# fegemo/palette-and-histo-gan

Measured on AMD Instinct MI355X. Metric: train images/sec (64x64x4 sprites), higher is better.
Workload: dtype bf16

## Files before the change

### include/p2pgan.h

```cpp
#ifndef P2PGAN_H
#define P2PGAN_H

#ifdef __cplusplus
extern "C" {
#endif

typedef enum { P2P_F32 = 0, P2P_BF16 = 1 } p2p_dtype;
typedef enum { P2P_OP_G = 0, P2P_OP_P = 1, P2P_OP_W = 2 } p2p_convop;
typedef enum { P2P_ACT_NONE = 0, P2P_ACT_LEAKY = 1, P2P_ACT_RELU = 2 } p2p_act;

typedef struct {
    void* ptr;
    long long img_stride;
    int row_stride;
    int ld;
} p2p_tensor;

typedef struct {
    const void* ptr;
    int kind;
    int nslabs;
    long long slab_stride;
    int ld;
    int coff;
} p2p_gsrc;

const char* p2p_last_error(void);
int p2p_version(void);
int p2p_view_halo_pixels(void);


int p2p_conv_direct(int op, int stride, int dtype, int N, int LH, int LW, int Cg, int Cd,
                    const p2p_tensor* hi, const p2p_tensor* lo, const void* w, const float* bias,
                    float* dw, float* dbias, void* stream);

int p2p_igemm(int op, int dtype, int N, int LH, int LW, int Cg, int Cd,
              const p2p_tensor* hi, const p2p_tensor* lo, const void* w,
              int splitk, float* slabs, float* stat_part, void* stream);
int p2p_igemm_stat_slots(int op, int N, int LH, int LW, int ncols);

int p2p_brig_ok(int op, int dtype, int N, int LH, int LW, int Cg, int Cd);
int p2p_igemm_norm_act_ok(int op, int dtype, int N, int LH, int LW, int Cg, int Cd);
int p2p_igemm_norm_act(int op, int dtype, int N, int LH, int LW, int Cg, int Cd, const p2p_tensor* hi, const p2p_tensor* lo,
                       const void* w, const float* gamma, const float* beta, float eps, int act, float alpha,
                       const p2p_tensor* act_out, float* stats, void* stream);
int p2p_brig_stat_slots(int op, int dtype, int N, int LH, int LW, int Cg, int Cd);
int p2p_igemm_layer_stat_slots(int op, int dtype, int N, int LH, int LW, int Cg, int Cd);

int p2p_igemm_edge(int op, int stride, int dtype, int N, int LH, int LW, int cin_pad, int ncols, int w_rows,
                   const p2p_tensor* in, const p2p_tensor* out, const void* w, const float* bias,
                   int act, float alpha, void* stream);

int p2p_conv_strip_ok(int op, int dtype, int N, int LH, int LW, int Cg, int Cd);
int p2p_conv_strip_stat_slots(int op, int dtype, int N, int LH, int LW, int Cg, int Cd);
int p2p_conv_strip(int op, int dtype, int N, int LH, int LW, int Cg, int Cd,
                   const p2p_tensor* hi, const p2p_tensor* lo, const void* w, float* stat_part, void* stream);

int p2p_conv_fewout_ok(int op, int stride, int dtype, int N, int LH, int LW, int cin_pad, int ncols);
int p2p_conv_fewout(int op, int stride, int dtype, int N, int LH, int LW, int cin_pad, int ncols, int w_rows,
                    const p2p_tensor* in, const p2p_tensor* out, const void* w, const float* bias,
                    int act, float alpha, void* stream);

int p2p_conv_fewin_ok(int op, int stride, int dtype, int N, int LH, int LW, int cin_pad, int ncols);
int p2p_conv_fewin(int op, int stride, int dtype, int N, int LH, int LW, int cin_pad, int ncols, int w_rows,
                   const p2p_tensor* in, const p2p_tensor* out, const void* w, const float* bias,
                   int act, float alpha, void* stream);

int p2p_conv_fewin_actbwd(int op, int stride, int dtype, int N, int LH, int LW, int cin_pad, int ncols, int w_rows,
                          const p2p_tensor* in, const p2p_tensor* out, const void* w, const p2p_tensor* gate, float alpha,
                          void* stream);

long long p2p_wgemm_workspace_bytes(int N, int LH, int LW, int Cg, int Cd, int msplit);
int p2p_wgemm(int dtype, int N, int LH, int LW, int Cg, int Cd,
              const p2p_tensor* hi, const p2p_tensor* lo, float* dw,
              int msplit, void* workspace, void* stream);

int p2p_wgemm_edge(int dtype, int stride, int N, int LH, int LW, int Cg, int Cd,
                   const p2p_tensor* hi, const p2p_tensor* lo, float* dw,
                   int msplit, void* workspace, void* stream);

int p2p_wgrad_small_blocks(int dtype, int stride, int N, int LH, int LW, int Cg, int Cd, int hi_ld, int lo_ld);
int p2p_wgrad_small(int dtype, int stride, int N, int LH, int LW, int Cg, int Cd,
                    const p2p_tensor* hi, const p2p_tensor* lo, float* dw, void* workspace, void* stream);

long long p2p_view_colsum_workspace_bytes(int dtype, int N, int H, int W, int C, const p2p_tensor* v);
int p2p_view_colsum(int dtype, int N, int H, int W, int C, const p2p_tensor* v, float* out, float* workspace, void* stream);


int p2p_norm_act_fwd(int dtype, int N, int H, int W, int C,
                     const void* raw, int raw_kind, int nslabs, long long slab_stride,
                     const float* gamma, const float* beta, float eps, int act, float alpha,
                     const unsigned char* mask, const p2p_tensor* out, void* raw_out, float* stats,
                     float* ws, long long ws_bytes, int nsplit, void* stream);
int p2p_norm_act_fwd_tail(int dtype, int N, int H, int W, int C,
                          const void* raw, int raw_kind, int nslabs, long long slab_stride,
                          const float* gamma, const float* beta, float eps, int act, float alpha,
                          const unsigned char* mask, const p2p_tensor* out, void* raw_out, float* stats,
                          float* ws, long long ws_bytes, int nsplit, const p2p_tensor* tail, int tail_ch, void* stream);

int p2p_norm_act_bwd(int dtype, int N, int H, int W, int C,
                     const void* raw, const float* stats, const float* gamma, const float* beta,
                     int act, float alpha, const unsigned char* mask,
                     const p2p_gsrc* g1, const p2p_gsrc* g2,
                     const p2p_tensor* draw, float* dgamma_part, float* dbeta_part,
                     float* ws, long long ws_bytes, int nsplit, void* stream);

int p2p_act_bwd(int dtype, int N, int H, int W, int C, const p2p_tensor* act_out, const p2p_gsrc* g1,
                const p2p_gsrc* g2, float alpha, const p2p_tensor* draw, void* stream);

int p2p_colsum(const float* part, int rows, int cols, float scale, float* out, void* stream);

int p2p_colsum_batched(const float* part, const int* table, int ntasks, int max_cols, float* out, void* stream);


#define P2P_LOSS_BLOCKS 256
int p2p_loss_partials_sum(const float* partials, int K, float* out, void* stream);

int p2p_bce_logits(int dtype, int N2, int n_real, int H, int W, const p2p_tensor* logits,
                   float inv_count, const p2p_tensor* dlogits_d, const p2p_tensor* dlogits_g,
                   float* partials, void* stream);
int p2p_bce_logits_pad8(int dtype, int N2, int n_real, int H, int W, const p2p_tensor* logits,
                        float inv_count, const p2p_tensor* dlogits_d, const p2p_tensor* dlogits_g,
                        float* partials, void* stream);

int p2p_tanh_l1_fwd(int dtype, int N, int H, int W, int C, const p2p_tensor* z, const p2p_tensor* real,
                    const p2p_tensor* fake, float inv_count, float* partials, float* fake_f32, void* stream);
int p2p_tanh_l1_fwd_pair(int dtype, int N, int H, int W, const p2p_tensor* z, const p2p_tensor* real_pair,
                         const p2p_tensor* fake_pair, float inv_count, float* partials, float* fake_f32, void* stream);

int p2p_tanh_l1_bwd(int dtype, int N, int H, int W, int C, const p2p_tensor* fake, const p2p_tensor* real,
                    const p2p_gsrc* g_d, const p2p_gsrc* g_extra, float l1_scale,
                    const p2p_tensor* dz, void* stream);
int p2p_tanh_l1_bwd_pad8(int dtype, int N, int H, int W, const p2p_tensor* fake, const p2p_tensor* real,
                         const p2p_gsrc* g_d, const p2p_gsrc* g_extra, float l1_scale, const p2p_tensor* dz,
                         void* stream);


int p2p_rgbuv_hist_fwd(int dtype, int N, int H, int W, const p2p_tensor* img, float* hist, void* stream);
int p2p_rgbuv_hist_general(int dtype, int N, int H, int W, const p2p_tensor* img, int size, int method, float sigma, float* hist,
                           void* stream);

long long p2p_rgbuv_hist_fwd3_workspace_bytes(int N);
int p2p_rgbuv_hist_fwd3(int dtype, int N, int H, int W, const p2p_tensor* img, const float* points, const int* npoints, int cap,
                        float* hist, float* workspace, void* stream);
int p2p_rgbuv_points(int dtype, int N, int H, int W, const p2p_tensor* img, int cap, float* points, int* npoints, void* stream);

int p2p_hist_normalize(const float* raw, int N, float* out, void* stream);

int p2p_hellinger_fwd(const float* hist_true, const float* hist_pred, int N, float* tot_true, float* tot_pred,
                      float* sq_part, float* sq_sum, void* stream);
int p2p_hellinger_finish(const float* sq_sum, float inv_global_batch, float* loss_out, void* stream);
int p2p_rgbuv_hist_hellinger_bwd(int dtype, int N, int H, int W, const p2p_tensor* fake, const float* hist_true,
                                 const float* hist_pred, const float* tot_true, const float* tot_pred,
                                 const float* sq_sum, float coef, float* gh_ws, float* dimg, void* stream);
int p2p_rgbuv_hist_hellinger_bwd3(int dtype, int N, int H, int W, const p2p_tensor* fake, const float* hist_true,
                                  const float* hist_pred, const float* tot_true, const float* tot_pred, const float* sq_sum,
                                  float coef, float* gh_ws, float* dimg, void* stream);

int p2p_hist_normalize_bwd(const float* raw, const float* grad_out, int N, int size, float* gh, void* stream);
int p2p_rgbuv_hist_bwd(int dtype, int N, int H, int W, const p2p_tensor* img, const float* gh, float* dimg, void* stream);
int p2p_rgbuv_hist_general_bwd(int dtype, int N, int H, int W, const p2p_tensor* img, int size, int method, float sigma,
                               const float* gh, float* dimg, void* stream);

long long p2p_soft_palette_workspace_bytes(int N, int H, int W);
int p2p_soft_palette_fwd(int N, int H, int W, const float* img, const int* palette, const int* sizes, int K, float tau,
                         float* hist, float* conf, float* workspace, void* stream);
int p2p_soft_palette_bwd(int N, int H, int W, const float* img, const int* palette, const int* sizes, int K, float tau,
                         const float* gh, const float* gm, float* dimg, void* stream);
int p2p_palette_extract(int N, int H, int W, const float* img, int cap, int* palette_out, int* sizes_out, void* stream);
int p2p_palette_snap(int N, int H, int W, const float* img, const int* palette, const int* sizes, int K, int* index_out,
                     float* image_out, int* dist_out, int* counts_out, long long* stats_out, void* stream);

long long p2p_diffaug_workspace_bytes(int N, int H, int W);
int p2p_diffaug_fwd(int N, int H, int W, const float* img, const float* color, const int* geometry, int ch, int cw,
                    int policy_bits, float fill, float* out, float* workspace, void* stream);
int p2p_diffaug_bwd(int N, int H, int W, const float* grad_out, const float* color, const int* geometry, int ch, int cw,
                    int policy_bits, float fill, float* grad_img, float* workspace, void* stream);


#define P2P_SOFTMAX_MAX_BLOCKS 8192
int p2p_softmax_cce_argmax(int dtype, int N, int H, int W, int C, const p2p_tensor* z, const p2p_tensor* target,
                           const p2p_tensor* fake_idx, float grad_scale, float inv_count, const p2p_tensor* dz,
                           float* probs_out, float* loss_part, float* loss_out, void* stream);
int p2p_softmax_bwd(int dtype, int N, int H, int W, int C, const float* probs, const float* gp, const float* gz,
                    float scale, const p2p_tensor* dz, void* stream);
int p2p_argmax_lastdim(const float* probs, long long M, int C, int* out, void* stream);

int p2p_head_softmax_ok(int dtype, int N, int H, int W, int cin_pad, int ncls);
long long p2p_head_softmax_workspace_bytes(int N, int H);
int p2p_head_softmax_cce(int dtype, int N, int H, int W, int cin_pad, int ncls, const p2p_tensor* in, const void* wt,
                         const float* bias, const p2p_tensor* target, const p2p_tensor* fake_idx, float grad_scale,
                         float inv_count, const p2p_tensor* dz, float* dbias, float* workspace, float* loss_out, void* stream);
int p2p_head_dgrad_ok(int dtype, int N, int H, int W, int ncls, int cout, int w_rows, int dz_ld, int out_ld);
int p2p_head_dgrad(int dtype, int N, int H, int W, int ncls, int cout, const p2p_tensor* dz, const void* wn, int w_rows,
                   const p2p_tensor* out, void* stream);


int p2p_adam_flat(float* p, const float* g, float* m, float* v, long long n, int t,
                  float lr, float beta1, float beta2, float eps, float gscale, void* stream);

int p2p_adam_tick(int* t_dev, float* lr_t_dev, float lr, float beta1, float beta2, void* stream);
int p2p_adam_flat_dev(float* p, const float* g, float* m, float* v, long long n, const float* lr_t_dev,
                      float beta1, float beta2, float eps, float gscale, void* stream);
int p2p_counter_add(long long* counter_dev, long long inc, void* stream);
int p2p_grad_accumulate(float* dst, const float* src, long long n, int first, void* stream);

int p2p_weight_prep(int dtype, const float* w, int Cg, int Cd, void* wn, void* wt, void* stream);

int p2p_weight_prep_pad(int dtype, const float* w, int Cg, int Cd, void* wn, int wn_rows, int wn_cols,
                        void* wt, int wt_rows, int wt_cols, void* stream);

typedef struct p2p_prep_task {
    const float* w;
    void* wn;
    void* wt;
    int Cg, Cd, wn_rows, wn_cols, wt_rows, wt_cols, tiles_g, tiles_d;
    long long first_block;
} p2p_prep_task;
long long p2p_weight_prep_task_blocks(int Cg, int Cd, int wn_rows, int wn_cols, int wt_rows, int wt_cols,
                                      int have_wn, int have_wt, int* tiles_g, int* tiles_d);
int p2p_weight_prep_batched(int dtype, const p2p_prep_task* tasks_dev, int ntasks, long long total_blocks, void* stream);
int p2p_adam_prep_batched(int dtype, long long n_elems, const p2p_prep_task* tasks_dev, int ntasks, long long total_blocks,
                          float* params, const float* grads, float* m, float* v, const float* lr_t_dev, float beta1, float beta2,
                          float eps, void* stream);


int p2p_pack_input(int dtype, int N, int H, int W, int C, const void* src, int src_is_int,
                   const p2p_tensor* dst, void* stream);
int p2p_pack_input_multi(int dtype, int N, int H, int W, int C, const void* src, int src_is_int,
                         const p2p_tensor* dsts, int ndst, void* stream);
int p2p_pack_pair(int dtype, int N, int H, int W, const float* source, const float* target,
                  const p2p_tensor* v_src, const p2p_tensor* v_c6, const p2p_tensor* v_dreal, const p2p_tensor* v_dfake,
                  void* stream);
int p2p_pack_pair_idx(int dtype, int N, int H, int W, const int* source, const int* target,
                      const p2p_tensor* v_src, const p2p_tensor* v_c6, const p2p_tensor* v_dreal, const p2p_tensor* v_dfake,
                      void* stream);
int p2p_finish_losses(const float* slots, int aux_slot, int l1_slot, float lambda_l1, float lambda_aux, float* out,
                      void* stream);
int p2p_unpack(int dtype, int N, int H, int W, int C, const p2p_tensor* src, float* dst, void* stream);

int p2p_dropout_mask(unsigned char* mask, long long n, long long seed, long long counter, void* stream);
int p2p_dropout_mask_dev(unsigned char* mask, long long n, long long seed, const long long* counter_dev,
                         long long salt, long long elem_offset, void* stream);


int p2p_comm_unique_id(void* id_out_128_bytes);
int p2p_comm_init(const void* id_128_bytes, int rank, int world, void** comm_out);
int p2p_comm_allreduce_sum(void* comm, float* buf, long long n, void* stream);
int p2p_comm_destroy(void* comm);

int p2p_event_create(void** ev_out);
int p2p_event_destroy(void* ev);
int p2p_event_record(void* ev, void* stream);
int p2p_stream_wait_event(void* stream, void* ev);
int p2p_arm_stop_event(void* ev);
int p2p_disarm_stop_event(int* was_pending);

#define P2P_REPLAY_MAX_ARGS 24
typedef struct {
    int fn;
    int nargs;
    unsigned ind64;
    unsigned ind32;
    unsigned long long a[P2P_REPLAY_MAX_ARGS];
} p2p_replay_call;
int p2p_replay_fn_index(const char* name);
int p2p_replay_fn_nargs(int fn);
int p2p_replay(const p2p_replay_call* calls, int n);


int p2p_png_unfilter(const unsigned char* filtered, int height, int row_bytes, int bpp, unsigned char* out);

int p2p_sprites_rgba_batch(const void* sprites, int n_sprites, int S, const int* src_idx, const int* tgt_idx, const float* aug,
                           int B, int normalise, float* source, float* target, void* stream);

int p2p_gather_rows_i32(const int* table, int n_rows, int row_ints, const int* sel, int B, int* out, void* stream);

int p2p_palette_relabel_batch(const int* src_idx, const int* tgt_idx, const int* palette, const int* perm, const int* inv,
                              int B, int n, int P, int C, int* src_out, int* tgt_out, int* pal_out, void* stream);


int p2p_inc_prep(int N, int H, int W, int C, const float* images, const int* rows, const int* cols, const int* chans, int OH,
                 int OW, double w0, double w1, int filter, const p2p_tensor* out, float* minmax, void* stream);
int p2p_inc_conv(int N, int H, int W, int Cin, int kh, int kw, int stride, int pad_top, int pad_left, int OH, int OW, int Cout,
                 const p2p_tensor* in, const float* w, const float* scale, const float* shift, const p2p_tensor* out, void* stream);
int p2p_inc_pool(int kind, int N, int H, int W, int C, const p2p_tensor* in, const p2p_tensor* out, void* stream);
int p2p_inc_gap(int N, int H, int W, int C, const p2p_tensor* in, float* out, void* stream);

#ifdef __cplusplus
}
#endif
#endif
```

### palette_and_histo_gan_amd/_lib.py

```python
import ctypes as C
import os

HERE = os.path.dirname(os.path.abspath(__file__))
LIB_PATH = os.environ.get("P2P_LIB") or os.path.join(HERE, "libp2pgan_hip.so")

F32, BF16 = 0, 1
OP_G, OP_P, OP_W = 0, 1, 2
ACT_NONE, ACT_LEAKY, ACT_RELU = 0, 1, 2


class Tensor(C.Structure):
    _fields_ = [("ptr", C.c_void_p), ("img_stride", C.c_longlong), ("row_stride", C.c_int), ("ld", C.c_int)]


class GSrc(C.Structure):
    _fields_ = [("ptr", C.c_void_p), ("kind", C.c_int), ("nslabs", C.c_int), ("slab_stride", C.c_longlong),
                ("ld", C.c_int), ("coff", C.c_int)]


_TP = C.POINTER(Tensor)
_GP = C.POINTER(GSrc)
_vp, _i, _f, _ll = C.c_void_p, C.c_int, C.c_float, C.c_longlong

SIGNATURES = {
    "p2p_conv_direct": [_i, _i, _i, _i, _i, _i, _i, _i, _TP, _TP, _vp, _vp, _vp, _vp, _vp],
    "p2p_igemm": [_i, _i, _i, _i, _i, _i, _i, _TP, _TP, _vp, _i, _vp, _vp, _vp],
    "p2p_igemm_norm_act": [_i, _i, _i, _i, _i, _i, _i, _TP, _TP, _vp, _vp, _vp, _f, _i, _f, _TP, _vp, _vp],
    "p2p_igemm_edge": [_i, _i, _i, _i, _i, _i, _i, _i, _i, _TP, _TP, _vp, _vp, _i, _f, _vp],
    "p2p_conv_strip": [_i, _i, _i, _i, _i, _i, _i, _TP, _TP, _vp, _vp, _vp],
    "p2p_conv_fewin": [_i, _i, _i, _i, _i, _i, _i, _i, _i, _TP, _TP, _vp, _vp, _i, _f, _vp],
    "p2p_conv_fewin_actbwd": [_i, _i, _i, _i, _i, _i, _i, _i, _i, _TP, _TP, _vp, _TP, _f, _vp],
    "p2p_conv_fewout": [_i, _i, _i, _i, _i, _i, _i, _i, _i, _TP, _TP, _vp, _vp, _i, _f, _vp],
    "p2p_wgemm_edge": [_i, _i, _i, _i, _i, _i, _i, _TP, _TP, _vp, _i, _vp, _vp],
    "p2p_wgrad_small": [_i, _i, _i, _i, _i, _i, _i, _TP, _TP, _vp, _vp, _vp],
    "p2p_view_colsum": [_i, _i, _i, _i, _i, _TP, _vp, _vp, _vp],
    "p2p_act_bwd": [_i, _i, _i, _i, _i, _TP, _GP, _GP, _f, _TP, _vp],
    "p2p_weight_prep_pad": [_i, _vp, _i, _i, _vp, _i, _i, _vp, _i, _i, _vp],
    "p2p_wgemm": [_i, _i, _i, _i, _i, _i, _TP, _TP, _vp, _i, _vp, _vp],
    "p2p_norm_act_fwd": [_i, _i, _i, _i, _i, _vp, _i, _i, _ll, _vp, _vp, _f, _i, _f, _vp, _TP, _vp, _vp, _vp, _ll, _i, _vp],
    "p2p_norm_act_fwd_tail": [_i, _i, _i, _i, _i, _vp, _i, _i, _ll, _vp, _vp, _f, _i, _f, _vp, _TP, _vp, _vp, _vp, _ll, _i, _TP, _i, _vp],
    "p2p_norm_act_bwd": [_i, _i, _i, _i, _i, _vp, _vp, _vp, _vp, _i, _f, _vp, _GP, _GP, _TP, _vp, _vp, _vp, _ll, _i, _vp],
    "p2p_colsum": [_vp, _i, _i, _f, _vp, _vp],
    "p2p_colsum_batched": [_vp, _vp, _i, _i, _vp, _vp],
    "p2p_bce_logits": [_i, _i, _i, _i, _i, _TP, _f, _TP, _TP, _vp, _vp],
    "p2p_bce_logits_pad8": [_i, _i, _i, _i, _i, _TP, _f, _TP, _TP, _vp, _vp],
    "p2p_loss_partials_sum": [_vp, _i, _vp, _vp],
    "p2p_tanh_l1_fwd": [_i, _i, _i, _i, _i, _TP, _TP, _TP, _f, _vp, _vp, _vp],
    "p2p_tanh_l1_fwd_pair": [_i, _i, _i, _i, _TP, _TP, _TP, _f, _vp, _vp, _vp],
    "p2p_tanh_l1_bwd": [_i, _i, _i, _i, _i, _TP, _TP, _GP, _GP, _f, _TP, _vp],
    "p2p_tanh_l1_bwd_pad8": [_i, _i, _i, _i, _TP, _TP, _GP, _GP, _f, _TP, _vp],
    "p2p_adam_flat": [_vp, _vp, _vp, _vp, _ll, _i, _f, _f, _f, _f, _f, _vp],
    "p2p_adam_tick": [_vp, _vp, _f, _f, _f, _vp],
    "p2p_adam_flat_dev": [_vp, _vp, _vp, _vp, _ll, _vp, _f, _f, _f, _f, _vp],
    "p2p_counter_add": [_vp, _ll, _vp],
    "p2p_grad_accumulate": [_vp, _vp, _ll, _i, _vp],
    "p2p_dropout_mask_dev": [_vp, _ll, _ll, _vp, _ll, _ll, _vp],
    "p2p_weight_prep": [_i, _vp, _i, _i, _vp, _vp, _vp],
    "p2p_weight_prep_batched": [_i, _vp, _i, _ll, _vp],
    "p2p_adam_prep_batched": [_i, _ll, _vp, _i, _ll, _vp, _vp, _vp, _vp, _vp, _f, _f, _f, _vp],
    "p2p_pack_input": [_i, _i, _i, _i, _i, _vp, _i, _TP, _vp],
    "p2p_pack_pair": [_i, _i, _i, _i, _vp, _vp, _TP, _TP, _TP, _TP, _vp],
    "p2p_pack_pair_idx": [_i, _i, _i, _i, _vp, _vp, _TP, _TP, _TP, _TP, _vp],
    "p2p_pack_input_multi": [_i, _i, _i, _i, _i, _vp, _i, _TP, _i, _vp],
    "p2p_finish_losses": [_vp, _i, _i, _f, _f, _vp, _vp],
    "p2p_unpack": [_i, _i, _i, _i, _i, _TP, _vp, _vp],
    "p2p_dropout_mask": [_vp, _ll, _ll, _ll, _vp],
    "p2p_rgbuv_hist_fwd": [_i, _i, _i, _i, _TP, _vp, _vp],
    "p2p_hist_normalize": [_vp, _i, _vp, _vp],
    "p2p_rgbuv_hist_general": [_i, _i, _i, _i, _TP, _i, _i, _f, _vp, _vp],
    "p2p_rgbuv_hist_fwd3": [_i, _i, _i, _i, _TP, _vp, _vp, _i, _vp, _vp, _vp],
    "p2p_rgbuv_points": [_i, _i, _i, _i, _TP, _i, _vp, _vp, _vp],
    "p2p_hellinger_fwd": [_vp, _vp, _i, _vp, _vp, _vp, _vp, _vp],
    "p2p_hellinger_finish": [_vp, _f, _vp, _vp],
    "p2p_rgbuv_hist_hellinger_bwd": [_i, _i, _i, _i, _TP, _vp, _vp, _vp, _vp, _vp, _f, _vp, _vp, _vp],
    "p2p_rgbuv_hist_hellinger_bwd3": [_i, _i, _i, _i, _TP, _vp, _vp, _vp, _vp, _vp, _f, _vp, _vp, _vp],
    "p2p_hist_normalize_bwd": [_vp, _vp, _i, _i, _vp, _vp],
    "p2p_rgbuv_hist_bwd": [_i, _i, _i, _i, _TP, _vp, _vp, _vp],
    "p2p_rgbuv_hist_general_bwd": [_i, _i, _i, _i, _TP, _i, _i, _f, _vp, _vp, _vp],
    "p2p_soft_palette_fwd": [_i, _i, _i, _vp, _vp, _vp, _i, _f, _vp, _vp, _vp, _vp],
    "p2p_soft_palette_bwd": [_i, _i, _i, _vp, _vp, _vp, _i, _f, _vp, _vp, _vp, _vp],
    "p2p_palette_extract": [_i, _i, _i, _vp, _i, _vp, _vp, _vp],
    "p2p_palette_snap": [_i, _i, _i, _vp, _vp, _vp, _i, _vp, _vp, _vp, _vp, _vp, _vp],
    "p2p_diffaug_fwd": [_i, _i, _i, _vp, _vp, _vp, _i, _i, _i, _f, _vp, _vp, _vp],
    "p2p_diffaug_bwd": [_i, _i, _i, _vp, _vp, _vp, _i, _i, _i, _f, _vp, _vp, _vp],
    "p2p_softmax_cce_argmax": [_i, _i, _i, _i, _i, _TP, _TP, _TP, _f, _f, _TP, _vp, _vp, _vp, _vp],
    "p2p_softmax_bwd": [_i, _i, _i, _i, _i, _vp, _vp, _vp, _f, _TP, _vp],
    "p2p_argmax_lastdim": [_vp, _ll, _i, _vp, _vp],
    "p2p_head_dgrad": [_i, _i, _i, _i, _i, _i, _TP, _vp, _i, _TP, _vp],
    "p2p_head_softmax_cce": [_i, _i, _i, _i, _i, _i, _TP, _vp, _vp, _TP, _TP, _f, _f, _TP, _vp, _vp, _vp, _vp],
    "p2p_comm_unique_id": [_vp],
    "p2p_comm_init": [_vp, _i, _i, C.POINTER(_vp)],
    "p2p_comm_allreduce_sum": [_vp, _vp, _ll, _vp],
    "p2p_comm_destroy": [_vp],
    "p2p_event_create": [C.POINTER(_vp)],
    "p2p_event_destroy": [_vp],
    "p2p_event_record": [_vp, _vp],
    "p2p_stream_wait_event": [_vp, _vp],
    "p2p_arm_stop_event": [_vp],
    "p2p_disarm_stop_event": [C.POINTER(C.c_int)],
    "p2p_png_unfilter": [_vp, _i, _i, _i, _vp],
    "p2p_sprites_rgba_batch": [_vp, _i, _i, _vp, _vp, _vp, _i, _i, _vp, _vp, _vp],
    "p2p_gather_rows_i32": [_vp, _i, _i, _vp, _i, _vp, _vp],
    "p2p_palette_relabel_batch": [_vp, _vp, _vp, _vp, _vp, _i, _i, _i, _i, _vp, _vp, _vp, _vp],
    "p2p_inc_prep": [_i, _i, _i, _i, _vp, _vp, _vp, _vp, _i, _i, C.c_double, C.c_double, _i, _TP, _vp, _vp],
    "p2p_inc_conv": [_i, _i, _i, _i, _i, _i, _i, _i, _i, _i, _i, _i, _TP, _vp, _vp, _vp, _TP, _vp],
    "p2p_inc_pool": [_i, _i, _i, _i, _i, _TP, _TP, _vp],
    "p2p_inc_gap": [_i, _i, _i, _i, _TP, _vp, _vp],
}
SPECIAL = {"p2p_last_error": ([], C.c_char_p),
           "p2p_replay_fn_index": ([C.c_char_p], C.c_int), "p2p_replay_fn_nargs": ([_i], C.c_int),
           "p2p_replay": ([_vp, _i], C.c_int), "p2p_version": ([], C.c_int), "p2p_view_halo_pixels": ([], C.c_int),
           "p2p_igemm_stat_slots": ([_i, _i, _i, _i, _i], C.c_int),
           "p2p_brig_ok": ([_i, _i, _i, _i, _i, _i, _i], C.c_int),
           "p2p_igemm_norm_act_ok": ([_i, _i, _i, _i, _i, _i, _i], C.c_int),
           "p2p_brig_stat_slots": ([_i, _i, _i, _i, _i, _i, _i], C.c_int),
           "p2p_igemm_layer_stat_slots": ([_i, _i, _i, _i, _i, _i, _i], C.c_int),
           "p2p_conv_fewin_ok": ([_i, _i, _i, _i, _i, _i, _i, _i], C.c_int),
           "p2p_conv_strip_ok": ([_i, _i, _i, _i, _i, _i, _i], C.c_int),
           "p2p_conv_strip_stat_slots": ([_i, _i, _i, _i, _i, _i, _i], C.c_int),
           "p2p_conv_fewout_ok": ([_i, _i, _i, _i, _i, _i, _i, _i], C.c_int),
           "p2p_wgrad_small_blocks": ([_i, _i, _i, _i, _i, _i, _i, _i, _i], C.c_int),
           "p2p_wgemm_workspace_bytes": ([_i, _i, _i, _i, _i, _i], C.c_longlong),
           "p2p_rgbuv_hist_fwd3_workspace_bytes": ([_i], C.c_longlong),
           "p2p_soft_palette_workspace_bytes": ([_i, _i, _i], C.c_longlong),
           "p2p_diffaug_workspace_bytes": ([_i, _i, _i], C.c_longlong),
           "p2p_head_softmax_ok": ([_i, _i, _i, _i, _i, _i], C.c_int),
           "p2p_head_dgrad_ok": ([_i, _i, _i, _i, _i, _i, _i, _i, _i], C.c_int),
           "p2p_head_softmax_workspace_bytes": ([_i, _i], C.c_longlong),
           "p2p_view_colsum_workspace_bytes": ([_i, _i, _i, _i, _i, _TP], C.c_longlong),
           "p2p_weight_prep_task_blocks": ([_i, _i, _i, _i, _i, _i, _i, _i, C.POINTER(C.c_int), C.POINTER(C.c_int)], C.c_longlong)}


class PrepTask(C.Structure):
    _fields_ = [("w", C.c_void_p), ("wn", C.c_void_p), ("wt", C.c_void_p),
                ("Cg", C.c_int), ("Cd", C.c_int), ("wn_rows", C.c_int), ("wn_cols", C.c_int),
                ("wt_rows", C.c_int), ("wt_cols", C.c_int), ("tiles_g", C.c_int), ("tiles_d", C.c_int),
                ("first_block", C.c_longlong)]

_lib = None


class P2PError(RuntimeError):
    pass


def lib():
    global _lib
    if _lib is None:
        if not os.path.exists(LIB_PATH):
            raise P2PError(f"{LIB_PATH} is missing: run `python -c 'import __graft_entry__ as g; g.build()'` "
                           "(hipcc --offload-arch=gfx950); there is no CPU fallback")
        import torch
        L = C.CDLL(LIB_PATH)
        for name, argtypes in SIGNATURES.items():
            fn = getattr(L, name)
            fn.argtypes = argtypes
            fn.restype = C.c_int
        for name, (argtypes, restype) in SPECIAL.items():
            fn = getattr(L, name)
            fn.argtypes = argtypes
            fn.restype = restype
        _lib = L
    return _lib


_fns = {}


def call(name, *args):
    fn = _fns.get(name)
    if fn is None:
        fn = _fns[name] = getattr(lib(), name)
    rc = fn(*args)
    if rc != 0:
        raise P2PError(f"{name} failed (rc={rc}): {lib().p2p_last_error().decode()}")


def exported_symbols():
    return list(SIGNATURES) + list(SPECIAL)
```

### palette_and_histo_gan_amd/csrc/norm_act.hip

```cpp
#include "p2p_common.hpp"
#include <stdlib.h>

typedef __attribute__((__vector_size__(2 * sizeof(float)))) float f32x2;

template <typename T>
__device__ __forceinline__ float raw_load(const void* raw, int raw_kind, int nslabs, long long slab, long long e) {
    if (raw_kind == 1) return to_f32(((const T*)raw)[e]);
    float s = 0.f;
    const float* p = (const float*)raw + e;
    for (int k = 0; k < nslabs; ++k) s += p[(long long)k * slab];
    return to_f32(from_f32<T>(s));
}

template <typename T>
__global__ void norm_act_fwd_kernel(int H, int W, int C, int CB, const void* __restrict__ raw, int raw_kind,
                                    int nslabs, long long slab, const float* __restrict__ gamma,
                                    const float* __restrict__ beta, float eps, int act, float alpha,
                                    const unsigned char* __restrict__ mask, TView out, T* __restrict__ raw_out,
                                    float* __restrict__ stats) {
    extern __shared__ float sm[];
    const int n = blockIdx.x;
    const int c0 = blockIdx.y * CB;
    const int cb = min(CB, C - c0);
    const int PL = blockDim.x / CB;
// ... 877 lines not shown
        f32x4 tsum = red[0][cq];
#pragma unroll
        for (int i = 1; i < 16; ++i) tsum += red[i][cq];
        for (int k = 0; k < 4; ++k)
            if (c + k < cols) out[ooff + c + k] = tsum[k];
    }
}

extern "C" int p2p_colsum_batched(const float* part, const int* table, int ntasks, int max_cols, float* out, void* stream) {
    P2P_REQUIRE(part && table && out && ntasks > 0 && max_cols > 0, "p2p_colsum_batched: bad args");
    P2P_REQUIRE(((uintptr_t)part % 16) == 0, "p2p_colsum_batched: partials must be 16-byte aligned");
    colsum_batched_kernel<<<dim3((max_cols + 63) / 64, ntasks), 256, 0, (hipStream_t)stream>>>(part, table, out);
    return p2p_check_launch("p2p_colsum_batched");
}

template <typename T>
__global__ void act_bwd_kernel(int N, int H, int W, int C, TView actv, GSrc g1, GSrc g2, float alpha, TView draw) {
    long long total = (long long)N * H * W * C;
    for (long long i = (long long)blockIdx.x * blockDim.x + threadIdx.x; i < total; i += (long long)gridDim.x * blockDim.x) {
        int c = (int)(i % C);
        long long p = i / C;
        int x = (int)(p % W);
        int y = (int)((p / W) % H);
        int n = (int)(p / ((long long)W * H));
        float a = to_f32(((const T*)actv.ptr)[actv.off(n, y, x) + c]);
        float g = gsrc_load<T>(g1, p, c) + gsrc_load<T>(g2, p, c);
        ((T*)draw.ptr)[draw.off(n, y, x) + c] = from_f32<T>(a > 0.f ? g : alpha * g);
    }
}

template <typename T>
__global__ void act_bwd_vec_kernel(int N, int H, int W, int C, TView actv, GSrc g1, GSrc g2, float alpha, TView draw) {
    constexpr int VN = VecOf<T>::N;
    const int cv = C / VN;
    long long total = (long long)N * H * W * cv;
    for (long long i = (long long)blockIdx.x * blockDim.x + threadIdx.x; i < total; i += (long long)gridDim.x * blockDim.x) {
        int c = (int)(i % cv) * VN;
        long long p = i / cv;
        int x = (int)(p % W);
        int y = (int)((p / W) % H);
        int n = (int)(p / ((long long)W * H));
        float a[VN], ga[VN], gb[VN];
        vload<T>((const T*)actv.ptr + actv.off(n, y, x) + c, a);
        gsrc_vload<T>(g1, p, c, ga);
        gsrc_vload<T>(g2, p, c, gb);
#pragma unroll
        for (int k = 0; k < VN; ++k) { float g = ga[k] + gb[k]; a[k] = a[k] > 0.f ? g : alpha * g; }
        vstore<T>((T*)draw.ptr + draw.off(n, y, x) + c, a);
    }
}

extern "C" int p2p_act_bwd(int dtype, int N, int H, int W, int C, const p2p_tensor* act_out, const p2p_gsrc* g1,
                           const p2p_gsrc* g2, float alpha, const p2p_tensor* draw, void* stream) {
    P2P_REQUIRE(N > 0 && H > 0 && W > 0 && C > 0 && act_out && act_out->ptr && g1 && draw && draw->ptr, "p2p_act_bwd: bad args");
    {
        const int esz = dtype == P2P_BF16 ? 2 : 4, vn = 16 / esz;
        auto gs_ok = [&](const p2p_gsrc* g) {
            if (!g || !g->ptr || g->kind == 0) return true;
            return g->kind != 1 || (g->ld % vn == 0 && g->coff % vn == 0 && ((uintptr_t)g->ptr % 16) == 0);
        };
        if (C % 8 == 0 && act_out->ld % vn == 0 && draw->ld % vn == 0 && ((uintptr_t)act_out->ptr % 16) == 0 &&
            ((uintptr_t)draw->ptr % 16) == 0 && gs_ok(g1) && gs_ok(g2)) {
            long long tv = (long long)N * H * W * (C / vn);
            long long bl = (tv + 255) / 256;
            if (bl > 8192) bl = 8192;
            P2P_DISPATCH_DTYPE(dtype, P2P_LAUNCH_LAST((act_bwd_vec_kernel<T>), dim3((unsigned)bl), dim3(256), 0, (hipStream_t)stream,
                                                      N, H, W, C, make_view(act_out), make_gsrc(g1), make_gsrc(g2), alpha, make_view(draw)));
            return p2p_check_launch("p2p_act_bwd");
        }
    }
    long long total = (long long)N * H * W * C;
    long long blocks = (total + 255) / 256;
    if (blocks > 4096) blocks = 4096;
    P2P_DISPATCH_DTYPE(dtype, (act_bwd_kernel<T><<<dim3((unsigned)blocks), 256, 0, (hipStream_t)stream>>>(
                                  N, H, W, C, make_view(act_out), make_gsrc(g1), make_gsrc(g2), alpha, make_view(draw))));
    return p2p_check_launch("p2p_act_bwd");
}

__global__ void colsum_kernel(const float* __restrict__ part, int rows, int cols, float scale, float* __restrict__ out) {
    int c = blockIdx.x * blockDim.x + threadIdx.x;
    if (c >= cols) return;
    float s = 0.f;
    for (int r = 0; r < rows; ++r) s += part[(long long)r * cols + c];
    out[c] = s * scale;
}

static inline int pick_cb(int C) { return C >= 64 ? 64 : (C >= 32 ? 32 : (C >= 16 ? 16 : (C >= 8 ? 8 : (C >= 4 ? 4 : (C >= 2 ? 2 : 1))))); }

static int norm_act_fwd_impl(int dtype, int N, int H, int W, int C, const void* raw, int raw_kind, int nslabs,
                             long long slab_stride, const float* gamma, const float* beta, float eps, int act,
                             float alpha, const unsigned char* mask, const p2p_tensor* out, void* raw_out,
                             float* stats, float* ws, long long ws_bytes, int nsplit, const p2p_tensor* tail, int tail_ch,
                             void* stream) {
    P2P_REQUIRE(N > 0 && H > 0 && W > 0 && C > 0, "p2p_norm_act_fwd: bad shape");
    P2P_REQUIRE(raw && out && out->ptr, "p2p_norm_act_fwd: null pointer");
    P2P_REQUIRE(raw_kind == 1 || (raw_kind == 2 && nslabs >= 1), "p2p_norm_act_fwd: bad raw_kind/nslabs");
    P2P_REQUIRE((gamma == nullptr) == (beta == nullptr), "p2p_norm_act_fwd: gamma/beta must both be set or null");
    P2P_REQUIRE(!gamma || stats, "p2p_norm_act_fwd: stats required with normalisation");
    const int esz = dtype == P2P_BF16 ? 2 : 4, vn = 16 / esz;
    const bool vec = C % vn == 0 && out->ld % vn == 0 && ((uintptr_t)out->ptr % 16) == 0 && ((uintptr_t)raw % 16) == 0 &&
                     (!raw_out || ((uintptr_t)raw_out % 16) == 0) && (raw_kind == 1 || slab_stride % 4 == 0) && C % 8 == 0;
    const int tvecs = tail ? tail_ch / vn : 0;
    TView tv = tail ? make_view(tail) : TView{};
    if (tail) {
        P2P_REQUIRE(tail->ptr && tail_ch > 0 && tail_ch % vn == 0 && tail->ld % vn == 0 && ((uintptr_t)tail->ptr % 16) == 0,
                    "p2p_norm_act_fwd_tail: the tail must be whole 16-byte vectors");
        int cgt = C > 64 ? 64 : C;
        while (C % cgt) cgt -= vn;
        P2P_REQUIRE(vec && H * W > 16 && 256 % (cgt / vn) == 0, "p2p_norm_act_fwd_tail: shape not served by the vector form");
    }
    if (vec && H * W <= 16) {
        int lgG, ppl;
        small_geom(H * W, lgG, ppl);
        const long long items = (long long)N * (C / vn);
        const long long threads = items << lgG;
        const dim3 grid((unsigned)((threads + 255) / 256));
        hipStream_t st = (hipStream_t)stream;
#define NF_SMALL2(P_, S_) norm_act_fwd_small<T, P_, S_><<<grid, 256, 0, st>>>(H * W, W, C, lgG, items, raw, raw_kind, nslabs, slab_stride, gamma, \
                                                                   beta, eps, act, alpha, mask, make_view(out), (T*)raw_out, stats)
#define NF_SMALL(P_) do { if (raw_kind == 2) NF_SMALL2(P_, 4); else NF_SMALL2(P_, 0); } while (0)
        if (ppl == 1) { P2P_DISPATCH_DTYPE(dtype, NF_SMALL(1)); }
        else if (ppl == 2) { P2P_DISPATCH_DTYPE(dtype, NF_SMALL(2)); }
        else { P2P_DISPATCH_DTYPE(dtype, NF_SMALL(4)); }
#undef NF_SMALL
#undef NF_SMALL2
        return p2p_check_launch("p2p_norm_act_fwd");
    }
    const bool legacy = nsplit > 0 && (nsplit & 0x100);
    const int n_geom = (nsplit > 0 && (nsplit & 0x200)) ? 256 : N;
    if (nsplit > 0) nsplit &= 0xff;
    if (vec && gamma && !tail && nsplit >= 0 && !legacy) {
        int ppl = 0;
        const int rcg = norm_bwd_reg_geom(n_geom, H * W, C, vn, ppl, true);
        if (rcg) {
            hipStream_t st = (hipStream_t)stream;
            const dim3 grid((unsigned)(((N + 7) / 8) * 8 * (C / rcg)));
#define NF_REG2(P_, S_) norm_act_fwd_reg<T, P_, S_><<<grid, 256, 0, st>>>(N, H * W, W, C, rcg, raw, raw_kind, nslabs, slab_stride, gamma, beta, eps, act, alpha, \
                                                                mask, make_view(out), (T*)raw_out, stats)
#define NF_REG(P_) do { if (raw_kind == 2) NF_REG2(P_, 4); else NF_REG2(P_, 0); } while (0)
            if (ppl == 1) { P2P_DISPATCH_DTYPE(dtype, NF_REG(1)); }
            else if (ppl == 2) { P2P_DISPATCH_DTYPE(dtype, NF_REG(2)); }
            else if (ppl == 4) { P2P_DISPATCH_DTYPE(dtype, NF_REG(4)); }
            else { P2P_DISPATCH_DTYPE(dtype, NF_REG(8)); }
#undef NF_REG
#undef NF_REG2
            return p2p_check_launch("p2p_norm_act_fwd");
        }
    }
    if (vec) {
        int CG = C > 64 ? 64 : C;
        while (C % CG) CG -= vn;
        int vpp = CG / vn;
        if (256 % vpp == 0) {
            hipStream_t st = (hipStream_t)stream;
            const int prr = 256 / vpp;
            int sp = nsplit < 1 ? 1 : nsplit;
            while (sp > 1 && (H * W + sp - 1) / sp < prr) sp >>= 1;
            if (nsplit < 0 && gamma && ws) {
                const int nslots = -nsplit;
                int sp2 = 1;
                while ((long long)N * (C / CG) * sp2 < 2048 && (H * W) / (sp2 * 2) >= prr && sp2 < 64) sp2 *= 2;
                dim3 grid3(N, C / CG, sp2);
                P2P_DISPATCH_DTYPE(dtype, (norm_act_fwd_vec<T, 3><<<grid3, 256, 0, st>>>(
                                              H, W, C, CG, raw, raw_kind, nslabs, slab_stride, gamma, beta, eps, act, alpha, mask,
                                              make_view(out), (T*)raw_out, stats, ws, nslots, tv, tvecs)));
                return p2p_check_launch("p2p_norm_act_fwd");
            }
            if (!ws || (long long)N * sp * C * 2 * 4 > ws_bytes) sp = gamma ? 1 : sp;
            dim3 grid(N, C / CG, sp);
            if (sp == 1 || !gamma) {
                P2P_DISPATCH_DTYPE(dtype, (norm_act_fwd_vec<T, 0><<<grid, 256, 0, st>>>(
                                              H, W, C, CG, raw, raw_kind, nslabs, slab_stride, gamma, beta, eps, act, alpha, mask,
                                              make_view(out), (T*)raw_out, stats, ws, 0, tv, tvecs)));
            } else {
                P2P_DISPATCH_DTYPE(dtype, (norm_act_fwd_vec<T, 1><<<grid, 256, 0, st>>>(
                                              H, W, C, CG, raw, raw_kind, nslabs, slab_stride, gamma, beta, eps, act, alpha, mask,
                                              make_view(out), (T*)raw_out, stats, ws, 0, tv, tvecs)));
                P2P_DISPATCH_DTYPE(dtype, (norm_act_fwd_vec<T, 2><<<grid, 256, 0, st>>>(
                                              H, W, C, CG, raw, raw_kind, nslabs, slab_stride, gamma, beta, eps, act, alpha, mask,
                                              make_view(out), (T*)raw_out, stats, ws, 0, tv, tvecs)));
            }
            return p2p_check_launch("p2p_norm_act_fwd");
        }
    }
    int CB = pick_cb(C);
    dim3 grid(N, (C + CB - 1) / CB);
    size_t shm = sizeof(float) * 256;
    P2P_DISPATCH_DTYPE(dtype, (norm_act_fwd_kernel<T><<<grid, 256, shm, (hipStream_t)stream>>>(
                                  H, W, C, CB, raw, raw_kind, nslabs, slab_stride, gamma, beta, eps, act, alpha, mask,
                                  make_view(out), (T*)raw_out, stats)));
    return p2p_check_launch("p2p_norm_act_fwd");
}

extern "C" int p2p_norm_act_fwd(int dtype, int N, int H, int W, int C, const void* raw, int raw_kind, int nslabs,
                                long long slab_stride, const float* gamma, const float* beta, float eps, int act,
                                float alpha, const unsigned char* mask, const p2p_tensor* out, void* raw_out,
                                float* stats, float* ws, long long ws_bytes, int nsplit, void* stream) {
    return norm_act_fwd_impl(dtype, N, H, W, C, raw, raw_kind, nslabs, slab_stride, gamma, beta, eps, act, alpha, mask, out,
                             raw_out, stats, ws, ws_bytes, nsplit, nullptr, 0, stream);
}

extern "C" int p2p_norm_act_fwd_tail(int dtype, int N, int H, int W, int C, const void* raw, int raw_kind, int nslabs,
                                     long long slab_stride, const float* gamma, const float* beta, float eps, int act,
                                     float alpha, const unsigned char* mask, const p2p_tensor* out, void* raw_out,
                                     float* stats, float* ws, long long ws_bytes, int nsplit, const p2p_tensor* tail,
                                     int tail_ch, void* stream) {
    P2P_REQUIRE(tail, "p2p_norm_act_fwd_tail: null tail");
    return norm_act_fwd_impl(dtype, N, H, W, C, raw, raw_kind, nslabs, slab_stride, gamma, beta, eps, act, alpha, mask, out,
                             raw_out, stats, ws, ws_bytes, nsplit, tail, tail_ch, stream);
}

extern "C" int p2p_norm_act_bwd(int dtype, int N, int H, int W, int C, const void* raw, const float* stats,
                                const float* gamma, const float* beta, int act, float alpha,
                                const unsigned char* mask, const p2p_gsrc* g1, const p2p_gsrc* g2,
                                const p2p_tensor* draw, float* dgamma_part, float* dbeta_part, float* ws,
                                long long ws_bytes, int nsplit, void* stream) {
    P2P_REQUIRE(N > 0 && H > 0 && W > 0 && C > 0, "p2p_norm_act_bwd: bad shape");
    P2P_REQUIRE(raw && draw && draw->ptr && g1, "p2p_norm_act_bwd: null pointer");
    P2P_REQUIRE(!gamma || (stats && beta && dgamma_part && dbeta_part), "p2p_norm_act_bwd: norm needs stats/beta/partials");
    const int esz = dtype == P2P_BF16 ? 2 : 4, vn = 16 / esz;
    auto gs_ok = [&](const p2p_gsrc* g) {
        if (!g || !g->ptr || g->kind == 0) return true;
        if (g->kind == 1) return g->ld % vn == 0 && g->coff % vn == 0 && ((uintptr_t)g->ptr % 16) == 0;
        return true;
    };
    const bool vec = gamma && C % 8 == 0 && draw->ld % vn == 0 && ((uintptr_t)draw->ptr % 16) == 0 &&
                     ((uintptr_t)raw % 16) == 0 && gs_ok(g1) && gs_ok(g2);
    const bool g_slabs = (g1 && g1->kind == 2) || (g2 && g2->kind == 2);
    if (vec && H * W <= 16) {
        int lgG, ppl;
        small_geom(H * W, lgG, ppl);
        const long long items = (long long)N * (C / vn);
        const long long threads = items << lgG;
        const dim3 grid((unsigned)((threads + 255) / 256));
        hipStream_t st = (hipStream_t)stream;
#define NB_SMALL2(P_, S_) P2P_LAUNCH_LAST((norm_act_bwd_small<T, P_, S_>), grid, dim3(256), 0, st, H * W, W, C, lgG, items, (const T*)raw, stats, gamma, beta, act, \
                                     alpha, mask, make_gsrc(g1), make_gsrc(g2), make_view(draw), dgamma_part, dbeta_part)
#define NB_SMALL(P_) do { if (g_slabs) NB_SMALL2(P_, 4); else NB_SMALL2(P_, 0); } while (0)
        if (ppl == 1) { P2P_DISPATCH_DTYPE(dtype, NB_SMALL(1)); }
        else if (ppl == 2) { P2P_DISPATCH_DTYPE(dtype, NB_SMALL(2)); }
        else { P2P_DISPATCH_DTYPE(dtype, NB_SMALL(4)); }
#undef NB_SMALL
#undef NB_SMALL2
        return p2p_check_launch("p2p_norm_act_bwd");
    }
    const bool legacy = nsplit > 0 && (nsplit & 0x100);
    const int n_geom = (nsplit > 0 && (nsplit & 0x200)) ? 256 : N;
    if (nsplit > 0) nsplit &= 0xff;
    if (vec && !legacy) {
        int ppl = 0;
        const int rcg = norm_bwd_reg_geom(n_geom, H * W, C, vn, ppl);
        if (rcg) {
            hipStream_t st = (hipStream_t)stream;
            const dim3 grid((unsigned)(((N + 7) / 8) * 8 * (C / rcg)));
#define NB_REG2(P_, S_) P2P_LAUNCH_LAST((norm_act_bwd_reg<T, P_, S_>), grid, dim3(256), 0, st, N, H * W, W, C, rcg, (const T*)raw, stats, gamma, beta, act, \
                                   alpha, mask, make_gsrc(g1), make_gsrc(g2), make_view(draw), dgamma_part, dbeta_part)
#define NB_REG(P_) do { if (g_slabs) NB_REG2(P_, 4); else NB_REG2(P_, 0); } while (0)
            if (ppl == 1) { P2P_DISPATCH_DTYPE(dtype, NB_REG(1)); }
            else if (ppl == 2) { P2P_DISPATCH_DTYPE(dtype, NB_REG(2)); }
            else if (ppl == 4) { P2P_DISPATCH_DTYPE(dtype, NB_REG(4)); }
            else { P2P_DISPATCH_DTYPE(dtype, NB_REG(8)); }
#undef NB_REG
#undef NB_REG2
            return p2p_check_launch("p2p_norm_act_bwd");
        }
    }
    if (vec) {
        int CG = C > 64 ? 64 : C;
        while (C % CG) CG -= vn;
        const bool narrow = nsplit > 1 && CG == 64 && C % 32 == 0 && (long long)N * (C / 32) >= 1024 && H * W >= 64;
        if (narrow) CG = 32;
        int vpp = CG / vn;
        if (256 % vpp == 0) {
            hipStream_t st = (hipStream_t)stream;
            const int prr = 256 / vpp;
            int sp = (nsplit < 1 || narrow) ? 1 : nsplit;
            while (sp > 1 && (H * W + sp - 1) / sp < prr) sp >>= 1;
            if (!ws || (long long)N * sp * C * 2 * 4 > ws_bytes) sp = 1;
            dim3 grid(N, C / CG, sp);
            if (sp == 1) {
                P2P_DISPATCH_DTYPE(dtype, P2P_LAUNCH_LAST((norm_act_bwd_vec<T, 0>), grid, dim3(256), 0, st,
                                                          H, W, C, CG, (const T*)raw, stats, gamma, beta, act, alpha, mask, make_gsrc(g1),
                                                          make_gsrc(g2), make_view(draw), dgamma_part, dbeta_part, ws));
            } else {
                P2P_DISPATCH_DTYPE(dtype, (norm_act_bwd_vec<T, 1><<<grid, 256, 0, st>>>(
                                              H, W, C, CG, (const T*)raw, stats, gamma, beta, act, alpha, mask, make_gsrc(g1),
                                              make_gsrc(g2), make_view(draw), dgamma_part, dbeta_part, ws)));
                P2P_DISPATCH_DTYPE(dtype, P2P_LAUNCH_LAST((norm_act_bwd_vec<T, 2>), grid, dim3(256), 0, st,
                                                          H, W, C, CG, (const T*)raw, stats, gamma, beta, act, alpha, mask, make_gsrc(g1),
                                                          make_gsrc(g2), make_view(draw), dgamma_part, dbeta_part, ws));
            }
            return p2p_check_launch("p2p_norm_act_bwd");
        }
    }
    int CB = pick_cb(C);
    dim3 grid(N, (C + CB - 1) / CB);
    size_t shm = sizeof(float) * 512;
    P2P_DISPATCH_DTYPE(dtype, (norm_act_bwd_kernel<T><<<grid, 256, shm, (hipStream_t)stream>>>(
                                  H, W, C, CB, (const T*)raw, stats, gamma, beta, act, alpha, mask, make_gsrc(g1),
                                  make_gsrc(g2), make_view(draw), dgamma_part, dbeta_part)));
    return p2p_check_launch("p2p_norm_act_bwd");
}

extern "C" int p2p_colsum(const float* part, int rows, int cols, float scale, float* out, void* stream) {
    P2P_REQUIRE(part && out && rows > 0 && cols > 0, "p2p_colsum: bad args");
    colsum_kernel<<<dim3((cols + 255) / 256), 256, 0, (hipStream_t)stream>>>(part, rows, cols, scale, out);
    return p2p_check_launch("p2p_colsum");
}
```

### palette_and_histo_gan_amd/csrc/optim.hip

```cpp
#include "p2p_common.hpp"
#include <math.h>
#include <stdlib.h>

__global__ void adam_flat_kernel(float* __restrict__ p, const float* __restrict__ g, float* __restrict__ m,
                                 float* __restrict__ v, long long n, float lr_t, float b1, float b2, float eps,
                                 float gscale) {
    long long i = (long long)blockIdx.x * blockDim.x + threadIdx.x;
    long long stride = (long long)gridDim.x * blockDim.x;
    for (; i < n; i += stride) {
        float gi = g[i] * gscale;
        float mi = b1 * m[i] + (1.f - b1) * gi;
        float vi = b2 * v[i] + (1.f - b2) * gi * gi;
        m[i] = mi;
        v[i] = vi;
        p[i] = p[i] - lr_t * mi / (sqrtf(vi) + eps);
    }
}

extern "C" int p2p_adam_flat(float* p, const float* g, float* m, float* v, long long n, int t, float lr, float beta1,
                             float beta2, float eps, float gscale, void* stream) {
    P2P_REQUIRE(p && g && m && v && n > 0 && t >= 1, "p2p_adam_flat: bad args");
    double lr_t = (double)lr * sqrt(1.0 - pow((double)beta2, (double)t)) / (1.0 - pow((double)beta1, (double)t));
    long long blocks = (n + 255) / 256;
    if (blocks > 4096) blocks = 4096;
    adam_flat_kernel<<<dim3((unsigned)blocks), 256, 0, (hipStream_t)stream>>>(p, g, m, v, n, (float)lr_t, beta1, beta2,
                                                                             eps, gscale);
    return p2p_check_launch("p2p_adam_flat");
}

__global__ void adam_tick_kernel(int* __restrict__ t, float* __restrict__ lr_t, float lr, float b1, float b2) {
    int tt = t[0] + 1;
    t[0] = tt;
    lr_t[0] = (float)((double)lr * sqrt(1.0 - pow((double)b2, (double)tt)) / (1.0 - pow((double)b1, (double)tt)));
}

__global__ void adam_flat_dev_kernel(float* __restrict__ p, const float* __restrict__ g, float* __restrict__ m,
                                     float* __restrict__ v, long long n, const float* __restrict__ lr_t_dev, float b1,
                                     float b2, float eps, float gscale) {
    const float lr_t = lr_t_dev[0];
    long long i = ((long long)blockIdx.x * blockDim.x + threadIdx.x) * 4;
    long long stride = (long long)gridDim.x * blockDim.x * 4;
    for (; i + 3 < n; i += stride) {
        f32x4 gi = *(const f32x4*)(g + i), mi = *(const f32x4*)(m + i), vi = *(const f32x4*)(v + i), pi = *(const f32x4*)(p + i);
#pragma unroll
        for (int k = 0; k < 4; ++k) {
            float gg = gi[k] * gscale;
            mi[k] = b1 * mi[k] + (1.f - b1) * gg;
            vi[k] = b2 * vi[k] + (1.f - b2) * gg * gg;
            pi[k] = pi[k] - lr_t * mi[k] / (sqrtf(vi[k]) + eps);
        }
        *(f32x4*)(m + i) = mi; *(f32x4*)(v + i) = vi; *(f32x4*)(p + i) = pi;
    }
    if (blockIdx.x == 0 && threadIdx.x == 0)
        for (long long j = n / 4 * 4; j < n; ++j) {
            float gg = g[j] * gscale;
            float mj = b1 * m[j] + (1.f - b1) * gg, vj = b2 * v[j] + (1.f - b2) * gg * gg;
            m[j] = mj; v[j] = vj; p[j] = p[j] - lr_t * mj / (sqrtf(vj) + eps);
        }
}

extern "C" int p2p_adam_tick(int* t_dev, float* lr_t_dev, float lr, float beta1, float beta2, void* stream) {
    P2P_REQUIRE(t_dev && lr_t_dev, "p2p_adam_tick: null pointer");
    adam_tick_kernel<<<1, 1, 0, (hipStream_t)stream>>>(t_dev, lr_t_dev, lr, beta1, beta2);
    return p2p_check_launch("p2p_adam_tick");
}

extern "C" int p2p_adam_flat_dev(float* p, const float* g, float* m, float* v, long long n, const float* lr_t_dev,
                                 float beta1, float beta2, float eps, float gscale, void* stream) {
    P2P_REQUIRE(p && g && m && v && n > 0 && lr_t_dev, "p2p_adam_flat_dev: bad args");
    P2P_REQUIRE(((uintptr_t)p % 16) == 0 && ((uintptr_t)g % 16) == 0 && ((uintptr_t)m % 16) == 0 && ((uintptr_t)v % 16) == 0,
                "p2p_adam_flat_dev: buffers must be 16-byte aligned");
    long long blocks = (n / 4 + 255) / 256;
    if (blocks > 8192) blocks = 8192;
    if (blocks < 1) blocks = 1;
    adam_flat_dev_kernel<<<dim3((unsigned)blocks), 256, 0, (hipStream_t)stream>>>(p, g, m, v, n, lr_t_dev, beta1, beta2, eps, gscale);
    return p2p_check_launch("p2p_adam_flat_dev");
}

__global__ void counter_add_kernel(long long* c, long long inc) { c[0] += inc; }

extern "C" int p2p_counter_add(long long* counter_dev, long long inc, void* stream) {
    P2P_REQUIRE(counter_dev, "p2p_counter_add: null pointer");
    counter_add_kernel<<<1, 1, 0, (hipStream_t)stream>>>(counter_dev, inc);
    return p2p_check_launch("p2p_counter_add");
}

__global__ void grad_accumulate_kernel(float* __restrict__ dst, const float* __restrict__ src, long long n, int first) {
    long long i = ((long long)blockIdx.x * blockDim.x + threadIdx.x) * 4;
    long long stride = (long long)gridDim.x * blockDim.x * 4;
    for (; i + 3 < n; i += stride) {
        f32x4 s = *(const f32x4*)(src + i);
        if (!first) {
            f32x4 d = *(const f32x4*)(dst + i);
#pragma unroll
            for (int k = 0; k < 4; ++k) s[k] = d[k] + s[k];
        }
        *(f32x4*)(dst + i) = s;
    }
    if (blockIdx.x == 0 && threadIdx.x == 0)
        for (long long j = n / 4 * 4; j < n; ++j) dst[j] = first ? src[j] : dst[j] + src[j];
}

extern "C" int p2p_grad_accumulate(float* dst, const float* src, long long n, int first, void* stream) {
    P2P_REQUIRE(dst && src && n > 0, "p2p_grad_accumulate: bad args");
    P2P_REQUIRE(((uintptr_t)dst % 16) == 0 && ((uintptr_t)src % 16) == 0, "p2p_grad_accumulate: buffers must be 16-byte aligned");
    long long blocks = (n / 4 + 255) / 256;
    if (blocks > 8192) blocks = 8192;
    if (blocks < 1) blocks = 1;
    grad_accumulate_kernel<<<dim3((unsigned)blocks), 256, 0, (hipStream_t)stream>>>(dst, src, n, first);
    return p2p_check_launch("p2p_grad_accumulate");
}

template <typename T>
__device__ __forceinline__ void weight_prep_tile(const float* __restrict__ w, int Cg, int Cd, T* __restrict__ wn, int wn_rows,
                                                 int wn_cols, T* __restrict__ wt, int wt_rows, int wt_cols, int t, int g0, int d0,
                                                 float (*tile)[33]) {
    const float* wp = w + (long long)t * Cg * Cd;
    int tx = threadIdx.x & 31, ty = threadIdx.x >> 5;
    for (int r = ty; r < 32; r += 8) {
        int g = g0 + r, d = d0 + tx;
        float val = (g < Cg && d < Cd) ? wp[(long long)g * Cd + d] : 0.f;
        tile[r][tx] = val;
        if (wn && g < wn_rows && d < wn_cols) wn[((long long)t * wn_rows + g) * wn_cols + d] = from_f32<T>(val);
    }
    __syncthreads();
    if (wt) {
        for (int r = ty; r < 32; r += 8) {
            int d = d0 + r, g = g0 + tx;
            if (d < wt_rows && g < wt_cols) wt[((long long)t * wt_rows + d) * wt_cols + g] = from_f32<T>(tile[tx][r]);
        }
    }
}

template <typename T>
__global__ void weight_prep_kernel(const float* __restrict__ w, int Cg, int Cd, T* __restrict__ wn, int wn_rows,
                                   int wn_cols, T* __restrict__ wt, int wt_rows, int wt_cols) {
    __shared__ float tile[32][33];
    weight_prep_tile<T>(w, Cg, Cd, wn, wn_rows, wn_cols, wt, wt_rows, wt_cols, blockIdx.z, blockIdx.y * 32, blockIdx.x * 32, tile);
}

static __host__ __device__ inline bool prep_tile64(int Cg, int Cd, int wn_rows, int wn_cols, int wt_rows, int wt_cols,
                                                   bool have_wn, bool have_wt) {
    return Cg % 64 == 0 && Cd % 64 == 0 && (!have_wn || (wn_rows == Cg && wn_cols == Cd)) &&
           (!have_wt || (wt_rows == Cd && wt_cols == Cg));
}

template <typename T>
__device__ __forceinline__ void weight_prep_tile64(const float* __restrict__ w, int Cg, int Cd, T* __restrict__ wn,
                                                   T* __restrict__ wt, int t, int g0, int d0, float (*tile)[65]) {
    typedef __attribute__((__vector_size__(4 * sizeof(T)))) T vec4_t;
    const float* wp = w + (long long)t * Cg * Cd;
    const int c4 = (threadIdx.x & 15) * 4, r0 = threadIdx.x >> 4;
#pragma unroll
    for (int i = 0; i < 4; ++i) {
        const int r = r0 + 16 * i;
        const f32x4 v = *(const f32x4*)(wp + (long long)(g0 + r) * Cd + d0 + c4);
        tile[r][c4] = v[0]; tile[r][c4 + 1] = v[1]; tile[r][c4 + 2] = v[2]; tile[r][c4 + 3] = v[3];
        if (wn) {
            vec4_t q;
#pragma unroll
            for (int k = 0; k < 4; ++k) q[k] = from_f32<T>(v[k]);
            *(vec4_t*)(wn + ((long long)t * Cg + g0 + r) * Cd + d0 + c4) = q;
        }
    }
    __syncthreads();
    if (wt) {
#pragma unroll
        for (int i = 0; i < 4; ++i) {
            const int d = r0 + 16 * i;
            vec4_t q;
#pragma unroll
            for (int k = 0; k < 4; ++k) q[k] = from_f32<T>(tile[c4 + k][d]);
            *(vec4_t*)(wt + ((long long)t * Cd + d0 + d) * Cg + g0 + c4) = q;
        }
    }
}

template <typename T>
__global__ void weight_prep_batched_kernel(const p2p_prep_task* __restrict__ tasks, int ntasks) {
    __shared__ float tile[64][65];
    const long long b = blockIdx.x;
    int ti = 0;
    while (ti + 1 < ntasks && tasks[ti + 1].first_block <= b) ++ti;
    const p2p_prep_task k = tasks[ti];
    const int local = (int)(b - k.first_block);
    const int per_tap = k.tiles_g * k.tiles_d;
    const int t = local / per_tap, rem = local - t * per_tap;
    const int gy = rem / k.tiles_d, dx = rem - gy * k.tiles_d;
    if (prep_tile64(k.Cg, k.Cd, k.wn_rows, k.wn_cols, k.wt_rows, k.wt_cols, k.wn != nullptr, k.wt != nullptr)) {
        weight_prep_tile64<T>(k.w, k.Cg, k.Cd, (T*)k.wn, (T*)k.wt, t, gy * 64, dx * 64, tile);
        return;
    }
    weight_prep_tile<T>(k.w, k.Cg, k.Cd, (T*)k.wn, k.wn_rows, k.wn_cols, (T*)k.wt, k.wt_rows, k.wt_cols, t, gy * 32, dx * 32,
                        (float (*)[33])tile);
}

struct AdamCtx { float* p0; const float* g0; float* m0; float* v0; const float* lr_t; float b1, b2, eps; };

#define ADAM_ONE(p, g, m, v)                                   \
    do {                                                       \
        m = c.b1 * (m) + (1.f - c.b1) * (g);                   \
        v = c.b2 * (v) + (1.f - c.b2) * (g) * (g);             \
        p = (p) - lr_t * (m) / (sqrtf(v) + c.eps);             \
    } while (0)

template <typename T>
__global__ void adam_prep_batched_kernel(const p2p_prep_task* __restrict__ tasks, int ntasks, AdamCtx c) {
    typedef __attribute__((__vector_size__(4 * sizeof(T)))) T vec4_t;
    __shared__ float tile[64][65];
    const long long b = blockIdx.x;
    int ti = 0;
    while (ti + 1 < ntasks && tasks[ti + 1].first_block <= b) ++ti;
    const p2p_prep_task k = tasks[ti];
    const int local = (int)(b - k.first_block);
    const int per_tap = k.tiles_g * k.tiles_d;
    const int t = local / per_tap, rem = local - t * per_tap;
    const int gy = rem / k.tiles_d, dx = rem - gy * k.tiles_d;
    const float lr_t = c.lr_t[0];
    const long long base = (k.w - c.p0) + (long long)t * k.Cg * k.Cd;
    T* wn = (T*)k.wn;
    T* wt = (T*)k.wt;
    if (prep_tile64(k.Cg, k.Cd, k.wn_rows, k.wn_cols, k.wt_rows, k.wt_cols, wn != nullptr, wt != nullptr)) {
        const int g0 = gy * 64, d0 = dx * 64;
        const int c4 = (threadIdx.x & 15) * 4, r0 = threadIdx.x >> 4;
#pragma unroll
        for (int i = 0; i < 4; ++i) {
            const int r = r0 + 16 * i;
            const long long e = base + (long long)(g0 + r) * k.Cd + d0 + c4;
            f32x4 pv = *(const f32x4*)(c.p0 + e), mv = *(const f32x4*)(c.m0 + e), vv = *(const f32x4*)(c.v0 + e);
            const f32x4 gv = *(const f32x4*)(c.g0 + e);
#pragma unroll
            for (int q = 0; q < 4; ++q) ADAM_ONE(pv[q], gv[q], mv[q], vv[q]);
            *(f32x4*)(c.p0 + e) = pv; *(f32x4*)(c.m0 + e) = mv; *(f32x4*)(c.v0 + e) = vv;
            tile[r][c4] = pv[0]; tile[r][c4 + 1] = pv[1]; tile[r][c4 + 2] = pv[2]; tile[r][c4 + 3] = pv[3];
            if (wn) {
                vec4_t q4;
#pragma unroll
                for (int q = 0; q < 4; ++q) q4[q] = from_f32<T>(pv[q]);
                *(vec4_t*)(wn + ((long long)t * k.Cg + g0 + r) * k.Cd + d0 + c4) = q4;
            }
        }
        __syncthreads();
        if (wt) {
#pragma unroll
            for (int i = 0; i < 4; ++i) {
                const int d = r0 + 16 * i;
                vec4_t q4;
#pragma unroll
                for (int q = 0; q < 4; ++q) q4[q] = from_f32<T>(tile[c4 + q][d]);
                *(vec4_t*)(wt + ((long long)t * k.Cd + d0 + d) * k.Cg + g0 + c4) = q4;
            }
        }
        return;
    }
    float (*t32)[33] = (float (*)[33])tile;
    const int g0 = gy * 32, d0 = dx * 32;
    const int tx = threadIdx.x & 31, ty = threadIdx.x >> 5;
    for (int r = ty; r < 32; r += 8) {
        const int g = g0 + r, d = d0 + tx;
        float val = 0.f;
        if (g < k.Cg && d < k.Cd) {
            const long long e = base + (long long)g * k.Cd + d;
            float pv = c.p0[e], mv = c.m0[e], vv = c.v0[e];
            const float gv = c.g0[e];
            ADAM_ONE(pv, gv, mv, vv);
            val = pv;
            c.p0[e] = pv; c.m0[e] = mv; c.v0[e] = vv;
        }
        t32[r][tx] = val;
        if (wn && g < k.wn_rows && d < k.wn_cols) wn[((long long)t * k.wn_rows + g) * k.wn_cols + d] = from_f32<T>(val);
    }
    __syncthreads();
    if (wt) {
        for (int r = ty; r < 32; r += 8) {
            const int d = d0 + r, g = g0 + tx;
            if (d < k.wt_rows && g < k.wt_cols) wt[((long long)t * k.wt_rows + d) * k.wt_cols + g] = from_f32<T>(t32[tx][r]);
        }
    }
}

extern "C" int p2p_adam_prep_batched(int dtype, long long n_elems, const p2p_prep_task* tasks_dev, int ntasks, long long total_blocks,
                                     float* params, const float* grads, float* m, float* v, const float* lr_t_dev, float beta1,
                                     float beta2, float eps, void* stream) {
    P2P_REQUIRE(tasks_dev && ntasks >= 1 && ntasks <= 64 && total_blocks >= 1 && total_blocks < (1LL << 31) && n_elems > 0,
                "p2p_adam_prep_batched: bad args");
    P2P_REQUIRE(params && grads && m && v && lr_t_dev, "p2p_adam_prep_batched: null pointer");
    P2P_REQUIRE(((uintptr_t)params % 16) == 0 && ((uintptr_t)grads % 16) == 0 && ((uintptr_t)m % 16) == 0 && ((uintptr_t)v % 16) == 0,
                "p2p_adam_prep_batched: buffers must be 16-byte aligned");
    AdamCtx c = {params, grads, m, v, lr_t_dev, beta1, beta2, eps};
    P2P_DISPATCH_DTYPE(dtype, (adam_prep_batched_kernel<T><<<dim3((unsigned)total_blocks), 256, 0, (hipStream_t)stream>>>(tasks_dev, ntasks, c)));
    return p2p_check_launch("p2p_adam_prep_batched");
}

extern "C" long long p2p_weight_prep_task_blocks(int Cg, int Cd, int wn_rows, int wn_cols, int wt_rows, int wt_cols,
                                                 int have_wn, int have_wt, int* tiles_g, int* tiles_d) {
    int gmax = Cg, dmax = Cd;
    if (have_wn) { gmax = gmax > wn_rows ? gmax : wn_rows; dmax = dmax > wn_cols ? dmax : wn_cols; }
    if (have_wt) { gmax = gmax > wt_cols ? gmax : wt_cols; dmax = dmax > wt_rows ? dmax : wt_rows; }
    const int ts = prep_tile64(Cg, Cd, wn_rows, wn_cols, wt_rows, wt_cols, have_wn != 0, have_wt != 0) ? 64 : 32;
    const int tg = (gmax + ts - 1) / ts, td = (dmax + ts - 1) / ts;
    if (tiles_g) *tiles_g = tg;
    if (tiles_d) *tiles_d = td;
    return 16LL * tg * td;
}

extern "C" int p2p_weight_prep_batched(int dtype, const p2p_prep_task* tasks_dev, int ntasks, long long total_blocks, void* stream) {
    P2P_REQUIRE(tasks_dev && ntasks >= 1 && ntasks <= 64 && total_blocks >= 1 && total_blocks < (1LL << 31),
                "p2p_weight_prep_batched: bad args");
    P2P_DISPATCH_DTYPE(dtype, (weight_prep_batched_kernel<T><<<dim3((unsigned)total_blocks), 256, 0, (hipStream_t)stream>>>(tasks_dev, ntasks)));
    return p2p_check_launch("p2p_weight_prep_batched");
}

extern "C" int p2p_weight_prep_pad(int dtype, const float* w, int Cg, int Cd, void* wn, int wn_rows, int wn_cols,
                                   void* wt, int wt_rows, int wt_cols, void* stream) {
    P2P_REQUIRE(w && Cg > 0 && Cd > 0 && (wn || wt), "p2p_weight_prep: bad args");
    int gmax = Cg, dmax = Cd;
    if (wn) { gmax = gmax > wn_rows ? gmax : wn_rows; dmax = dmax > wn_cols ? dmax : wn_cols; }
    if (wt) { gmax = gmax > wt_cols ? gmax : wt_cols; dmax = dmax > wt_rows ? dmax : wt_rows; }
    dim3 grid((dmax + 31) / 32, (gmax + 31) / 32, 16);
    P2P_DISPATCH_DTYPE(dtype, (weight_prep_kernel<T><<<grid, 256, 0, (hipStream_t)stream>>>(
                                  w, Cg, Cd, (T*)wn, wn_rows, wn_cols, (T*)wt, wt_rows, wt_cols)));
    return p2p_check_launch("p2p_weight_prep");
}

extern "C" int p2p_weight_prep(int dtype, const float* w, int Cg, int Cd, void* wn, void* wt, void* stream) {
    return p2p_weight_prep_pad(dtype, w, Cg, Cd, wn, Cg, Cd, wt, Cd, Cg, stream);
}

template <typename T>
__global__ void pack_input_kernel(int N, PixDec dec, int C, const void* __restrict__ src, int src_is_int, TView dst) {
    const unsigned npix = (unsigned)N * dec.H * dec.W;
    for (unsigned p = blockIdx.x * blockDim.x + threadIdx.x; p < npix; p += gridDim.x * blockDim.x) {
        int n, y, x;
        dec(p, n, y, x);
        T* d = (T*)dst.ptr + dst.off(n, y, x);
        const long long e = (long long)p * C;
        for (int c = 0; c < C; ++c) {
            float v = src_is_int ? (float)((const int*)src)[e + c] : ((const float*)src)[e + c];
            d[c] = from_f32<T>(v);
        }
    }
}

struct PackDst { TView v[4]; int n; };

template <typename T>
__global__ void pack_multi_kernel(int N, PixDec dec, int C, const void* __restrict__ src, int src_is_int, PackDst dst) {
    const unsigned npix = (unsigned)N * dec.H * dec.W;
    for (unsigned p = blockIdx.x * blockDim.x + threadIdx.x; p < npix; p += gridDim.x * blockDim.x) {
        int n, y, x;
        dec(p, n, y, x);
        if (C == 4 && !src_is_int) {
            typedef __attribute__((__vector_size__(4 * sizeof(T)))) T vec4_t;
            f32x4 v = *(const f32x4*)((const float*)src + (long long)p * 4);
            vec4_t q;
#pragma unroll
            for (int k = 0; k < 4; ++k) q[k] = from_f32<T>(v[k]);
#pragma unroll
            for (int k = 0; k < 4; ++k)
                if (k < dst.n) *(vec4_t*)((T*)dst.v[k].ptr + dst.v[k].off(n, y, x)) = q;
            continue;
        }
        const long long e = (long long)p * C;
        for (int c = 0; c < C; ++c) {
            float v = src_is_int ? (float)((const int*)src)[e + c] : ((const float*)src)[e + c];
            T q = from_f32<T>(v);
#pragma unroll
            for (int k = 0; k < 4; ++k)
                if (k < dst.n) ((T*)dst.v[k].ptr)[dst.v[k].off(n, y, x) + c] = q;
        }
    }
}

template <typename T>
__global__ void pack_pair_kernel(int N, PixDec dec, const float* __restrict__ source, const float* __restrict__ target, TView v_src,
                                 TView v_c6, TView v_dreal, TView v_dfake) {
    typedef __attribute__((__vector_size__(4 * sizeof(T)))) T vec4_t;
    typedef __attribute__((__vector_size__(8 * sizeof(T)))) T vec8_t;
    const unsigned npix = (unsigned)N * dec.H * dec.W;
// ... 186 lines not shown
```

### palette_and_histo_gan_amd/csrc/replay.hip

```cpp
#include "p2p_common.hpp"
#include <string.h>
#include <utility>

namespace {

template <typename T>
inline T slot_as(unsigned long long v) {
    static_assert(sizeof(T) <= 8, "replayable entry points take scalars and pointers only");
    T t;
    memcpy(&t, &v, sizeof(T));
    return t;
}

template <typename... A, size_t... I>
inline int call_slots(int (*fn)(A...), const unsigned long long* a, std::index_sequence<I...>) {
    return fn(slot_as<A>(a[I])...);
}

template <typename... A>
constexpr int arg_count(int (*)(A...)) { return (int)sizeof...(A); }

template <auto Fn>
struct Thunk {
    template <typename... A>
    static int go(int (*fn)(A...), const unsigned long long* a) { return call_slots(fn, a, std::index_sequence_for<A...>{}); }
    static int call(const unsigned long long* a) { return go(Fn, a); }
};

struct Entry {
    const char* name;
    int (*call)(const unsigned long long*);
    int nargs;
};

#define P2P_E(f) {#f, &Thunk<&f>::call, arg_count(&f)},
constexpr Entry TABLE[] = {
    P2P_E(p2p_conv_direct) P2P_E(p2p_igemm) P2P_E(p2p_igemm_norm_act)
    P2P_E(p2p_igemm_edge) P2P_E(p2p_conv_strip) P2P_E(p2p_conv_fewin)
    P2P_E(p2p_conv_fewin_actbwd) P2P_E(p2p_conv_fewout) P2P_E(p2p_wgemm_edge)
    P2P_E(p2p_wgrad_small) P2P_E(p2p_view_colsum) P2P_E(p2p_act_bwd)
    P2P_E(p2p_weight_prep_pad) P2P_E(p2p_wgemm) P2P_E(p2p_norm_act_fwd)
    P2P_E(p2p_norm_act_fwd_tail) P2P_E(p2p_norm_act_bwd) P2P_E(p2p_colsum)
    P2P_E(p2p_colsum_batched) P2P_E(p2p_bce_logits) P2P_E(p2p_bce_logits_pad8)
    P2P_E(p2p_loss_partials_sum) P2P_E(p2p_tanh_l1_fwd) P2P_E(p2p_tanh_l1_fwd_pair)
    P2P_E(p2p_tanh_l1_bwd) P2P_E(p2p_tanh_l1_bwd_pad8) P2P_E(p2p_adam_flat)
    P2P_E(p2p_adam_tick) P2P_E(p2p_adam_flat_dev) P2P_E(p2p_counter_add) P2P_E(p2p_grad_accumulate)
    P2P_E(p2p_dropout_mask_dev) P2P_E(p2p_weight_prep) P2P_E(p2p_weight_prep_batched)
    P2P_E(p2p_adam_prep_batched) P2P_E(p2p_pack_input) P2P_E(p2p_pack_pair)
    P2P_E(p2p_pack_pair_idx) P2P_E(p2p_pack_input_multi) P2P_E(p2p_finish_losses)
    P2P_E(p2p_unpack) P2P_E(p2p_dropout_mask) P2P_E(p2p_rgbuv_hist_fwd)
    P2P_E(p2p_hist_normalize) P2P_E(p2p_rgbuv_hist_general) P2P_E(p2p_rgbuv_hist_fwd3) P2P_E(p2p_rgbuv_points)
    P2P_E(p2p_hellinger_fwd) P2P_E(p2p_hellinger_finish) P2P_E(p2p_rgbuv_hist_hellinger_bwd)
    P2P_E(p2p_rgbuv_hist_hellinger_bwd3) P2P_E(p2p_softmax_cce_argmax) P2P_E(p2p_argmax_lastdim)
    P2P_E(p2p_head_dgrad) P2P_E(p2p_head_softmax_cce) P2P_E(p2p_comm_unique_id)
    P2P_E(p2p_comm_init) P2P_E(p2p_comm_allreduce_sum) P2P_E(p2p_comm_destroy)
    P2P_E(p2p_event_create) P2P_E(p2p_event_destroy) P2P_E(p2p_event_record)
    P2P_E(p2p_stream_wait_event) P2P_E(p2p_arm_stop_event) P2P_E(p2p_disarm_stop_event) P2P_E(p2p_png_unfilter) P2P_E(p2p_sprites_rgba_batch)
    P2P_E(p2p_gather_rows_i32) P2P_E(p2p_palette_relabel_batch) P2P_E(p2p_hist_normalize_bwd)
    P2P_E(p2p_rgbuv_hist_bwd) P2P_E(p2p_rgbuv_hist_general_bwd) P2P_E(p2p_softmax_bwd)
    P2P_E(p2p_inc_prep) P2P_E(p2p_inc_conv) P2P_E(p2p_inc_pool) P2P_E(p2p_inc_gap)
    P2P_E(p2p_soft_palette_fwd) P2P_E(p2p_soft_palette_bwd) P2P_E(p2p_palette_extract)
    P2P_E(p2p_palette_snap) P2P_E(p2p_diffaug_fwd) P2P_E(p2p_diffaug_bwd)
};
#undef P2P_E
constexpr int NFN = (int)(sizeof(TABLE) / sizeof(TABLE[0]));

constexpr bool table_fits() {
    for (int i = 0; i < NFN; ++i)
        if (TABLE[i].nargs > P2P_REPLAY_MAX_ARGS) return false;
    return true;
}
static_assert(table_fits(), "an entry point has more arguments than P2P_REPLAY_MAX_ARGS");

}

extern "C" int p2p_replay_fn_index(const char* name) {
    if (!name) return -1;
    for (int i = 0; i < NFN; ++i)
        if (strcmp(TABLE[i].name, name) == 0) return i;
    return -1;
}

extern "C" int p2p_replay_fn_nargs(int fn) { return (fn >= 0 && fn < NFN) ? TABLE[fn].nargs : -1; }

extern "C" int p2p_replay(const p2p_replay_call* calls, int n) {
    P2P_REQUIRE(calls || n == 0, "p2p_replay: null call list");
    for (int i = 0; i < n; ++i) {
        const p2p_replay_call& c = calls[i];
        P2P_REQUIRE(c.fn >= 0 && c.fn < NFN && c.nargs == TABLE[c.fn].nargs, "p2p_replay: call %d: bad entry %d / %d arguments", i,
                    c.fn, c.nargs);
        const unsigned long long* ap = c.a;
        unsigned long long a[P2P_REPLAY_MAX_ARGS];
        if (c.ind64 | c.ind32) {
            for (int k = 0; k < c.nargs; ++k) {
                unsigned long long v = c.a[k];
                if ((c.ind64 >> k) & 1u) v = *(const unsigned long long*)(uintptr_t)v;
                else if ((c.ind32 >> k) & 1u) v = *(const unsigned*)(uintptr_t)v;
                a[k] = v;
            }
            ap = a;
        }
        const int rc = TABLE[c.fn].call(ap);
        if (rc != 0) {
            char why[400];
            strncpy(why, p2p_last_error(), sizeof(why) - 1);
            why[sizeof(why) - 1] = 0;
            p2p_set_error("p2p_replay: call %d of %d (%s) failed: %s", i, n, TABLE[c.fn].name, why);
            return rc;
        }
    }
    return 0;
}
```

### palette_and_histo_gan_amd/engine.py

```python
from collections import OrderedDict
import ctypes as C
import math
import os

import numpy as np
import torch

from . import _lib as L
from . import histogram as _histogram

HALO = 2
IN_EPS = 1e-3
LEAKY_ALPHA = 0.3
DOWN_FILTERS = (64, 128, 256, 512, 512, 512)
UP_FILTERS = (512, 512, 256, 128, 64, 32)
UP_DROPOUT = (True, True, True, False, False, False)
MAX_PALETTE_SIZE = 256


def _torch_dtype(dtype):
    return torch.float32 if dtype == L.F32 else torch.bfloat16


_RAW_STREAM = getattr(torch._C, "_cuda_getCurrentRawStream", None)
# ... 123 lines not shown


def _raw(stream):
    return C.c_void_p(stream.cuda_stream)


def _order(after, before):
    ev = _ring_event()
    _op("p2p_event_record", ev, _raw(before))
    _op("p2p_stream_wait_event", _raw(after), ev)


class _SideStream:

    def __init__(self, device, enabled):
        self.enabled = enabled and torch.device(device).type == "cuda"
        self.stream = torch.cuda.Stream(device=device) if self.enabled else None
        self.stop_event_forks = os.environ.get("P2P_STOP_EVENT_FORKS", "1") != "0"
        self._pending = None

    def prefork(self):
        if self.enabled and self.stop_event_forks and not torch.cuda.is_current_stream_capturing():
            self._pending = _ring_event()
            _op("p2p_arm_stop_event", self._pending)

    def fork(self):
        if not self.enabled:
            return
        ev, self._pending = self._pending, None
        if ev is not None:
            unclaimed = C.c_int(0)
            if L.lib().p2p_disarm_stop_event(C.byref(unclaimed)) != 0:
                raise L.P2PError(L.lib().p2p_last_error().decode())
            if not unclaimed.value:
                _op("p2p_stream_wait_event", _raw(self.stream), ev)
                return
            if _REC[0] is not None:
                _REC[0].append(("p2p_disarm_stop_event", (None,)))
        _order(self.stream, torch.cuda.current_stream())

    def run(self):
        return torch.cuda.stream(self.stream) if self.enabled else _NullCtx()

    def join(self):
        if self.enabled:
            _order(torch.cuda.current_stream(), self.stream)


class _LightEvent:
    def __init__(self, st):
        self.ev = _ring_event()
        _op("p2p_event_record", self.ev, _raw(st))

    def wait(self, st):
        _op("p2p_stream_wait_event", _raw(st), self.ev)


def _record_event():
    return _LightEvent(torch.cuda.current_stream())


def _wait_event(ev):
    ev.wait(torch.cuda.current_stream())


class _NullCtx:
    def __enter__(self):
        return self

    def __exit__(self, *a):
        return False


class HaloBuf:

    def __init__(self, n, h, w, c, dtype, device):
        self.n, self.h, self.w, self.c, self.dtype = n, h, w, c, dtype
        self.hp, self.wp = h + 2 * HALO, w + 2 * HALO
        numel = n * self.hp * self.wp * c
        self._flat = torch.zeros(numel + 256, dtype=_torch_dtype(dtype), device=device)
        self.t = self._flat[:numel].view(n, self.hp, self.wp, c)
        self.esz = self.t.element_size()
        self._views = {}

    def view(self, coff=0, n0=0):
        v = self._views.get((coff, n0))
        if v is None:
            off = ((n0 * self.hp + HALO) * self.wp + HALO) * self.c + coff
            v = self._views[(coff, n0)] = L.Tensor(self.t.data_ptr() + off * self.esz, self.hp * self.wp, self.wp, self.c)
        return v


class DenseBuf:

    def __init__(self, n, h, w, c, torch_dtype, device):
        self.n, self.h, self.w, self.c = n, h, w, c
        self.t = torch.empty((n * h * w, c), dtype=torch_dtype, device=device)
        self.esz = self.t.element_size()
        self._views = {}

    def view(self, coff=0, n0=0):
        v = self._views.get((coff, n0))
        if v is None:
            v = self._views[(coff, n0)] = L.Tensor(self.t.data_ptr() + (n0 * self.h * self.w * self.c + coff) * self.esz,
                                                   self.h * self.w, self.w, self.c)
        return v

    def ptr(self, n0=0):
        return C.c_void_p(self.t.data_ptr() + n0 * self.h * self.w * self.c * self.esz)

    def gsrc(self, coff=0, kind=1, nslabs=1, n0=0):
        return L.GSrc(self.t.data_ptr() + n0 * self.h * self.w * self.c * self.esz, kind, nslabs,
                      self.n * self.h * self.w * self.c, self.c, coff)


def pad8(c):
    return (c + 7) // 8 * 8


def up32(c):
    return (c + 31) // 32 * 32


def _p(t, off_elems=0):
    return C.c_void_p(t.data_ptr() + off_elems * t.element_size())


NULL = C.c_void_p(0)


class ParamStore:

    BUCKET_MIN = 4 * 1024 * 1024

    def __init__(self, shapes, device):
        self.shapes = OrderedDict(shapes)
        self.offsets = OrderedDict()
        kernels = [k for k in self.shapes if k.endswith(".kernel")]
        small = [k for k in self.shapes if not k.endswith(".kernel")]
        off, self.buckets, start, self.bucket_of = 0, [], 0, {}
        for k in reversed(kernels):
            self.offsets[k] = off
            off += int(np.prod(self.shapes[k]))
            off = (off + 3) // 4 * 4
            self.bucket_of[k[:-7]] = len(self.buckets)
            if off - start >= self.BUCKET_MIN:
                self.buckets.append((start, off))
                start = off
        if off > start:
            self.buckets.append((start, off))
        self.bucket_last_layer = {}
        for k in reversed(kernels):
            self.bucket_last_layer[self.bucket_of[k[:-7]]] = k[:-7]
        self.small_range = (off, off)
        for k in small:
            self.offsets[k] = off
            off += int(np.prod(self.shapes[k]))
            off = (off + 3) // 4 * 4
        self.small_range = (self.small_range[0], off)
        self.numel = off
        self.params = torch.zeros(off, dtype=torch.float32, device=device)
        self.grads = None
        self.m = torch.zeros(off, dtype=torch.float32, device=device)
        self.v = torch.zeros(off, dtype=torch.float32, device=device)
        self.t = 0
        self.t_dev = torch.zeros(1, dtype=torch.int32, device=device)
        self.lr_t_dev = torch.zeros(1, dtype=torch.float32, device=device)

    def count(self):
        return int(sum(int(np.prod(s)) for s in self.shapes.values()))

    def view(self, buf, name):
        o = self.offsets[name]
        return buf[o:o + int(np.prod(self.shapes[name]))].view(self.shapes[name])

    def p(self, name):
        return _p(self.params, self.offsets[name])

    def g(self, name):
        return _p(self.grads, self.offsets[name])

    def variable_name(self, t):
        if not isinstance(t, torch.Tensor) or t.device != self.params.device or t.dtype != torch.float32:
            return None
        off = t.data_ptr() - self.params.data_ptr()
        if off < 0 or off % 4 or off >= 4 * self.numel:
            return None
        if getattr(self, "_by_offset", None) is None:
            self._by_offset = {o: k for k, o in self.offsets.items()}
        name = self._by_offset.get(off // 4)
        return name if name is not None and tuple(t.shape) == tuple(self.shapes[name]) else None

    def load(self, values):
        for k in self.shapes:
            self.view(self.params, k).copy_(torch.as_tensor(np.asarray(values[k]), dtype=torch.float32))

    def export(self, buf=None):
        buf = self.params if buf is None else buf
        return OrderedDict((k, self.view(buf, k).detach().cpu().numpy().copy()) for k in self.shapes)


def generator_param_shapes(in_ch, out_ch):
    shapes = OrderedDict()
    c = in_ch
    for i, f in enumerate(DOWN_FILTERS, start=1):
        shapes[f"down{i}.kernel"] = (4, 4, c, f)
        if i > 1:
            shapes[f"down{i}.gamma"] = (f,)
            shapes[f"down{i}.beta"] = (f,)
        c = f
    skips = list(reversed(DOWN_FILTERS[:-1])) + [in_ch]
    for i, (f, s) in enumerate(zip(UP_FILTERS, skips), start=1):
        shapes[f"up{i}.kernel"] = (4, 4, f, c)
        shapes[f"up{i}.gamma"] = (f,)
        shapes[f"up{i}.beta"] = (f,)
        c = f + s
    shapes["last.kernel"] = (4, 4, c, out_ch)
    shapes["last.bias"] = (out_ch,)
    return shapes


def discriminator_param_shapes(in_ch):
    return OrderedDict([("down.kernel", (4, 4, 2 * in_ch, 64)), ("last.kernel", (4, 4, 64, 1)), ("last.bias", (1,))])


class LayerW:

    def __init__(self, cg, cd, hi_pad, lo_pad, need_g, need_p):
        self.cg, self.cd, self.hi_pad, self.lo_pad = cg, cd, hi_pad, lo_pad
        self.need_g, self.need_p = need_g, need_p
        self.wt = self.wn = self.wd = None
        self.main = cg % 32 == 0 and cd % 32 == 0 and hi_pad == cg and lo_pad == cd


class Pix2PixEngine:

    def __init__(self, in_ch=4, out_ch=4, head="tanh", img_size=64, dtype=L.BF16, device="cuda:0", seed=47,
                 use_mfma=True, overlap_wgrad=True):
        assert img_size % 64 == 0 and (img_size & (img_size - 1)) == 0, "IMG_SIZE must be a power of two >= 64"
        L.lib()
        self.in_ch, self.out_ch, self.head, self.S = in_ch, out_ch, head, img_size
        self.dtype, self.device, self.use_mfma = dtype, torch.device(device), use_mfma
        self.tdt = _torch_dtype(dtype)
        if self.device.type == "cuda":
            idx = self.device.index if self.device.index is not None else torch.cuda.current_device()
            if _STREAM_DEVICE[0] is not None and _STREAM_DEVICE[0] != idx and _EVENT_RING:
                raise RuntimeError(f"this process already drives cuda:{_STREAM_DEVICE[0]}; one process per GPU (got cuda:{idx})")
            _STREAM_DEVICE[0] = idx
        self.G = ParamStore(generator_param_shapes(in_ch, out_ch), self.device)
        self.D = ParamStore(discriminator_param_shapes(in_ch), self.device)
        self._grad_all = torch.zeros(self.G.numel + self.D.numel + 16, dtype=torch.float32, device=self.device)
        self.G.grads = self._grad_all[:self.G.numel]
        self.D.grads = self._grad_all[self.G.numel:self.G.numel + self.D.numel]
        self.rng = np.random.default_rng(seed)
        self._slot_seed = C.c_longlong()
        self.seed = int(seed)
        self.mask_counter_dev = torch.zeros(1, dtype=torch.int64, device=self.device)
        self._init_params()
        self.c6_ch = pad8(UP_FILTERS[5] + in_ch)
        self.src_ch = pad8(in_ch)
        self.dcat_ch = pad8(2 * in_ch)
        self.dz_ch = pad8(out_ch)
        self.W = {}
        self._alloc_weight_copies()
        self.plans = {}
        self._slot_lr, self._slot_b1, self._slot_b2, self._slot_eps = C.c_float(), C.c_float(), C.c_float(), C.c_float()
        self.lr, self.beta1, self.beta2, self.adam_eps = 2e-4, 0.5, 0.999, 1e-7
        self.losses = self._grad_all[self.G.numel + self.D.numel:]
        self.loss_part = torch.zeros(5 * 256, dtype=torch.float32, device=self.device)
        self.step_count = 0
        self._ticked = False
        self._adam_head_ev = None
        self.side = _SideStream(self.device, overlap_wgrad)
        self.side_hist = _SideStream(self.device, overlap_wgrad)
        self._dp = None
        self._batch_offset = 0
        self.use_conv_fewout = os.environ.get("P2P_CONV_FEWOUT", "1") != "0"
        self.use_conv_strip = os.environ.get("P2P_CONV_STRIP", "1") != "0"
        self.use_conv_fewin = os.environ.get("P2P_CONV_FEWIN", "1") != "0"
        self.wgemm_want = int(os.environ.get("P2P_WGEMM_WANT", "512"))
        self.batch_invariant = dtype == L.F32 and os.environ.get("P2P_BATCH_INVARIANT", "1") != "0"
        self.wgemm_pipe = os.environ.get("P2P_WGEMM_PIPE", "1") != "0"
        self.wgemm_want_pipe = int(os.environ.get("P2P_WGEMM_WANT_PIPE", "256"))
        self.splitk_target = int(os.environ.get("P2P_SPLITK_TARGET", "0"))
        self._prep_table = {}
        self._head_prepped = False
        self._arena_pool, self._tape_ws = {}, {}
        self._copies_version = 0
        self._down1_wn, self._down1_wn_key = None, None
        self.tape_refusal = None
        self.full_pixels = os.environ.get("P2P_FULL_PIXELS", "1") != "0"
        self.fuse_act_bwd = int(os.environ.get("P2P_FUSE_ACT_BWD", "1"))
        self.fuse_adam = False
        self._adam_tables = {}
        self.replay_max_batch = int(os.environ.get("P2P_REPLAY_MAX_BATCH", str(1 << 30)))
        self._replays, self._replay_seen = OrderedDict(), {}
        self._replay_fn = L.lib().p2p_replay
        self.replay_enabled = os.environ.get("P2P_REPLAY", "1") != "0"
        self._slot_src, self._slot_real, self._slot_out = C.c_void_p(), C.c_void_p(), C.c_void_p()
        self._real_view = L.Tensor(None, 0, 0, 4)
        self.use_head_fused = os.environ.get("P2P_HEAD_FUSED", "1") != "0"
        self.hist_fwd3 = self.hist_bwd3 = self.hist_points = 1
        self.split_prep = int(os.environ.get("P2P_SPLIT_PREP", "1"))
        self.refresh_weight_copies()

    def _slot_property(slot):
        def get(self):
            return getattr(self, slot).value

        def put(self, v):
            getattr(self, slot).value = v
        return property(get, put)

    lr, beta1, beta2 = _slot_property("_slot_lr"), _slot_property("_slot_b1"), _slot_property("_slot_b2")
    adam_eps, seed = _slot_property("_slot_eps"), _slot_property("_slot_seed")
    del _slot_property

    def _init_params(self):
        for store in (self.G, self.D):
            vals = {}
            for k, s in store.shapes.items():
                if k.endswith(".kernel"):
                    vals[k] = self.rng.normal(0.0, 0.02, size=s).astype(np.float32)
                elif k.endswith(".gamma"):
                    vals[k] = np.ones(s, np.float32)
                else:
                    vals[k] = np.zeros(s, np.float32)
            store.load(vals)

    def _store(self, sid):
        return self.G if sid == "G" else self.D

    def _alloc_weight_copies(self):
        dev, tdt = self.device, self.tdt
        for sid, store in (("G", self.G), ("D", self.D)):
            for key in store.shapes:
                if not key.endswith(".kernel"):
                    continue
                name = key[:-7]
                _, _, cg, cd = store.shapes[key]
                hi_pad, lo_pad, need_p = cg, cd, True
                if (sid, name) == ("G", "down1"):
                    hi_pad, need_p = self.src_ch, False
                elif (sid, name) == ("G", "last"):
                    hi_pad, lo_pad = self.c6_ch, self.dz_ch
                elif (sid, name) == ("D", "down"):
                    hi_pad = self.dcat_ch
                elif (sid, name) == ("D", "last"):
                    lo_pad = 8
                lw = LayerW(cg, cd, hi_pad, lo_pad, True, need_p)
                if self.use_mfma:
                    lw.wt = torch.zeros(16 * up32(cd) * hi_pad, dtype=tdt, device=dev)
                    if need_p and not (lw.main and self.dtype == L.F32):
                        lw.wn = torch.zeros(16 * up32(cg) * lo_pad, dtype=tdt, device=dev)
                if (not self.use_mfma or not lw.main) and self.dtype != L.F32:
                    lw.wd = torch.zeros(16 * cg * cd, dtype=tdt, device=dev)
                self.W[(sid, name)] = lw

    def _prep_tasks(self, part="all"):
        if self._prep_table.get(part) is not None:
            return self._prep_table[part]
        head_end = self.G.buckets[-1][0] if len(self.G.buckets) >= 2 else 0
        specs = []
        for (sid, name), lw in self.W.items():
            in_head = sid == "G" and self.G.offsets[name + ".kernel"] + 16 * lw.cg * lw.cd <= head_end
            if (part == "head" and not in_head) or (part == "rest" and in_head) or (part in ("G", "D") and sid != part):
                continue
            master = self._store(sid).p(name + ".kernel")
            if lw.wt is not None or lw.wn is not None:
                specs.append((master, lw.cg, lw.cd, lw.wn, up32(lw.cg), lw.lo_pad, lw.wt, up32(lw.cd), lw.hi_pad))
            if lw.wd is not None:
                specs.append((master, lw.cg, lw.cd, lw.wd, lw.cg, lw.cd, None, 0, 0))
        if not specs:
            self._prep_table[part] = (None, 0, 0)
            return self._prep_table[part]
        tasks = (L.PrepTask * len(specs))()
        first = 0
        for k, (master, cg, cd, wn, wn_r, wn_c, wt, wt_r, wt_c) in enumerate(specs):
            tg, td = C.c_int(0), C.c_int(0)
            nb = L.lib().p2p_weight_prep_task_blocks(cg, cd, wn_r, wn_c, wt_r, wt_c, int(wn is not None), int(wt is not None),
                                                     C.byref(tg), C.byref(td))
            t = tasks[k]
            t.w = master.value
            t.wn = wn.data_ptr() if wn is not None else None
            t.wt = wt.data_ptr() if wt is not None else None
            t.Cg, t.Cd, t.wn_rows, t.wn_cols, t.wt_rows, t.wt_cols = cg, cd, wn_r, wn_c, wt_r, wt_c
            t.tiles_g, t.tiles_d, t.first_block = tg.value, td.value, first
            first += nb
        raw = torch.frombuffer(bytearray(bytes(tasks)), dtype=torch.uint8).to(self.device)
        self._prep_table[part] = (raw, len(specs), first)
        return self._prep_table[part]

    def _adam_table(self, part):
        if part in self._adam_tables:
            return self._adam_tables[part]
        head_end = self.G.buckets[-1][0] if len(self.G.buckets) >= 2 else 0
        specs, n_elems = [], 0
        for (sid, name), lw in self.W.items():
            store = self._store(sid)
            in_head = sid == "G" and store.offsets[name + ".kernel"] + 16 * lw.cg * lw.cd <= head_end
            where = "D" if sid == "D" else ("G_head" if in_head else "G_rest")
            master = store.p(name + ".kernel")
            sets = []
            if lw.wt is not None or lw.wn is not None:
                sets.append((master, lw.cg, lw.cd, lw.wn, up32(lw.cg), lw.lo_pad, lw.wt, up32(lw.cd), lw.hi_pad))
            if lw.wd is not None:
                sets.append((master, lw.cg, lw.cd, lw.wd, lw.cg, lw.cd, None, 0, 0))
            if not sets:
                sets.append((master, lw.cg, lw.cd, None, 0, 0, None, 0, 0))
            if part == where:
                specs.append(sets[0])
                n_elems += 16 * lw.cg * lw.cd
            elif part == "extra":
                specs += sets[1:]
        if not specs:
            self._adam_tables[part] = (None, 0, 0, 0)
            return self._adam_tables[part]
        tasks = (L.PrepTask * len(specs))()
        first = 0
        for k, (master, cg, cd, wn, wn_r, wn_c, wt, wt_r, wt_c) in enumerate(specs):
            tg, td = C.c_int(0), C.c_int(0)
            nb = L.lib().p2p_weight_prep_task_blocks(cg, cd, wn_r, wn_c, wt_r, wt_c, int(wn is not None), int(wt is not None),
                                                     C.byref(tg), C.byref(td))
            t = tasks[k]
            t.w = master.value
            t.wn = wn.data_ptr() if wn is not None else None
            t.wt = wt.data_ptr() if wt is not None else None
            t.Cg, t.Cd, t.wn_rows, t.wn_cols, t.wt_rows, t.wt_cols = cg, cd, wn_r, wn_c, wt_r, wt_c
            t.tiles_g, t.tiles_d, t.first_block = tg.value, td.value, first
            first += nb
        raw = torch.frombuffer(bytearray(bytes(tasks)), dtype=torch.uint8).to(self.device)
        self._adam_tables[part] = (raw, len(specs), first, n_elems)
        return self._adam_tables[part]

    def _adam_prep(self, part):
        raw, ntasks, total, n_elems = self._adam_table(part)
        if not ntasks:
            return
        store = self.D if part == "D" else self.G
        L.call("p2p_adam_prep_batched", self.dtype, n_elems, _p(raw), ntasks, total, _p(store.params), _p(store.grads), _p(store.m),
               _p(store.v), _p(store.lr_t_dev), self._slot_b1, self._slot_b2, self._slot_eps, _stream())

    def refresh_weight_copies(self, part="all"):
        self._copies_version += 1
        raw, ntasks, total = self._prep_tasks(part)
        if ntasks:
            L.call("p2p_weight_prep_batched", self.dtype, _p(raw), ntasks, total, _stream())

    def _wn(self, sid, name):
        lw = self.W[(sid, name)]
        return _p(lw.wn) if lw.wn is not None else self._store(sid).p(name + ".kernel")

    def _wd(self, sid, name):
        lw = self.W[(sid, name)]
        return _p(lw.wd) if lw.wd is not None else self._store(sid).p(name + ".kernel")

    def set_params(self, g_values=None, d_values=None):
        if g_values is not None:
            self.G.load(g_values)
        if d_values is not None:
            self.D.load(d_values)
        self.refresh_weight_copies()

    def plan(self, B):
        if B in self.plans:
            return self.plans[B]
        P = {"B": B}
        self._alloc_generator(P, B)
        self._alloc_discriminator(P, 2 * B, B)
        self._alloc_workspaces(P, B)
        self.plans[B] = P
        return P

    def _alloc_generator(self, P, B):
        S, dt, dev, tdt = self.S, self.dtype, self.device, self.tdt
        skips = list(reversed(DOWN_FILTERS[:-1])) + [self.in_ch]
        P["c"] = [None]
        for k in range(1, 7):
            res = S // 64 * (2 ** k)
            ch = UP_FILTERS[k - 1] + skips[k - 1] if k < 6 else self.c6_ch
            P["c"].append(HaloBuf(B, res, res, ch, dt, dev))
        r6 = S // 64
        P["a6"] = HaloBuf(B, r6, r6, 512, dt, dev)
        P["src"] = HaloBuf(B, S, S, self.src_ch, dt, dev)
        P["rd"], P["ru"], P["sd"], P["su"], P["dd"], P["du"], P["mask"] = {}, {}, {}, {}, {}, {}, {}
        for i, f in enumerate(DOWN_FILTERS, start=1):
            res = S // (2 ** i)
            if i > 1 or not self.use_mfma:
                P["rd"][i] = DenseBuf(B, res, res, f, tdt, dev)
            P["dd"][i] = HaloBuf(B, res, res, f, dt, dev)
            if i > 1:
                P["sd"][i] = torch.empty((B, f, 2), dtype=torch.float32, device=dev)
        for i, f in enumerate(UP_FILTERS, start=1):
            res = S // 64 * (2 ** i)
            P["ru"][i] = DenseBuf(B, res, res, f, tdt, dev)
            P["du"][i] = HaloBuf(B, res, res, f, dt, dev)
            P["su"][i] = torch.empty((B, f, 2), dtype=torch.float32, device=dev)
            if UP_DROPOUT[i - 1]:
                P["mask"][i] = torch.empty((B * res * res, f), dtype=torch.uint8, device=dev)
        P["gc"] = [None] + [DenseBuf(B, P["c"][k].h, P["c"][k].w,
                                     UP_FILTERS[5] if (k == 6 and self.full_pixels and self.use_mfma) else P["c"][k].c, tdt, dev)
                            for k in range(1, 7)]
        P["ga"] = {i: DenseBuf(B, S // 2 ** i, S // 2 ** i, DOWN_FILTERS[i - 1], tdt, dev) for i in range(1, 7)}
        P["part_off"], tasks, off = {}, [], 0
        for name in [k[:-6] for k in self.G.shapes if k.endswith(".gamma")]:
            cch = self.G.shapes[name + ".gamma"][0]
            P["part_off"][name] = (off, off + B * cch)
            tasks.append([off, B, cch, self.G.offsets[name + ".beta"]])
            tasks.append([off + B * cch, B, cch, self.G.offsets[name + ".gamma"]])
            off += 2 * B * cch
        P["part"] = torch.empty(off, dtype=torch.float32, device=dev)
        P["part_tasks"] = torch.tensor(tasks, dtype=torch.int32, device=dev)
        P["part_maxc"] = max(t[2] for t in tasks)
        P["z"] = DenseBuf(B, S, S, self.out_ch, tdt, dev)
        P["dz"] = HaloBuf(B, S, S, self.dz_ch, dt, dev)

    def _alloc_discriminator(self, P, N, B=None):
        S, dt, dev, tdt = self.S, self.dtype, self.device, self.tdt
        h2 = S // 2
        P["dcat"] = HaloBuf(N, S, S, self.dcat_ch, dt, dev)
        P["d_act"] = HaloBuf(N, h2, h2, 64, dt, dev)
        P["logits"] = DenseBuf(N, h2, h2, 1, tdt, dev)
        P["dld"] = HaloBuf(N, h2, h2, 8, dt, dev)
        if B is not None:
            P["dlg"] = HaloBuf(B, h2, h2, 8, dt, dev)
        P["g_dact"] = DenseBuf(N, h2, h2, 64, tdt, dev)
        P["d_draw"] = HaloBuf(N, h2, h2, 64, dt, dev)
        if B is not None:
            P["d_draw_g"] = HaloBuf(B, h2, h2, 64, dt, dev)
            P["g_dact_g"] = DenseBuf(B, h2, h2, 64, tdt, dev)
        P["g_dcat"] = DenseBuf(N if B is None else B, S, S, 4 if (self.in_ch == 4 and self.full_pixels) else self.dcat_ch, tdt, dev)
        if not self.use_mfma:
            P["d_raw"] = DenseBuf(N, h2, h2, 64, tdt, dev)

    def _alloc_workspaces(self, P, B):
        dev = self.device
        P["nws"] = torch.empty(max(B, 2) * 16 * 1024 * 2, dtype=torch.float32, device=dev)
        P["spart"] = torch.empty(4 * 1024 * 1024, dtype=torch.float32, device=dev)
        P["slabs"] = torch.empty(self._max_slab_elems(B), dtype=torch.float32, device=dev)
        P["wws"] = torch.empty(self._max_wgrad_ws(B) // 4 + 4, dtype=torch.float32, device=dev)

    def _splitk(self, op, B, lh, cg, cd):
        if self.batch_invariant:
            B = 256
        ntaps = 16 if op == L.OP_G else 4
        if lh == 1:
            ntaps = 4 if op == L.OP_G else 1
        ncols = cd if op == L.OP_G else cg
        cc = cg if op == L.OP_G else cd
        esz = 2 if self.dtype == L.BF16 else 4
        bn = 128 if ncols % 128 == 0 else (64 if ncols % 64 == 0 else 32)
        blocks = ((B * lh * lh + 127) // 128) * (ncols // bn) * (1 if op == L.OP_G else 4)
        target = self.splitk_target or (64 if B <= 16 else (128 if B <= 32 else 256))
        sk = 1
        while blocks * sk < target and sk * 2 <= ntaps and ((ntaps // (sk * 2)) * cc * esz) % 128 == 0:
            sk *= 2
        return sk

    def _msplit(self, B, lh, cg, cd):
        bg = 128 if cg > 64 else (64 if cg > 32 else 32)
        bd = 128 if cd > 64 else (64 if cd > 32 else 32)
        nw = (bg // 32) * (bd // 32)
        nw = 4 if nw >= 4 else nw
        tiles = 16 * ((cg + bg - 1) // bg) * ((cd + bd - 1) // bd)
        want = self.wgemm_want if nw == 4 else 4096 // nw
        if self.dtype == L.BF16 and cg % 128 == 0 and cd % 128 == 0 and self.wgemm_pipe and tiles <= 448:
            want = self.wgemm_want_pipe
        min_chunk = 256 if nw == 4 else 1024
        m = B * lh * lh
        ms = 1
        while tiles * ms < want and m // (ms * 2) >= min_chunk:
            ms *= 2
        return ms

    def _s2_layers(self):
        out = []
        for i in range(2, 7):
            out.append((DOWN_FILTERS[i - 2], DOWN_FILTERS[i - 1], self.S // 2 ** i))
        cin = 512
        skips = list(reversed(DOWN_FILTERS[:-1])) + [self.in_ch]
        for i in range(1, 7):
            out.append((UP_FILTERS[i - 1], cin, self.S // 64 * 2 ** (i - 1)))
            cin = UP_FILTERS[i - 1] + skips[i - 1]
        return out

    def _max_slab_elems(self, B):
        best = 4
        for cg, cd, lh in self._s2_layers():
            best = max(best, self._splitk(L.OP_G, B, lh, cg, cd) * B * lh * lh * cd)
            best = max(best, self._splitk(L.OP_P, B, lh, cg, cd) * B * 4 * lh * lh * cg)
        return best

    def _max_wgrad_ws(self, B):
        S, best = self.S, 16
        layers = self._s2_layers() + [(self.in_ch, 64, S // 2), (self.c6_ch - (self.c6_ch - 32 - self.in_ch), self.out_ch, S)]
        for cg, cd, lh in layers:
            best = max(best, self._msplit(B, lh, cg, cd) * 16 * cg * cd * 4)
        for cg, cd, lh in ((2 * self.in_ch, 64, S // 2), (64, 1, S // 2)):
            best = max(best, self._msplit(2 * B, lh, cg, cd) * 16 * cg * cd * 4)
        return max(best, (68 << 20) + 16)

    def _conv(self, P, op, sid, name, N, lh, in_view, out_view, stride=2, ncols=None, bias=None, act=L.ACT_NONE,
              tmp=None, want_stats=False, slab_key=None, w_p=None):
        lw = self.W[(sid, name)]
        cg, cd = lw.cg, lw.cd
        hi, lo = (in_view, out_view) if op == L.OP_G else (out_view, in_view)
        if self.use_mfma and lw.main and stride == 2 and bias is None and act == L.ACT_NONE and ncols is None:
            w = _p(lw.wt) if op == L.OP_G else self._wn(sid, name)
            if self.use_conv_strip and L.lib().p2p_conv_strip_ok(op, self.dtype, N, lh, lh, cg, cd):
                slots = L.lib().p2p_conv_strip_stat_slots(op, self.dtype, N, lh, lh, cg, cd) if (want_stats and not self.batch_invariant) else 0
                if N * slots * cg * 2 > P["spart"].numel():
                    slots = 0
                L.call("p2p_conv_strip", op, self.dtype, N, lh, lh, cg, cd, C.byref(hi), C.byref(lo), w,
                       _p(P["spart"]) if slots else NULL, _stream())
                return (1, 1, slots) if slots else (1, 1)
            sk = self._splitk(op, N, lh, cg, cd)
            slots = 0
            if want_stats and sk == 1 and not self.batch_invariant:
                slots = L.lib().p2p_igemm_layer_stat_slots(op, self.dtype, N, lh, lh, cg, cd)
                if N * slots * (cd if op == L.OP_G else cg) * 2 > P["spart"].numel():
                    slots = 0
            slabs = P["slabs"]
            if sk > 1 and slab_key is not None:
                need = sk * N * (lh * lh * cd if op == L.OP_G else 4 * lh * lh * cg)
                slabs = P.setdefault("own_slabs", {}).get(slab_key)
                if slabs is None or slabs.numel() < need:
                    slabs = P["own_slabs"][slab_key] = torch.empty(need, dtype=torch.float32, device=self.device)
            L.call("p2p_igemm", op, self.dtype, N, lh, lh, cg, cd, C.byref(hi), C.byref(lo), w, sk,
                   _p(slabs) if sk > 1 else NULL, _p(P["spart"]) if slots else NULL, _stream())
            if slots:
                return (1, 1, slots)
            if sk == 1:
                return (1, 1)
            return (2, sk, slabs) if slab_key is not None else (2, sk)
        if self.use_mfma:
            if op == L.OP_G:
                cin_pad, nc, rows, w = lw.hi_pad, cd, up32(cd), _p(lw.wt)
            else:
                cin_pad, nc, rows, w = lw.lo_pad, (ncols or cg), up32(cg), w_p or self._wn(sid, name)
            if self.use_conv_fewout and L.lib().p2p_conv_fewout_ok(op, stride, self.dtype, N, lh, lh, cin_pad, nc):
                entry = "p2p_conv_fewout"
            elif self.use_conv_fewin and L.lib().p2p_conv_fewin_ok(op, stride, self.dtype, N, lh, lh, cin_pad, nc):
                entry = "p2p_conv_fewin"
            else:
                entry = "p2p_igemm_edge"
            L.call(entry, op, stride, self.dtype, N, lh, lh, cin_pad, nc, rows, C.byref(in_view),
                   C.byref(out_view), w, bias if bias is not None else NULL, act, LEAKY_ALPHA, _stream())
            return (1, 1)
        if act != L.ACT_NONE:
            L.call("p2p_conv_direct", op, stride, self.dtype, N, lh, lh, cg, cd, C.byref(hi), C.byref(tmp.view()),
                   self._wd(sid, name), bias if bias is not None else NULL, NULL, NULL, _stream())
            L.call("p2p_norm_act_fwd", self.dtype, N, lh, lh, cd, tmp.ptr(), 1, 1, 0, NULL, NULL, IN_EPS, act,
                   LEAKY_ALPHA, NULL, C.byref(out_view), NULL, NULL, NULL, 0, 1, _stream())
        else:
            L.call("p2p_conv_direct", op, stride, self.dtype, N, lh, lh, cg, cd, C.byref(hi), C.byref(lo),
                   self._wd(sid, name), bias if bias is not None else NULL, NULL, NULL, _stream())
        return (1, 1)

    def _fused_block(self, P, op, name, N, lh, in_view, raw_buf, act, out_view, stats):
        lw = self.W[("G", name)]
        if not (self.use_mfma and lw.main and L.lib().p2p_igemm_norm_act_ok(op, self.dtype, N, lh, lh, lw.cg, lw.cd)):
            return False
        hi, lo = (in_view, raw_buf.view()) if op == L.OP_G else (raw_buf.view(), in_view)
        w = _p(lw.wt) if op == L.OP_G else self._wn("G", name)
        L.call("p2p_igemm_norm_act", op, self.dtype, N, lh, lh, lw.cg, lw.cd, C.byref(hi), C.byref(lo), w,
               self.G.p(name + ".gamma"), self.G.p(name + ".beta"), IN_EPS, act, LEAKY_ALPHA, C.byref(out_view), _p(stats), _stream())
        return True

    def _c6_tail(self, P):
        key = ("c6_tail", self.full_pixels)
        if key not in P:
            lw, S = self.W[("G", "up6")], self.S
            fused = (not UP_DROPOUT[5]) and self.use_mfma and lw.main and \
                bool(L.lib().p2p_igemm_norm_act_ok(L.OP_P, self.dtype, P["B"], S // 2, S // 2, lw.cg, lw.cd))
            P[key] = bool(self.full_pixels and not fused and self.src_ch == 8 and P["c"][6].c == UP_FILTERS[5] + 8
                                and UP_FILTERS[5] % 8 == 0 and S * S > 16)
        return P[key]

    def _wgrad(self, P, sid, name, N, lh, hi, lo, stride=2, dbias=None):
        self.side.fork()
        with self.side.run():
            self._wgrad_impl(P, sid, name, N, lh, hi, lo, stride, dbias)
            dp = self._dp
            if dp is None and sid == "G" and self.side.enabled and len(self.G.buckets) >= 2 \
                    and self.G.bucket_last_layer[len(self.G.buckets) - 2] == name:
                self._adam_head_ev = _record_event()
            if dp is not None and sid == "G":
                b = self.G.bucket_of[name]
                if self.G.bucket_last_layer[b] == name and b != len(self.G.buckets) - 1:
                    lo_e, hi_e = self.G.buckets[b]
                    dp.allreduce_async(self.G.grads[lo_e:hi_e])

    def _wgrad_impl(self, P, sid, name, N, lh, hi, lo, stride=2, dbias=None):
        lw = self.W[(sid, name)]
        cg, cd = lw.cg, lw.cd
        dw = self._store(sid).g(name + ".kernel")
        if not self.use_mfma:
            L.call("p2p_conv_direct", L.OP_W, stride, self.dtype, N, lh, lh, cg, cd, C.byref(hi), C.byref(lo),
                   NULL, NULL, dw, dbias if dbias is not None else NULL, _stream())
            return
        if lh >= 16:
            nb = L.lib().p2p_wgrad_small_blocks(self.dtype, stride, N, lh, lh, cg, cd, hi.ld, lo.ld)
            if nb > 0 and nb * 16 * cg * cd <= P["wws"].numel():
                L.call("p2p_wgrad_small", self.dtype, stride, N, lh, lh, cg, cd, C.byref(hi), C.byref(lo), dw, _p(P["wws"]), _stream())
                if dbias is not None:
                    self._colsum(P, N, lh, cd, lo, dbias)
                return
        ms = self._msplit(N, lh, cg, cd)
        ws = _p(P["wws"]) if ms > 1 else NULL
        if lw.main and stride == 2:
            L.call("p2p_wgemm", self.dtype, N, lh, lh, cg, cd, C.byref(hi), C.byref(lo), dw, ms, ws, _stream())
        else:
            L.call("p2p_wgemm_edge", self.dtype, stride, N, lh, lh, cg, cd, C.byref(hi), C.byref(lo), dw, ms, ws, _stream())
        if dbias is not None:
            self._colsum(P, N, lh, cd, lo, dbias)

    def _colsum(self, P, N, lh, cd, lo, dbias):
        need = L.lib().p2p_view_colsum_workspace_bytes(self.dtype, N, lh, lh, cd, C.byref(lo)) // 4
        key = ("cs_ws", cd)
        ws = P.get(key)
        if ws is None or ws.numel() < need:
            ws = P[key] = torch.empty(max(need, 16), dtype=torch.float32, device=self.device)
        L.call("p2p_view_colsum", self.dtype, N, lh, lh, cd, C.byref(lo), dbias, _p(ws), _stream())

    def _nsplit(self, N, res, c, bwd=False):
        if not bwd:
            return 0x101 if self.batch_invariant else 1
        if self.batch_invariant:
            N = 256
        groups = max(1, c // 64)
        sp = 1
        while N * groups * sp < 1024 and res * res // (sp * 2) >= 64 and sp < 16:
            sp *= 2
        return sp | 0x100 if self.batch_invariant else sp

    def _norm_fwd(self, P, N, res, c, raw_buf, rk, gamma, beta, act, mask, out_view, stats, tail=None):
        raw_kind, nslabs = rk[0], rk[1]
        raw = raw_buf.ptr() if raw_kind == 1 else _p(P["slabs"])
        slab = N * res * res * c
        entry, extra = "p2p_norm_act_fwd", ()
        if tail is not None:
            entry, extra = "p2p_norm_act_fwd_tail", (C.byref(tail), self.src_ch)
        if len(rk) == 3:
            L.call(entry, self.dtype, N, res, res, c, raw, 1, 1, 0, gamma, beta, IN_EPS, act, LEAKY_ALPHA,
                   _p(mask) if mask is not None else NULL, C.byref(out_view), NULL, _p(stats),
                   _p(P["spart"]), P["spart"].numel() * 4, -rk[2], *extra, _stream())
            return
        L.call(entry, self.dtype, N, res, res, c, raw, raw_kind, nslabs, slab,
               gamma if gamma is not None else NULL, beta if beta is not None else NULL, IN_EPS, act, LEAKY_ALPHA,
               _p(mask) if mask is not None else NULL, C.byref(out_view),
               raw_buf.ptr() if raw_kind == 2 else NULL, _p(stats) if stats is not None else NULL,
               _p(P["nws"]), P["nws"].numel() * 4, self._nsplit(N, res, c), *extra, _stream())

    def _gs(self, P, buf, rk, coff=0):
        if rk[0] == 1:
            return buf.gsrc(coff=coff, kind=1)
        slabs = rk[2] if len(rk) == 3 else P["slabs"]
        return L.GSrc(slabs.data_ptr(), 2, rk[1], buf.n * buf.h * buf.w * buf.c, buf.c, coff)

    def _norm_bwd(self, P, name, N, res, c, raw_buf, stats, act, mask, g1, g2, draw_view):
        ob, og = P["part_off"][name]
        self.side.prefork()
        L.call("p2p_norm_act_bwd", self.dtype, N, res, res, c, raw_buf.ptr(), _p(stats), self.G.p(name + ".gamma"),
               self.G.p(name + ".beta"), act, LEAKY_ALPHA, _p(mask) if mask is not None else NULL, C.byref(g1),
               C.byref(g2) if g2 is not None else None, C.byref(draw_view), _p(P["part"], og), _p(P["part"], ob),
               _p(P["nws"]), P["nws"].numel() * 4, self._nsplit(N, res, c, bwd=True), _stream())

    def _act_bwd(self, N, res, c, act_view, g1, g2, draw_view, fork_follows=False):
        if fork_follows:
            self.side.prefork()
        L.call("p2p_act_bwd", self.dtype, N, res, res, c, C.byref(act_view), C.byref(g1),
               C.byref(g2) if g2 is not None else None, LEAKY_ALPHA, C.byref(draw_view), _stream())

    def _to_device(self, arr, c, B, is_int=False):
        t = torch.as_tensor(arr)
        t = t.to(device=self.device, dtype=torch.int32 if is_int else torch.float32).contiguous()
        if tuple(t.shape) != (B, self.S, self.S, c):
            raise ValueError(f"expected batch of shape {(B, self.S, self.S, c)}, got {tuple(t.shape)}")
        return t

    def _pack(self, P, t, view, c, ptr=None):
        is_int = t.dtype == torch.int32
        L.call("p2p_pack_input", self.dtype, P["B"], self.S, self.S, c, ptr or _p(t), 1 if is_int else 0, C.byref(view), _stream())

    def _pack_multi(self, P, t, views, c, ptr=None):
        arr = (L.Tensor * len(views))(*views)
        L.call("p2p_pack_input_multi", self.dtype, P["B"], self.S, self.S, c, ptr or _p(t), 1 if t.dtype == torch.int32 else 0,
               arr, len(views), _stream())

    REPLAY_CACHE = 8

    def _replay_key(self, kind, B, masks, dp, apply_update, *extra):
        if (masks is not None or not apply_update or B > self.replay_max_batch or self.device.type != "cuda"
                or L.call is not _ORIG_CALL or not self.replay_enabled or torch.cuda.is_current_stream_capturing()):
            return None
        st = torch.cuda.current_stream()
        return (kind, B, self.side.enabled, self.side.stop_event_forks, self.side_hist.enabled, self.fuse_adam, self.use_head_fused, self.hist_fwd3, self.hist_bwd3,
                self.hist_points, self.fuse_act_bwd, self.split_prep, self.full_pixels, self.use_conv_fewout, self.use_conv_strip, self.use_conv_fewin,
                self.use_mfma, bool(self.batch_invariant), bool(self.wgemm_pipe), int(self.splitk_target), int(self.wgemm_want), int(self.wgemm_want_pipe),
                int(st.cuda_stream), int(st.stream_id),
                None if dp is None else id(dp)) + extra

    def _bind_batch(self, src_t, real_t):
        self._slot_src.value, self._slot_real.value = src_t.data_ptr(), real_t.data_ptr()
        S = self.S
        self._real_view.ptr, self._real_view.img_stride, self._real_view.row_stride, self._real_view.ld = real_t.data_ptr(), S * S, S, 4
        self._keep_alive = (src_t, real_t)

    def _new_out(self):
        out = torch.empty(8, dtype=torch.float32, device=self.device)
        self._slot_out.value = out.data_ptr()
        return out

    def _begin_record(self, key):
        if key is None:
            return False
        n = self._replay_seen.get(key, 0)
        if n == 0 and len(self._replay_seen) >= 8 * self.REPLAY_CACHE:
            self._replay_seen.clear()
        self._replay_seen[key] = n + 1
        if n < 1:
            return False
        _REC[0] = []
        L.call = _rec_call
        return True

    def _end_record(self, key, ok):
        rec, _REC[0] = _REC[0], None
        L.call = _ORIG_CALL
        if ok:
            segs, run = [], []
            for name, args in rec:
                if name is None:
                    if run:
                        segs.append(pack_replay(run))
                        run = []
                    segs.append(args)
                else:
                    run.append((name, args))
            if run:
                segs.append(pack_replay(run))
            self._replays[key] = (segs, rec)
            while len(self._replays) > self.REPLAY_CACHE:
                old, _ = self._replays.popitem(last=False)
                self._replay_seen.pop(old, None)

    def _replay(self, key, P, src_t, real_t, hist=False):
        segs, _ = self._replays[key]
        self._replays.move_to_end(key)
        self._bind_batch(src_t, real_t)
        out = self._new_out()
        for seg in segs:
            if callable(seg):
                seg()
            elif self._replay_fn(seg[0], seg[1]) != 0:
                raise L.P2PError(L.lib().p2p_last_error().decode())
        self._dp = None
        self.G.t += 1
        self.D.t += 1
        self.step_count += 1
        if hist:
            P["h_real_src"] = real_t
        return out[:7]

    def _pack_source(self, P, src_t, with_disc=False):
        ic, B = self.in_ch, P["B"]
        views = [P["src"].view()]
        if not self._c6_tail(P):
            views.append(P["c"][6].view(coff=UP_FILTERS[5]))
        if with_disc:
            views += [P["dcat"].view(coff=ic), P["dcat"].view(coff=ic, n0=B)]
        self._pack_multi(P, src_t, views, ic, ptr=self._slot_src if src_t.data_ptr() == self._slot_src.value else None)

    def _early_side(self, P, masks, apply_update):
        self.side.fork()
        with self.side.run():
            if masks is None:
                for i, drop in enumerate(UP_DROPOUT, start=1):
                    if drop:
                        m = P["mask"][i]
                        L.call("p2p_dropout_mask_dev", _p(m), m.numel(), self._slot_seed, _p(self.mask_counter_dev), i,
                               self._batch_offset * (m.numel() // P["B"]), _stream())
            if apply_update:
                L.call("p2p_counter_add", _p(self.mask_counter_dev), 1, _stream())
                for store in (self.G, self.D):
                    L.call("p2p_adam_tick", _p(store.t_dev), _p(store.lr_t_dev), self._slot_lr, self._slot_b1, self._slot_b2, _stream())
                self._ticked = True
            P["early_masks"] = masks is None
            P["early_ev"] = None
            if self.side.enabled:
                P["early_ev"] = _record_event()

    def generator_forward(self, P, masks=None, head=True):
        B, S = P["B"], self.S
        c = P["c"]
        P["rk_d"], P["rk_u"] = {}, {}
        src_view = P["src"].view()
        for i, f in enumerate(DOWN_FILTERS, start=1):
            res = S // 2 ** i
            out_view = P["a6"].view() if i == 6 else c[6 - i].view(coff=UP_FILTERS[5 - i])
            if i == 1:
                self._conv(P, L.OP_G, "G", "down1", B, res, src_view, out_view, act=L.ACT_LEAKY, tmp=P["rd"].get(1))
            elif self._fused_block(P, L.OP_G, f"down{i}", B, res, src_view, P["rd"][i], L.ACT_LEAKY, out_view, P["sd"][i]):
                pass
            else:
                rk = self._conv(P, L.OP_G, "G", f"down{i}", B, res, src_view, P["rd"][i].view(), want_stats=True)
                self._norm_fwd(P, B, res, f, P["rd"][i], rk, self.G.p(f"down{i}.gamma"), self.G.p(f"down{i}.beta"),
                               L.ACT_LEAKY, None, out_view, P["sd"][i])
            src_view = out_view
        lo_view = P["a6"].view()
        for i, f in enumerate(UP_FILTERS, start=1):
            lh = S // 64 * 2 ** (i - 1)
            if not UP_DROPOUT[i - 1] and self._fused_block(P, L.OP_P, f"up{i}", B, lh, lo_view, P["ru"][i], L.ACT_RELU,
                                                           c[i].view(coff=0), P["su"][i]):
                lo_view = c[i].view()
                continue
            rk = self._conv(P, L.OP_P, "G", f"up{i}", B, lh, lo_view, P["ru"][i].view(), want_stats=True)
            mask = None
            if UP_DROPOUT[i - 1]:
                mask = P["mask"][i]
                if masks is not None:
                    mask.copy_(torch.as_tensor(masks[i - 1]).reshape(mask.shape).to(torch.uint8))
                elif P.get("early_masks"):
                    if P.get("early_ev") is not None:
                        _wait_event(P["early_ev"])
                        P["early_ev"] = None
                else:
                    L.call("p2p_dropout_mask_dev", _p(mask), mask.numel(), self._slot_seed, _p(self.mask_counter_dev), i,
                           self._batch_offset * (mask.numel() // B), _stream())
            self._norm_fwd(P, B, 2 * lh, f, P["ru"][i], rk, self.G.p(f"up{i}.gamma"), self.G.p(f"up{i}.beta"),
                           L.ACT_RELU, mask, c[i].view(coff=0), P["su"][i],
                           tail=P["src"].view() if i == 6 and self._c6_tail(P) else None)
            lo_view = c[i].view()
        if head:
            self._conv(P, L.OP_G, "G", "last", B, S, c[6].view(), P["z"].view(), stride=1, bias=self.G.p("last.bias"))
        P["early_masks"] = False

    def discriminator_forward(self, P, N2):
        h2 = self.S // 2
        self._conv(P, L.OP_G, "D", "down", N2, h2, P["dcat"].view(), P["d_act"].view(), act=L.ACT_LEAKY, tmp=P.get("d_raw"))
        self._conv(P, L.OP_G, "D", "last", N2, h2, P["d_act"].view(), P["logits"].view(), stride=1, bias=self.D.p("last.bias"))

    def discriminator_backward(self, P, B):
        S, ic, h2 = self.S, self.in_ch, self.S // 2
        self._wgrad(P, "D", "last", 2 * B, h2, P["d_act"].view(), P["dld"].view(), stride=1, dbias=self.D.g("last.bias"))
        if not self._d_last_dgrad_gated(2 * B, h2, P["dld"].view(), P["d_act"].view(), P["d_draw"].view()):
            self._conv(P, L.OP_P, "D", "last", 2 * B, h2, P["dld"].view(), P["g_dact"].view(), stride=1)
            self._act_bwd(2 * B, h2, 64, P["d_act"].view(), P["g_dact"].gsrc(), None, P["d_draw"].view(), fork_follows=True)
        self._wgrad(P, "D", "down", 2 * B, h2, P["dcat"].view(), P["d_draw"].view())
        if P.get("skip_g_through_d"):
            return
        if not self._d_last_dgrad_gated(B, h2, P["dlg"].view(), P["d_act"].view(n0=B), P["d_draw_g"].view()):
            self._conv(P, L.OP_P, "D", "last", B, h2, P["dlg"].view(), P["g_dact_g"].view(), stride=1)
            self._act_bwd(B, h2, 64, P["d_act"].view(n0=B), P["g_dact_g"].gsrc(), None, P["d_draw_g"].view())
        self._conv(P, L.OP_P, "D", "down", B, h2, P["d_draw_g"].view(), P["g_dcat"].view(), ncols=ic)

    def _d_last_dgrad_gated(self, N, h2, dlogits_view, act_view, out_view):
        lw = self.W[("D", "last")]
        if not (self.use_mfma and self.use_conv_fewin and self.fuse_act_bwd and
                L.lib().p2p_conv_fewin_ok(L.OP_P, 1, self.dtype, N, h2, h2, lw.lo_pad, lw.cg)):
            return False
        L.call("p2p_conv_fewin_actbwd", L.OP_P, 1, self.dtype, N, h2, h2, lw.lo_pad, lw.cg, up32(lw.cg), C.byref(dlogits_view),
               C.byref(out_view), self._wn("D", "last"), C.byref(act_view), LEAKY_ALPHA, _stream())
        return True

    def train_step_rgba(self, source, real, lambda_l1, lambda_hist=None, masks=None, global_batch=None,
                        apply_update=True, dp=None, batch_offset=0):
        B = int(source.shape[0])
        P = self.plan(B)
        S, ic = self.S, self.in_ch
        Bg = global_batch or B
        self._dp = dp
        self._batch_offset = int(batch_offset)
        src_t, real_t = self._to_device(source, ic, B), self._to_device(real, ic, B)
        key = self._replay_key("rgba", B, masks, dp, apply_update, float(lambda_l1),
                               None if lambda_hist is None else float(lambda_hist), Bg, int(batch_offset))
        if key in self._replays:
            return self._replay(key, P, src_t, real_t, hist=lambda_hist is not None)
        recording = self._begin_record(key)
        if recording and dp is not None:
            dp = self._dp = _RecDP(dp)
        try:
            out = self._train_step_rgba_body(P, B, Bg, src_t, real_t, lambda_l1, lambda_hist, masks, apply_update, dp)
        except BaseException:
            if recording:
                self._end_record(key, False)
            raise
        if recording:
            self._end_record(key, True)
        return out

    def _train_step_rgba_body(self, P, B, Bg, src_t, real_t, lambda_l1, lambda_hist, masks, apply_update, dp):
        S, ic = self.S, self.in_ch
        self._bind_batch(src_t, real_t)
        whole_fake = ic == 4 and self.src_ch == 8 and self.dcat_ch == 8 and self.full_pixels and self.out_ch == 4
        if ic == 4 and self.src_ch == 8 and self.dcat_ch == 8:
            L.call("p2p_pack_pair", self.dtype, B, S, S, self._slot_src, self._slot_real, C.byref(P["src"].view()),
                   None if self._c6_tail(P) else C.byref(P["c"][6].view(coff=UP_FILTERS[5])), C.byref(P["dcat"].view(coff=0)),
                   None if whole_fake else C.byref(P["dcat"].view(coff=0, n0=B)), _stream())
        else:
            self._pack_source(P, src_t, with_disc=True)
            self._pack(P, real_t, P["dcat"].view(coff=0), ic, ptr=self._slot_real)
        if lambda_hist is not None:
            self._hist_real_early(P, B, real_t)
        self._early_side(P, masks, apply_update)
        self.generator_forward(P, masks)
        real_view, fake_view = P["dcat"].view(coff=0), P["dcat"].view(coff=0, n0=B)
        inv_l1 = 1.0 / (Bg * S * S * self.out_ch)
        if lambda_hist is not None:
            self._hist_buffers(P, B)
        if whole_fake:
            L.call("p2p_tanh_l1_fwd_pair", self.dtype, B, S, S, C.byref(P["z"].view()), C.byref(real_view), C.byref(fake_view), inv_l1,
                   _p(self.loss_part, 3 * 256), _p(P["fake32"]) if lambda_hist is not None else NULL, _stream())
        else:
            L.call("p2p_tanh_l1_fwd", self.dtype, B, S, S, self.out_ch, C.byref(P["z"].view()), C.byref(real_view),
                   C.byref(fake_view), inv_l1, _p(self.loss_part, 3 * 256), _p(P["fake32"]) if lambda_hist is not None else NULL,
                   _stream())
        g_extra = None
        if lambda_hist is not None:
            self.side_hist.fork()
            with self.side_hist.run():
                g_extra = self._histogram_loss(P, B, Bg, lambda_hist, dp.allreduce_scalar_sum if dp is not None else None)
        self.discriminator_forward(P, 2 * B)
        h2 = S // 2
        inv_bce = 1.0 / (Bg * h2 * h2)
        L.call("p2p_bce_logits_pad8" if self.full_pixels else "p2p_bce_logits", self.dtype, 2 * B, B, h2, h2,
               C.byref(P["logits"].view()), inv_bce, C.byref(P["dld"].view()), C.byref(P["dlg"].view()), _p(self.loss_part), _stream())
        P["skip_g_through_d"] = False
        P["head_dbias_done"] = False
        self.discriminator_backward(P, B)
        if lambda_hist is not None:
            self.side_hist.join()
        if self.full_pixels and self.out_ch == 4 and self.dz_ch == 8:
            L.call("p2p_tanh_l1_bwd_pad8", self.dtype, B, S, S, C.byref(fake_view), C.byref(real_view),
                   C.byref(P["g_dcat"].gsrc()), C.byref(g_extra) if g_extra is not None else None,
                   float(lambda_l1) * inv_l1, C.byref(P["dz"].view()), _stream())
        else:
            L.call("p2p_tanh_l1_bwd", self.dtype, B, S, S, self.out_ch, C.byref(fake_view), C.byref(real_view),
                   C.byref(P["g_dcat"].gsrc()), C.byref(g_extra) if g_extra is not None else None,
                   float(lambda_l1) * inv_l1, C.byref(P["dz"].view()), _stream())
        self.generator_backward(P)
        return self._finish_step(P, lambda_l1, lambda_hist, apply_update)

    def train_step_rgba_hooked(self, source, real, generator_loss, discriminator_loss, masks=None, apply_update=True):
        B = int(source.shape[0])
        P = self.plan(B)
        S, ic, h2 = self.S, self.in_ch, self.S // 2
        assert self.head == "tanh", "the palette-index model has a train_step of its own"
        self._dp, self._batch_offset = None, 0
        src_t, real_t = self._to_device(source, ic, B), self._to_device(real, ic, B)
        self._bind_batch(src_t, real_t)
        self._pack_source(P, src_t, with_disc=True)
        self._pack(P, real_t, P["dcat"].view(coff=0), ic)
        self._early_side(P, masks, apply_update)
        self.generator_forward(P, masks)
        real_view, fake_view = P["dcat"].view(coff=0), P["dcat"].view(coff=0, n0=B)
        fake32 = P.get("fake32_hook")
        if fake32 is None:
            fake32 = P["fake32_hook"] = torch.empty(B * S * S * self.out_ch, dtype=torch.float32, device=self.device)
        L.call("p2p_tanh_l1_fwd", self.dtype, B, S, S, self.out_ch, C.byref(P["z"].view()), C.byref(real_view), C.byref(fake_view), 0.0,
               _p(self.loss_part, 4 * 256), _p(fake32), _stream())
        self.discriminator_forward(P, 2 * B)
        logits = P["logits"].t.detach().float().view(2 * B, h2, h2, 1)
        lg_d = logits.clone().requires_grad_(True)
        d_loss = discriminator_loss(lg_d[:B], lg_d[B:])
        d_loss[0].backward()
        lg_g = logits[B:].clone().requires_grad_(True)
        fake = fake32.view(B, S, S, self.out_ch).clone().requires_grad_(True)
        g_loss = generator_loss(lg_g, fake, real_t)
        g_loss[0].backward()
        zero = lambda t: torch.zeros_like(t) if t.grad is None else t.grad
        inner = slice(HALO, HALO + h2)
        P["dld"].t[:, inner, inner, 0] = zero(lg_d).view(2 * B, h2, h2).to(self.tdt)
        P["dlg"].t[:, inner, inner, 0] = zero(lg_g).view(B, h2, h2).to(self.tdt)
        d_fake = zero(fake).contiguous()
        P["hook_keep"] = (d_fake, lg_d, lg_g, fake)
        g_extra = L.GSrc(d_fake.data_ptr(), 2, 1, B * S * S * self.out_ch, self.out_ch, 0)
        P["skip_g_through_d"] = False
        P["head_dbias_done"] = False
        self.discriminator_backward(P, B)
        L.call("p2p_tanh_l1_bwd", self.dtype, B, S, S, self.out_ch, C.byref(fake_view), C.byref(real_view), C.byref(P["g_dcat"].gsrc()),
               C.byref(g_extra), 0.0, C.byref(P["dz"].view()), _stream())
        self.generator_backward(P)
        head = self._adam_head(apply_update)
        self.side.join()
        if apply_update:
            self.apply_adam(g_from=head)
        self.step_count += 1
        vals = [g_loss[0], g_loss[1], g_loss[2], g_loss[3] if len(g_loss) > 3 else torch.zeros((), device=self.device),
                d_loss[0], d_loss[1], d_loss[2]]
        return torch.stack([v.detach().reshape(()).float() for v in vals])

    def generator_backward(self, P):
        B, S = P["B"], self.S
        c, gc, ga = P["c"], P["gc"], P["ga"]
        dbias = None if P.get("head_dbias_done") else self.G.g("last.bias")
        self._wgrad(P, "G", "last", B, S, c[6].view(), P["dz"].view(), stride=1, dbias=dbias)
        lw = self.W[("G", "last")]
        if (self.use_mfma and self.use_head_fused and lw.wn is not None and
                L.lib().p2p_head_dgrad_ok(self.dtype, B, S, S, lw.cd, UP_FILTERS[5], up32(lw.cg), P["dz"].c, gc[6].c)):
            L.call("p2p_head_dgrad", self.dtype, B, S, S, lw.cd, UP_FILTERS[5], C.byref(P["dz"].view()), _p(lw.wn), up32(lw.cg),
                   C.byref(gc[6].view()), _stream())
        else:
            self._conv(P, L.OP_P, "G", "last", B, S, P["dz"].view(), gc[6].view(), stride=1, ncols=UP_FILTERS[5])
        rk_gc = {6: (1, 1)}
        for i in range(6, 0, -1):
            f = UP_FILTERS[i - 1]
            lh = S // 64 * 2 ** (i - 1)
            lo_buf = c[i - 1] if i > 1 else P["a6"]
            self._norm_bwd(P, f"up{i}", B, 2 * lh, f, P["ru"][i], P["su"][i], L.ACT_RELU, P["mask"].get(i),
                           self._gs(P, gc[i], rk_gc[i], 0), None, P["du"][i].view())
            self._wgrad(P, "G", f"up{i}", B, lh, P["du"][i].view(), lo_buf.view())
            out_buf = gc[i - 1] if i > 1 else ga[6]
            rk = self._conv(P, L.OP_G, "G", f"up{i}", B, lh, P["du"][i].view(), out_buf.view(), slab_key=f"up{i}.dgrad")
            if i > 1:
                rk_gc[i - 1] = rk
        g_from_down = self._gs(P, ga[6], rk, 0)
        for i in range(6, 0, -1):
            f = DOWN_FILTERS[i - 1]
            res = S // 2 ** i
            if i == 6:
                g1, g2 = g_from_down, None
            else:
                g1 = self._gs(P, gc[6 - i], rk_gc[6 - i], UP_FILTERS[5 - i])
                g2 = g_from_down
            if i > 1:
                self._norm_bwd(P, f"down{i}", B, res, f, P["rd"][i], P["sd"][i], L.ACT_LEAKY, None, g1, g2,
                               P["dd"][i].view())
                hi_view = c[7 - i].view(coff=UP_FILTERS[6 - i])
            else:
                self._act_bwd(B, res, f, c[5].view(coff=UP_FILTERS[4]), g1, g2, P["dd"][1].view(), fork_follows=True)
                hi_view = P["src"].view()
            self._wgrad(P, "G", f"down{i}", B, res, hi_view, P["dd"][i].view())
            if i > 1:
                rk = self._conv(P, L.OP_P, "G", f"down{i}", B, res, P["dd"][i].view(), ga[i - 1].view(),
                                slab_key=f"down{i}.dgrad")
                g_from_down = self._gs(P, ga[i - 1], rk, 0)
        self.side.fork()
        with self.side.run():
            L.call("p2p_colsum_batched", _p(P["part"]), _p(P["part_tasks"]), int(P["part_tasks"].shape[0]), P["part_maxc"],
                   _p(self.G.grads), _stream())

    def _reduce_tail(self):
        dp = self._dp
        if dp is None:
            return
        assert self.G.buckets[-1][1] == self.G.small_range[0]
        dp.allreduce_async(self._grad_all[self.G.buckets[-1][0]:])
        dp.wait_all()
        self._dp = None

    def _finish_step(self, P, lambda_l1, lambda_hist, apply_update):
        head = self._adam_head(apply_update)
        self.side.join()
        L.call("p2p_loss_partials_sum", _p(self.loss_part), 4, _p(self.losses), _stream())
        self._reduce_tail()
        if apply_update:
            self.apply_adam(g_from=head)
        out = self._new_out()
        L.call("p2p_finish_losses", _p(self.losses), 4 if lambda_hist is not None else -1, 3, float(lambda_l1),
               float(lambda_hist) if lambda_hist is not None else 0.0, self._slot_out, _stream())
        self.step_count += 1
        return out[:7]

    def train_step_empty(self, lambda_l1, lambda_hist=None, lambda_aux=None, dp=None, apply_update=True):
        self._dp = dp
        self._grad_all.zero_()
        if dp is not None:
            if lambda_hist is not None:
                if getattr(self, "_zero_scalar", None) is None:
                    self._zero_scalar = torch.zeros(1, dtype=torch.float32, device=self.device)
                self._zero_scalar.zero_()
                dp.allreduce_scalar_sum(self._zero_scalar)
            for lo_e, hi_e in self.G.buckets[:-1]:
                dp.allreduce_async(self.G.grads[lo_e:hi_e])
        self._reduce_tail()
        if apply_update:
            self.apply_adam()
        out = torch.empty(8, dtype=torch.float32, device=self.device)
        if self.head == "softmax":
            L.call("p2p_finish_losses", _p(self.losses), 5, 6, 0.0, float(lambda_aux or 0.0), _p(out), _stream())
        else:
            L.call("p2p_finish_losses", _p(self.losses), 4 if lambda_hist is not None else -1, 3, float(lambda_l1),
                   float(lambda_hist) if lambda_hist is not None else 0.0, _p(out), _stream())
        self.step_count += 1
        return out[:7]

    def _adam_head(self, apply_update):
        ev, self._adam_head_ev = self._adam_head_ev, None
        if not apply_update or not self._ticked or len(self.G.buckets) < 2:
            return 0
        if self._dp is not None:
            self._dp.wait_all()
        elif ev is not None:
            _wait_event(ev)
        else:
            return 0
        n = self.G.buckets[-1][0]
        if self.fuse_adam:
            self._adam_prep("G_head")
            self._head_prepped = True
            return n
        L.call("p2p_adam_flat_dev", _p(self.G.params), _p(self.G.grads), _p(self.G.m), _p(self.G.v), n,
               _p(self.G.lr_t_dev), self._slot_b1, self._slot_b2, self._slot_eps, 1.0, _stream())
        if self.split_prep:
            self.refresh_weight_copies("head")
            self._head_prepped = True
        return n

    def apply_adam(self, g_from=0):
        ticked, self._ticked = self._ticked, False
        if self.fuse_adam:
            for store in (self.G, self.D):
                store.t += 1
                if not ticked:
                    L.call("p2p_adam_tick", _p(store.t_dev), _p(store.lr_t_dev), self._slot_lr, self._slot_b1, self._slot_b2, _stream())
            if g_from == 0:
                self._adam_prep("G_head")
            self._adam_prep("G_rest")
            self._adam_prep("D")
            for store in (self.G, self.D):
                lo_e, hi_e = store.small_range
                if hi_e > lo_e:
                    L.call("p2p_adam_flat_dev", _p(store.params, lo_e), _p(store.grads, lo_e), _p(store.m, lo_e), _p(store.v, lo_e),
                           hi_e - lo_e, _p(store.lr_t_dev), self._slot_b1, self._slot_b2, self._slot_eps, 1.0, _stream())
            raw, ntasks, total, _ = self._adam_table("extra")
            if ntasks:
                L.call("p2p_weight_prep_batched", self.dtype, _p(raw), ntasks, total, _stream())
            if not ticked:
                L.call("p2p_counter_add", _p(self.mask_counter_dev), 1, _stream())
            self._head_prepped = False
            return
        for store in (self.G, self.D):
            store.t += 1
            if not ticked:
                L.call("p2p_adam_tick", _p(store.t_dev), _p(store.lr_t_dev), self._slot_lr, self._slot_b1, self._slot_b2, _stream())
            off = g_from if store is self.G else 0
            L.call("p2p_adam_flat_dev", _p(store.params, off), _p(store.grads, off), _p(store.m, off), _p(store.v, off),
                   store.numel - off, _p(store.lr_t_dev), self._slot_b1, self._slot_b2, self._slot_eps, 1.0, _stream())
        if not ticked:
            L.call("p2p_counter_add", _p(self.mask_counter_dev), 1, _stream())
        head_done, self._head_prepped = self._head_prepped and g_from > 0, False
        self.refresh_weight_copies("rest" if head_done else "all")

    def _histogram_loss(self, P, B, Bg, lambda_hist, hist_allreduce):
        S = self.S
        self._hist_buffers(P, B)
        fake_view = L.Tensor(P["fake32"].data_ptr(), S * S, S, 4)
        assert P.get("h_real_done"), "the real histogram is taken by _hist_real_early"
        P["h_real_done"] = False
        self._hist_fwd(P, B, fake_view, P["h_fake"], points=False)
        L.call("p2p_hellinger_fwd", _p(P["h_real"]), _p(P["h_fake"]), B, _p(P["h_tot"][0]), _p(P["h_tot"][1]),
               _p(P["h_sqp"]), _p(P["h_sq"]), _stream())
        if hist_allreduce is not None:
            hist_allreduce(P["h_sq"][:1])
        L.call("p2p_hellinger_finish", _p(P["h_sq"]), (1.0 / Bg) * (B / Bg), _p(self.losses, 4), _stream())
        coef = float(lambda_hist) / (2.0 * math.sqrt(2.0) * Bg)
        bwd3 = self.hist_fwd3 and self.hist_bwd3
        L.call("p2p_rgbuv_hist_hellinger_bwd3" if bwd3 else "p2p_rgbuv_hist_hellinger_bwd", L.F32, B, S, S, C.byref(fake_view),
               _p(P["h_real"]), _p(P["h_fake"]), _p(P["h_tot"][0]), _p(P["h_tot"][1]), _p(P["h_sq"]), coef, _p(P["h_gh"]),
               _p(P["h_dimg"]), _stream())
        return L.GSrc(P["h_dimg"].data_ptr(), 2, 1 if bwd3 else 3, B * S * S * 4, 4, 0)

    def _hist_buffers(self, P, B):
        if "h_real" in P:
            return
        dev, S = self.device, self.S
        P["h_real"] = torch.empty(B * 3 * 64 * 64, dtype=torch.float32, device=dev)
        P["h_fake"] = torch.empty(B * 3 * 64 * 64, dtype=torch.float32, device=dev)
        P["h_gh"] = torch.empty(B * 3 * 64 * 64, dtype=torch.float32, device=dev)
        P["h_tot"] = torch.empty((2, B), dtype=torch.float32, device=dev)
        P["h_sq"] = torch.zeros(4, dtype=torch.float32, device=dev)
        P["h_sqp"] = torch.zeros(B, dtype=torch.float32, device=dev)
        P["h_dimg"] = torch.empty(3 * B * S * S * 4, dtype=torch.float32, device=dev)
        P["h_ws"] = torch.empty(L.lib().p2p_rgbuv_hist_fwd3_workspace_bytes(B) // 4, dtype=torch.float32, device=dev)
        P["h_points"] = torch.empty((B, self.HIST_POINT_CAP, 4), dtype=torch.float32, device=dev)
        P["h_npoints"] = torch.zeros(B, dtype=torch.int32, device=dev)
        P["fake32"] = torch.empty(B * S * S * 4, dtype=torch.float32, device=dev)

    def _hist_real_early(self, P, B, real_t):
        self._hist_buffers(P, B)
        S = self.S
        P["h_real_src"] = real_t
        self.side_hist.fork()
        with self.side_hist.run():
            rv = self._real_view if real_t.data_ptr() == self._real_view.ptr else L.Tensor(real_t.data_ptr(), S * S, S, 4)
            self._hist_fwd(P, B, rv, P["h_real"], points=True)
        P["h_real_done"] = True

    HIST_POINT_CAP = 1024

    def _hist_fwd(self, P, B, view, out, points):
        S = self.S
        if not self.hist_fwd3:
            L.call("p2p_rgbuv_hist_fwd", L.F32, B, S, S, C.byref(view), _p(out), _stream())
            return
        pts = npts = NULL
        if points and self.hist_points:
            L.call("p2p_rgbuv_points", L.F32, B, S, S, C.byref(view), self.HIST_POINT_CAP, _p(P["h_points"]), _p(P["h_npoints"]), _stream())
            pts, npts = _p(P["h_points"]), _p(P["h_npoints"])
        L.call("p2p_rgbuv_hist_fwd3", L.F32, B, S, S, C.byref(view), pts, npts, self.HIST_POINT_CAP, _p(out), _p(P["h_ws"]), _stream())

    def rgbuv_histogram(self, image):
        B = int(image.shape[0])
        return _histogram.rgbuv_histogram(self._to_device(image, 4, B))

    def train_step_indexed(self, source_idx, real_idx, lambda_segmentation, masks=None, global_batch=None,
                           apply_update=True, dp=None, batch_offset=0):
        assert self.head == "softmax" and self.in_ch == 1
        B = int(source_idx.shape[0])
        P = self.plan(B)
        S = self.S
        Bg = global_batch or B
        self._dp = dp
        self._batch_offset = int(batch_offset)
        src_t = self._to_device(source_idx, 1, B, is_int=True)
        real_t = self._to_device(real_idx, 1, B, is_int=True)
        key = self._replay_key("indexed", B, masks, dp, apply_update, float(lambda_segmentation), Bg, int(batch_offset))
        if key in self._replays:
            return self._replay(key, P, src_t, real_t)
        recording = self._begin_record(key)
        if recording and dp is not None:
            self._dp = _RecDP(dp)
        try:
            out = self._train_step_indexed_body(P, B, Bg, src_t, real_t, lambda_segmentation, masks, apply_update)
        except BaseException:
            if recording:
                self._end_record(key, False)
            raise
        if recording:
            self._end_record(key, True)
        return out

    def _pack_indexed(self, P, B, src_t, real_t):
        S = self.S
        self._bind_batch(src_t, real_t)
        if self.full_pixels and self.in_ch == 1 and self.src_ch == 8 and self.dcat_ch == 8:
            L.call("p2p_pack_pair_idx", self.dtype, B, S, S, self._slot_src, self._slot_real, C.byref(P["src"].view()),
                   None if self._c6_tail(P) else C.byref(P["c"][6].view(coff=UP_FILTERS[5])), C.byref(P["dcat"].view(coff=0)),
                   C.byref(P["dcat"].view(coff=0, n0=B)), _stream())
        else:
            self._pack_source(P, src_t, with_disc=True)
            self._pack(P, real_t, P["dcat"].view(coff=0), 1, ptr=self._slot_real)

    def _train_step_indexed_body(self, P, B, Bg, src_t, real_t, lambda_segmentation, masks, apply_update):
        S = self.S
        self._pack_indexed(P, B, src_t, real_t)
        self._early_side(P, masks, apply_update)
        fused = (self.use_mfma and self.use_head_fused and
                 L.lib().p2p_head_softmax_ok(self.dtype, B, S, S, self.c6_ch, self.out_ch))
        self.generator_forward(P, masks, head=not fused)
        real_view, fake_view = P["dcat"].view(coff=0), P["dcat"].view(coff=0, n0=B)
        inv_pix = 1.0 / (Bg * S * S)
        P["head_dbias_done"] = fused
        if fused:
            if "head_ws" not in P:
                P["head_ws"] = torch.empty(L.lib().p2p_head_softmax_workspace_bytes(B, S) // 4 + 4, dtype=torch.float32, device=self.device)
            L.call("p2p_head_softmax_cce", self.dtype, B, S, S, self.c6_ch, self.out_ch, C.byref(P["c"][6].view()),
                   _p(self.W[("G", "last")].wt), self.G.p("last.bias"), C.byref(real_view), C.byref(fake_view),
                   float(lambda_segmentation) * inv_pix, inv_pix, C.byref(P["dz"].view()), self.G.g("last.bias"),
                   _p(P["head_ws"]), _p(self.losses, 5), _stream())
        else:
            L.call("p2p_softmax_cce_argmax", self.dtype, B, S, S, self.out_ch, C.byref(P["z"].view()), C.byref(real_view),
                   C.byref(fake_view), float(lambda_segmentation) * inv_pix, inv_pix, C.byref(P["dz"].view()), NULL,
                   _p(self._softmax_part()), _p(self.losses, 5), _stream())
        self.discriminator_forward(P, 2 * B)
        h2 = S // 2
        L.call("p2p_bce_logits_pad8" if self.full_pixels else "p2p_bce_logits", self.dtype, 2 * B, B, h2, h2,
               C.byref(P["logits"].view()), 1.0 / (Bg * h2 * h2), C.byref(P["dld"].view()), None, _p(self.loss_part), _stream())
        P["skip_g_through_d"] = True
        self.discriminator_backward(P, B)
        self.generator_backward(P)
        head = self._adam_head(apply_update)
        self.side.join()
        L.call("p2p_loss_partials_sum", _p(self.loss_part), 3, _p(self.losses), _stream())
        self._reduce_tail()
        if apply_update:
            self.apply_adam(g_from=head)
        out = self._new_out()
        L.call("p2p_finish_losses", _p(self.losses), 5, 6, 0.0, float(lambda_segmentation), self._slot_out, _stream())
        self.step_count += 1
        return out[:7]

    def train_step_indexed_hooked(self, source_idx, real_idx, generator_loss, discriminator_loss, masks=None, apply_update=True):
        assert self.head == "softmax" and self.in_ch == 1, "the RGBA models have train_step_rgba_hooked"
        B = int(source_idx.shape[0])
        P = self.plan(B)
        S, h2, Cn = self.S, self.S // 2, self.out_ch
        self._dp, self._batch_offset = None, 0
        src_t = self._to_device(source_idx, 1, B, is_int=True)
        real_t = self._to_device(real_idx, 1, B, is_int=True)
        self._pack_indexed(P, B, src_t, real_t)
        self._early_side(P, masks, apply_update)
        self.generator_forward(P, masks, head=True)
        real_view, fake_view = P["dcat"].view(coff=0), P["dcat"].view(coff=0, n0=B)
        bufs = P.get("hook_idx")
        if bufs is None:
            bufs = P["hook_idx"] = tuple(torch.empty((B, S, S, Cn), dtype=torch.float32, device=self.device) for _ in range(3))
        probs32, z32, onehot = bufs
        L.call("p2p_softmax_cce_argmax", self.dtype, B, S, S, Cn, C.byref(P["z"].view()), C.byref(real_view), C.byref(fake_view),
               0.0, 0.0, None, _p(probs32), _p(self._softmax_part()), _p(self.losses, 14), _stream())
        L.call("p2p_unpack", self.dtype, B, S, S, Cn, C.byref(P["z"].view()), _p(z32), _stream())
        onehot.zero_()
        onehot.view(-1, Cn).scatter_(1, real_t.view(-1, 1).long(), 1.0)
        self.discriminator_forward(P, 2 * B)
        logits = P["logits"].t.detach().float().view(2 * B, h2, h2, 1)
        lg_d = logits.clone().requires_grad_(True)
        d_loss = discriminator_loss(lg_d[:B], lg_d[B:])
        d_loss[0].backward()
        lg_g = logits[B:].clone().requires_grad_(True)
        probs = probs32.detach().requires_grad_(True)
        probs._keras_logits = z32.detach().requires_grad_(True)
        g_loss = generator_loss(lg_g, probs, onehot)
        g_loss[0].backward()
        grad = lambda t: None if t.grad is None else t.grad.contiguous()
        gp, gz = grad(probs), grad(probs._keras_logits)
        inner = slice(HALO, HALO + h2)
        P["dld"].t[:, inner, inner, 0] = (torch.zeros_like(lg_d) if lg_d.grad is None else lg_d.grad).view(2 * B, h2, h2).to(self.tdt)
        P["hook_keep"] = (gp, gz, lg_d, lg_g, probs)
        L.call("p2p_softmax_bwd", self.dtype, B, S, S, Cn, _p(probs32), NULL if gp is None else _p(gp), NULL if gz is None else _p(gz),
               1.0, C.byref(P["dz"].view()), _stream())
        P["skip_g_through_d"] = True
        P["head_dbias_done"] = False
        self.discriminator_backward(P, B)
        self.generator_backward(P)
        head = self._adam_head(apply_update)
        self.side.join()
        if apply_update:
            self.apply_adam(g_from=head)
        self.step_count += 1
        vals = [g_loss[0], g_loss[1], g_loss[2], g_loss[3] if len(g_loss) > 3 else torch.zeros((), device=self.device),
                d_loss[0], d_loss[1], d_loss[2]]
        return torch.stack([v.detach().reshape(()).float() for v in vals])

    def _softmax_part(self):
        if getattr(self, "_sm_part", None) is None:
            self._sm_part = torch.zeros(2 * 8192, dtype=torch.float32, device=self.device)
        return self._sm_part

    def discriminate(self, target, source):
        B = int(target.shape[0])
        P = self.plan(B)
        S, ic, h2 = self.S, self.in_ch, self.S // 2
        is_int = self.head == "softmax"
        self._pack(P, self._to_device(target, ic, B, is_int), P["dcat"].view(coff=0), ic)
        self._pack(P, self._to_device(source, ic, B, is_int), P["dcat"].view(coff=ic), ic)
        self.discriminator_forward(P, B)
        out = torch.empty((B, h2, h2, 1), dtype=torch.float32, device=self.device)
        L.call("p2p_unpack", self.dtype, B, h2, h2, 1, C.byref(P["logits"].view()), _p(out), _stream())
        return out

    def generate_indexed(self, source_idx, masks=None, with_probs=False):
        assert self.head == "softmax"
        B = int(source_idx.shape[0])
        P = self.plan(B)
        S = self.S
        src_t = self._to_device(source_idx, 1, B, is_int=True)
        self._batch_offset = 0
        self._pack_source(P, src_t)
        self.generator_forward(P, masks)
        fake_view = P["dcat"].view(coff=0, n0=B)
        probs = torch.empty((B, S, S, self.out_ch), dtype=torch.float32, device=self.device)
        L.call("p2p_softmax_cce_argmax", self.dtype, B, S, S, self.out_ch, C.byref(P["z"].view()), C.byref(fake_view),
               C.byref(fake_view), 0.0, 0.0, None, _p(probs), _p(self._softmax_part()), _p(self.losses, 14), _stream())
        idx = torch.empty((B * S * S,), dtype=torch.int32, device=self.device)
        L.call("p2p_argmax_lastdim", _p(probs), B * S * S, self.out_ch, _p(idx), _stream())
        idx = idx.view(B, S, S, 1)
        return (idx, probs) if with_probs else idx

    def graphed_rgba_step(self, B, lambda_l1, lambda_hist=None, global_batch=None):
        S, ic = self.S, self.in_ch
        self.replay_enabled = False
        src_s = torch.zeros((B, S, S, ic), dtype=torch.float32, device=self.device)
        real_s = torch.zeros((B, S, S, ic), dtype=torch.float32, device=self.device)
        snap = [(t, t.clone()) for st in (self.G, self.D) for t in (st.params, st.m, st.v, st.t_dev, st.lr_t_dev)]
        snap.append((self.mask_counter_dev, self.mask_counter_dev.clone()))
        t_host = (self.G.t, self.D.t)
        side = torch.cuda.Stream(device=self.device)
        side.wait_stream(torch.cuda.current_stream())
        with torch.cuda.stream(side):
            self.train_step_rgba(src_s, real_s, lambda_l1, lambda_hist, global_batch=global_batch)
        torch.cuda.current_stream().wait_stream(side)
        for t, c in snap:
            t.copy_(c)
        self.G.t, self.D.t = t_host
        self.refresh_weight_copies()
        torch.cuda.synchronize(self.device)
        graph = torch.cuda.CUDAGraph()
        with torch.cuda.graph(graph):
            out = self.train_step_rgba(src_s, real_s, lambda_l1, lambda_hist, global_batch=global_batch)
        self.G.t, self.D.t = t_host

        def step(source, real):
            src_s.copy_(torch.as_tensor(source), non_blocking=True)
            real_s.copy_(torch.as_tensor(real), non_blocking=True)
            graph.replay()
            self.G.t += 1
            self.D.t += 1
            self.step_count += 1
            return out

        step.graph = graph
        return step

    def generate(self, source, masks=None):
        if self.head != "tanh":
            raise NotImplementedError("use generate_indexed for the softmax head")
        B = int(source.shape[0])
        P = self.plan(B)
        S = self.S
        src_t = self._to_device(source, self.in_ch, B)
        self._batch_offset = 0
        self._pack_source(P, src_t)
        self.generator_forward(P, masks)
        fake_view = P["dcat"].view(coff=0, n0=B)
        L.call("p2p_tanh_l1_fwd", self.dtype, B, S, S, self.out_ch, C.byref(P["z"].view()), C.byref(fake_view),
               C.byref(fake_view), 0.0, _p(self.loss_part, 4 * 256), NULL, _stream())
        out = torch.empty((B, S, S, self.out_ch), dtype=torch.float32, device=self.device)
        L.call("p2p_unpack", self.dtype, B, S, S, self.out_ch, C.byref(fake_view), _p(out), _stream())
        return out

    def tape_arena(self, kind, N):
        pool = self._arena_pool.setdefault((kind, N), [])
        if pool:
            return pool.pop()
        P = {"B": N, "kind": kind}
        if kind == "G":
            self._alloc_generator(P, N)
            P["fake"] = DenseBuf(N, self.S, self.S, self.out_ch, self.tdt, self.device)
        else:
            self._alloc_discriminator(P, N)
        ws = self._tape_ws.get(N)
        if ws is None:
            ws = {}
            self._alloc_workspaces(ws, N)
            self._tape_ws[N] = ws
        P.update(ws)
        return P

    def release_tape_arena(self, P):
        self._arena_pool[(P["kind"], P["B"])].append(P)

    def free_tape_arenas(self):
        self._arena_pool.clear()
        self._tape_ws.clear()

    @staticmethod
    def arena_bytes(P):
        seen, total = set(), 0

        def add(t):
            nonlocal total
            if isinstance(t, (HaloBuf, DenseBuf)):
                t = t._flat if isinstance(t, HaloBuf) else t.t
            if isinstance(t, torch.Tensor) and t.data_ptr() not in seen:
                seen.add(t.data_ptr())
                total += t.numel() * t.element_size()
            elif isinstance(t, (list, tuple)):
                for x in t:
                    add(x)
            elif isinstance(t, dict):
                for x in t.values():
                    add(x)
        add({k: v for k, v in P.items() if k not in ("nws", "spart", "slabs", "wws")})
        return total

    def tape_generator_forward(self, P, source, masks=None):
        B, S = P["B"], self.S
        src_t = self._to_device(source, self.in_ch, B)
        self._dp, self._batch_offset = None, 0
        self._pack_source(P, src_t)
        P["early_masks"] = False
        self.generator_forward(P, masks)
        L.call("p2p_counter_add", _p(self.mask_counter_dev), 1, _stream())
        out = torch.empty((B, S, S, self.out_ch), dtype=torch.float32, device=self.device)
        fake = P["fake"].view()
        L.call("p2p_tanh_l1_fwd", self.dtype, B, S, S, self.out_ch, C.byref(P["z"].view()), C.byref(fake), C.byref(fake), 0.0,
               _p(self.loss_part, 4 * 256), _p(out), _stream())
        return out

    def _gradient_f32(self, g, shape):
        g = g.detach().to(device=self.device, dtype=torch.float32).reshape(shape).contiguous()
        return g if g.data_ptr() % 16 == 0 else g.clone()

    def _down1_copy(self):
        key = (self.G.t, self._copies_version)
        lw = self.W[("G", "down1")]
        if self._down1_wn is None:
            self._down1_wn = torch.zeros(16 * up32(lw.cg) * lw.lo_pad, dtype=self.tdt, device=self.device)
        if self._down1_wn_key != key:
            L.call("p2p_weight_prep_pad", self.dtype, self.G.p("down1.kernel"), lw.cg, lw.cd, _p(self._down1_wn), up32(lw.cg),
                   lw.lo_pad, None, 0, 0, _stream())
            self._down1_wn_key = key
        return _p(self._down1_wn)

    def tape_generator_backward(self, P, d_image, need_source_grad):
        B, S, ic = P["B"], self.S, self.in_ch
        g = self._gradient_f32(d_image, (B, S, S, self.out_ch))
        gx = L.GSrc(g.data_ptr(), 2, 1, B * S * S * self.out_ch, self.out_ch, 0)
        fake = P["fake"].view()
        if self.full_pixels and self.out_ch == 4 and self.dz_ch == 8:
            L.call("p2p_tanh_l1_bwd_pad8", self.dtype, B, S, S, C.byref(fake), C.byref(fake), None, C.byref(gx), 0.0,
                   C.byref(P["dz"].view()), _stream())
        else:
            L.call("p2p_tanh_l1_bwd", self.dtype, B, S, S, self.out_ch, C.byref(fake), C.byref(fake), None, C.byref(gx), 0.0,
                   C.byref(P["dz"].view()), _stream())
        P["head_dbias_done"] = False
        self.generator_backward(P)
        d_src = None
        if need_source_grad:
            buf = P.get("g_src")
            if buf is None:
                buf = P["g_src"] = DenseBuf(B, S, S, 4 if (ic == 4 and self.full_pixels) else self.src_ch, self.tdt, self.device)
            self._conv(P, L.OP_P, "G", "down1", B, S // 2, P["dd"][1].view(), buf.view(), ncols=ic,
                       w_p=self._down1_copy() if self.use_mfma else None)
            skip = P.get("g_c6")
            if skip is None:
                skip = P["g_c6"] = DenseBuf(B, S, S, self.c6_ch, self.tdt, self.device)
            self._conv(P, L.OP_P, "G", "last", B, S, P["dz"].view(), skip.view(), stride=1, ncols=UP_FILTERS[5] + ic)
            d_src = torch.empty((B, S, S, ic), dtype=torch.float32, device=self.device)
            d_skip = torch.empty((B, S, S, ic), dtype=torch.float32, device=self.device)
            L.call("p2p_unpack", self.dtype, B, S, S, ic, C.byref(buf.view()), _p(d_src), _stream())
            L.call("p2p_unpack", self.dtype, B, S, S, ic, C.byref(skip.view(coff=UP_FILTERS[5])), _p(d_skip), _stream())
            L.call("p2p_grad_accumulate", _p(d_src), _p(d_skip), d_src.numel(), 0, _stream())
        self.side.join()
        self._adam_head_ev = None
        P["keep"] = g
        return d_src

    def tape_discriminator_forward(self, P, first, second):
        N, S, ic, h2 = P["B"], self.S, self.in_ch, self.S // 2
        self._pack(P, self._to_device(first, ic, N), P["dcat"].view(coff=0), ic)
        self._pack(P, self._to_device(second, ic, N), P["dcat"].view(coff=ic), ic)
        self.discriminator_forward(P, N)
        out = torch.empty((N, h2, h2, 1), dtype=torch.float32, device=self.device)
        L.call("p2p_unpack", self.dtype, N, h2, h2, 1, C.byref(P["logits"].view()), _p(out), _stream())
        return out

    def tape_discriminator_backward(self, P, d_logits, weights, need_first, need_second):
        N, S, ic, h2 = P["B"], self.S, self.in_ch, self.S // 2
        g = self._gradient_f32(d_logits, (N, h2, h2, 1))
        L.call("p2p_pack_input", self.dtype, N, h2, h2, 1, _p(g), 0, C.byref(P["dld"].view()), _stream())
        dld, d_act, d_draw = P["dld"].view(), P["d_act"].view(), P["d_draw"].view()
        if weights:
            self._wgrad(P, "D", "last", N, h2, d_act, dld, stride=1, dbias=self.D.g("last.bias"))
        if not self._d_last_dgrad_gated(N, h2, dld, d_act, d_draw):
            self._conv(P, L.OP_P, "D", "last", N, h2, dld, P["g_dact"].view(), stride=1)
            self._act_bwd(N, h2, 64, d_act, P["g_dact"].gsrc(), None, d_draw, fork_follows=weights)
        if weights:
            self._wgrad(P, "D", "down", N, h2, P["dcat"].view(), d_draw)
        outs = [None, None]
        if need_first or need_second:
            nc = 2 * ic if need_second else ic
            buf = P["g_dcat"]
            if buf.c < nc:
                buf = P.get("g_dcat2")
                if buf is None:
                    buf = P["g_dcat2"] = DenseBuf(N, S, S, self.dcat_ch, self.tdt, self.device)
            self._conv(P, L.OP_P, "D", "down", N, h2, d_draw, buf.view(), ncols=nc)
            for k, want in enumerate((need_first, need_second)):
                if want:
                    outs[k] = torch.empty((N, S, S, ic), dtype=torch.float32, device=self.device)
                    L.call("p2p_unpack", self.dtype, N, S, S, ic, C.byref(buf.view(coff=k * ic)), _p(outs[k]), _stream())
        self.side.join()
        P["keep"] = g
        return outs

    def tape_collect(self, sid, dst, first):
        store = self._store(sid)
        L.call("p2p_grad_accumulate", _p(dst), _p(store.grads), store.numel, int(bool(first)), _stream())

    def apply_adam_store(self, store, grads):
        store.t += 1
        L.call("p2p_adam_tick", _p(store.t_dev), _p(store.lr_t_dev), self._slot_lr, self._slot_b1, self._slot_b2, _stream())
        L.call("p2p_adam_flat_dev", _p(store.params), _p(grads), _p(store.m), _p(store.v), store.numel, _p(store.lr_t_dev),
               self._slot_b1, self._slot_b2, self._slot_eps, 1.0, _stream())
        self.refresh_weight_copies("G" if store is self.G else "D")
```

### palette_and_histo_gan_amd/flops.py

```python
from .engine import DOWN_FILTERS, UP_FILTERS

__all__ = ["layer_macs", "train_step_flops_per_image", "call_work", "entry_roofline", "roofline_for_dominant", "rooflines_top"]


def layer_macs(S, in_ch, out_ch):
    macs = {}
    c = in_ch
    for i, f in enumerate(DOWN_FILTERS, start=1):
        res = S // 2 ** i
        macs[f"down{i}"] = res * res * 16 * c * f
        c = f
    skips = list(reversed(DOWN_FILTERS[:-1])) + [in_ch]
    for i, (f, s) in enumerate(zip(UP_FILTERS, skips), start=1):
        lh = S // 64 * 2 ** (i - 1)
        macs[f"up{i}"] = lh * lh * 16 * c * f
        c = f + s
    macs["last"] = S * S * 16 * c * out_ch
    macs["D.down"] = (S // 2) ** 2 * 16 * (2 * in_ch) * 64
    macs["D.last"] = (S // 2) ** 2 * 16 * 64
    return macs


def train_step_flops_per_image(S, in_ch=4, out_ch=4, indexed=False):
    m = layer_macs(S, in_ch, out_ch)
    g_fwd = sum(v for k, v in m.items() if not k.startswith("D."))
    if indexed:
        total = 3 * g_fwd - m["down1"] + 4 * m["D.down"] + 6 * m["D.last"]
    else:
        total = 3 * g_fwd - m["down1"] + 5 * m["D.down"] + 7 * m["D.last"]
    return 2 * total


HBM_PEAK_GBS = 8000.0
MFMA_PEAK_TFLOPS = {"bf16": 2500.0, "f32": 157.3}


def _ints(args, n):
    return [int(a) for a in args[:n]]


def _null(a):
    return a is None or (hasattr(a, "value") and not a.value)


def _view_ld(byref_obj, default):
    t = getattr(byref_obj, "_obj", None)
    return int(getattr(t, "ld", default)) if t is not None else default


def _gsrc_bytes(byref_obj, elems, esz):
    g = getattr(byref_obj, "_obj", None)
    if g is None:
        return 0.0
    return elems * (esz if int(g.kind) == 1 else 4 * int(g.nslabs))


def call_work(name, args, dtype):
    esz = 2 if dtype == "bf16" else 4
    mf = dtype
    if name in ("p2p_igemm", "p2p_igemm_norm_act", "p2p_conv_strip"):
        _, _, n, lh, lw, cg, cd = _ints(args, 7)
        fl = 2.0 * n * lh * lw * 16 * cg * cd
        by = (n * 4 * lh * lw * cg + n * lh * lw * cd + 16 * cg * cd) * esz
        if name == "p2p_igemm_norm_act":
            by += n * (lh * lw * cd if args[0] == 0 else 4 * lh * lw * cg) * esz
        return {"flops": fl, "mfma": mf, "bytes": by}
    if name in ("p2p_igemm_edge", "p2p_conv_fewin", "p2p_conv_fewout", "p2p_conv_fewin_actbwd"):
        op, stride, _, n, lh, lw, cin, nc = _ints(args, 8)
        fl = 2.0 * n * lh * lw * 16 * cin * nc
        hi_px, lo_px = n * stride * stride * lh * lw, n * lh * lw
        in_px, out_px = (hi_px, lo_px) if op == 0 else (lo_px, hi_px)
        by = (in_px * cin + out_px * nc + 16 * cin * nc) * esz
        if name == "p2p_conv_fewin_actbwd":
            by += out_px * nc * esz
        return {"flops": fl, "mfma": mf, "bytes": by}
    if name in ("p2p_wgemm", "p2p_wgemm_edge", "p2p_wgrad_small"):
        if name == "p2p_wgemm":
            _, n, lh, lw, cg, cd = _ints(args, 6)
            stride, hi_i = 2, 6
        else:
            a = _ints(args, 7)
            stride = a[1]
            n, lh, lw, cg, cd = a[2:7]
            hi_i = 7
        fl = 2.0 * n * lh * lw * 16 * cg * cd
        hi_ld, lo_ld = _view_ld(args[hi_i], cg), _view_ld(args[hi_i + 1], cd)
        by = (n * stride * stride * lh * lw * min(hi_ld, max(cg, 8)) + n * lh * lw * min(lo_ld, max(cd, 8))) * esz + 16 * cg * cd * 4
        return {"flops": fl, "mfma": mf, "bytes": by}
    if name == "p2p_conv_direct":
        _, _, _, n, lh, lw, cg, cd = _ints(args, 8)
        return {"flops": 2.0 * n * lh * lw * 16 * cg * cd, "mfma": None, "bytes": 0.0}
    if name in ("p2p_norm_act_fwd", "p2p_norm_act_fwd_tail"):
        _, n, h, w, c = _ints(args, 5)
        raw_kind, nslabs = int(args[6]), int(args[7])
        t = n * h * w * c
        by = t * (esz if raw_kind == 1 else 4 * nslabs) + t * esz
        if raw_kind == 2:
            by += t * esz
        if name == "p2p_norm_act_fwd_tail":
            by += 2.0 * n * h * w * int(args[22]) * esz
        return {"flops": 0.0, "mfma": None, "bytes": by}
    if name == "p2p_norm_act_bwd":
        _, n, h, w, c = _ints(args, 5)
        t = n * h * w * c
        by = t * esz + _gsrc_bytes(args[12], t, esz) + (_gsrc_bytes(args[13], t, esz) if args[13] is not None else 0) + t * esz
        return {"flops": 0.0, "mfma": None, "bytes": by}
    if name == "p2p_act_bwd":
        _, n, h, w, c = _ints(args, 5)
        t = n * h * w * c
        by = 2 * t * esz + _gsrc_bytes(args[6], t, esz) + (_gsrc_bytes(args[7], t, esz) if args[7] is not None else 0)
        return {"flops": 0.0, "mfma": None, "bytes": by}
    if name == "p2p_rgbuv_hist_fwd":
        _, n, h, w = _ints(args, 4)
        return {"flops": 3 * 2.0 * 64 * 64 * h * w * n, "mfma": "f32", "bytes": n * (h * w * 4 + 3 * 64 * 64) * 4.0}
    if name == "p2p_rgbuv_hist_fwd3":
        _, n, h, w = _ints(args, 4)
        listed = getattr(args[5], "value", None) not in (None, 0)
        by = n * (h * w * 4 + 3 * 64 * 64) * 4.0
        if listed:
            return {"flops": 0.0, "mfma": None, "bytes": by}
        alg = 3 * 2.0 * 64 * 64 * h * w * n
        return {"flops": alg, "executed_flops": 6 * alg, "mfma": "bf16", "bytes": by}
    if name == "p2p_rgbuv_points":
        _, n, h, w = _ints(args, 4)
        return {"flops": 0.0, "mfma": None, "bytes": n * h * w * 4 * 4.0}
    if name == "p2p_rgbuv_hist_hellinger_bwd3":
        _, n, h, w = _ints(args, 4)
        alg = 2 * 3 * 2.0 * 64 * 64 * h * w * n
        return {"flops": alg, "executed_flops": 6 * alg, "mfma": "bf16", "bytes": n * (h * w * 4 + 3 * 3 * 64 * 64 + h * w * 4) * 4.0}
    if name == "p2p_rgbuv_hist_hellinger_bwd":
        _, n, h, w = _ints(args, 4)
        return {"flops": 2 * 3 * 2.0 * 64 * 64 * h * w * n, "mfma": "f32",
                "bytes": n * (h * w * 4 + 3 * 3 * 64 * 64 + 3 * h * w * 4) * 4.0}
    if name == "p2p_head_softmax_cce":
        _, n, h, w, cin, ncls = _ints(args, 6)
        return {"flops": 2.0 * n * h * w * 16 * cin * ncls, "mfma": mf,
                "bytes": n * h * w * (cin + ncls + 16.0) * esz + 16 * cin * ncls * esz}
    if name == "p2p_head_dgrad":
        _, n, h, w, ncls, cout = _ints(args, 6)
        return {"flops": 2.0 * n * h * w * 16 * ncls * cout, "mfma": mf, "bytes": n * h * w * (ncls + cout) * esz + 16.0 * ncls * cout * esz}
    if name == "p2p_softmax_cce_argmax":
        _, n, h, w, c = _ints(args, 5)
        return {"flops": 0.0, "mfma": None, "bytes": n * h * w * (2.0 * c * esz + 2 * 8 * esz)}
    if name == "p2p_adam_flat_dev":
        return {"flops": 0.0, "mfma": None, "bytes": 7 * 4.0 * int(args[4])}
    if name == "p2p_adam_prep_batched":
        return {"flops": 0.0, "mfma": None, "bytes": (7 * 4.0 + 2 * esz) * int(args[1])}
    if name == "p2p_pack_pair":
        _, n, h, w = _ints(args, 4)
        ch = 8 + 8 + (0 if _null(args[7]) else 8) + (0 if _null(args[9]) else 4)
        return {"flops": 0.0, "mfma": None, "bytes": n * h * w * (2 * 4 * 4.0 + ch * esz)}
    if name == "p2p_pack_pair_idx":
        _, n, h, w = _ints(args, 4)
        return {"flops": 0.0, "mfma": None, "bytes": n * h * w * (2 * 4.0 + (24 + (0 if _null(args[7]) else 8)) * esz)}
    if name == "p2p_tanh_l1_fwd_pair":
        _, n, h, w = _ints(args, 4)
        return {"flops": 0.0, "mfma": None, "bytes": n * h * w * ((4 + 8 + 8) * esz + (0.0 if _null(args[9]) else 16.0))}
    if name == "p2p_tanh_l1_bwd_pad8":
        _, n, h, w = _ints(args, 4)
        return {"flops": 0.0, "mfma": None, "bytes": n * h * w * 3.0 * 8 * esz}
    if name in ("p2p_tanh_l1_fwd", "p2p_tanh_l1_bwd"):
        _, n, h, w, c = _ints(args, 5)
        return {"flops": 0.0, "mfma": None, "bytes": n * h * w * 3.0 * max(c, 8) * esz}
    if name == "p2p_dropout_mask_dev":
        return {"flops": 0.0, "mfma": None, "bytes": float(int(args[1]))}
    return None


def _call_flops(name, args, dtype="bf16"):
    w = call_work(name, args, dtype)
    return w["flops"] if w and w["mfma"] else None


def entry_roofline(name, records, dtype):
    cls = {"mfma": [0.0, 0.0, 0.0, 0, None], "hbm": [0.0, 0.0, 0.0, 0, None]}
    fl_all = ex_all = by_all = ms_all = 0.0
    n = 0
    for rname, args, a, b in records:
        if rname != name:
            continue
        w = call_work(rname, args, dtype)
        if w is None:
            continue
        ms = a.elapsed_time(b)
        t_mfma = w.get("executed_flops", w["flops"]) / (MFMA_PEAK_TFLOPS[w["mfma"]] * 1e12) if w["mfma"] else 0.0
        t_hbm = w["bytes"] / (HBM_PEAK_GBS * 1e9)
        c = cls["mfma"] if (t_mfma >= t_hbm and w["mfma"]) else cls["hbm"]
        c[0] += w["flops"] if c is cls["mfma"] else w["bytes"]
        c[1] += max(t_mfma, t_hbm)
        c[2] += ms
        c[3] += 1
        c[4] = c[4] or w["mfma"]
        fl_all += w["flops"] if w["mfma"] else 0.0
        ex_all += w.get("executed_flops", w["flops"]) if w["mfma"] else 0.0
        by_all += w["bytes"]
        ms_all += ms
        n += 1
    if n == 0 or ms_all <= 0:
        return None
    bound = "mfma" if cls["mfma"][2] >= cls["hbm"][2] else "hbm"
    work, tb, ms, k, pipe = cls[bound]
    out = {"kernel": name, "launches": n, "avg_launch_ms": round(ms_all / n, 5), "flops_per_launch_avg": fl_all / n,
           "algorithmic_bytes_per_launch_avg": by_all / n, "traffic": None,
           "frac_all": round((cls["mfma"][1] + cls["hbm"][1]) / (ms_all * 1e-3), 5), "launches_in_bound_class": k}
    if bound == "mfma":
        ach = fl_all / (ms_all * 1e-3) / 1e12
        ach_c = work / (ms * 1e-3) / 1e12
        out.update({"bound": "mfma", "mfma_dtype": pipe, "achieved": round(ach, 3), "peak": MFMA_PEAK_TFLOPS[pipe],
                    "unit": "TFLOP/s", "frac": round(ach / MFMA_PEAK_TFLOPS[pipe], 5),
                    "frac_bound_class": round(ach_c / MFMA_PEAK_TFLOPS[pipe], 5)})
        if ex_all > fl_all:
            out["frac_executed"] = round(ex_all / (ms_all * 1e-3) / 1e12 / MFMA_PEAK_TFLOPS[pipe], 5)
    else:
        ach = by_all / (ms_all * 1e-3) / 1e9
        ach_c = work / (ms * 1e-3) / 1e9
        out.update({"bound": "hbm", "achieved": round(ach, 1), "peak": HBM_PEAK_GBS, "unit": "GB/s",
                    "frac": round(ach / HBM_PEAK_GBS, 5), "frac_bound_class": round(ach_c / HBM_PEAK_GBS, 5)})
    return out


def roofline_for_dominant(prof, records, B, S, dtype, peak_tflops=None):
    for name, _ in sorted(prof.items(), key=lambda kv: -kv[1]["ms_per_step"]):
        r = entry_roofline(name, records, dtype)
        if r is not None:
            return r
    return {"kernel": None, "bound": "hbm", "achieved": None, "peak": HBM_PEAK_GBS, "unit": "GB/s", "frac": None, "traffic": None}


def rooflines_top(prof, records, dtype, k=8):
    out = []
    for name, v in sorted(prof.items(), key=lambda kv: -kv[1]["ms_per_step"]):
        r = entry_roofline(name, records, dtype)
        if r is not None:
            r["ms_per_step"] = round(v["ms_per_step"], 4)
            for key in ("traffic", "flops_per_launch_avg", "algorithmic_bytes_per_launch_avg"):
                r.pop(key, None)
            out.append(r)
        if len(out) >= k:
            break
    return out


def write_detail(records, path, n_steps, dtype="bf16"):
    agg, work = {}, {}
    for name, args, a, b in records:
        ints = tuple(x for x in args[:8] if isinstance(x, int))
        key = (name, ints)
        if key not in work:
            work[key] = call_work(name, args, dtype)
        d = agg.setdefault(key, [0.0, 0])
        d[0] += a.elapsed_time(b)
        d[1] += 1
    rows = sorted(agg.items(), key=lambda kv: -kv[1][0])
    with open(path, "w") as f:
        f.write("ms_per_step  launches  ms_each  TFLOP/s     GB/s  entry  int-args\n")
        for (name, ints), (ms, n) in rows:
            w = work.get((name, ints))
            tf = (w["flops"] * n / (ms * 1e-3) / 1e12) if w and w["mfma"] else 0.0
            gbs = (w["bytes"] * n / (ms * 1e-3) / 1e9) if w else 0.0
            f.write(f"{ms / n_steps:10.4f} {n / n_steps:8.1f} {ms / n:9.4f} {tf:8.1f} {gbs:8.0f}  {name} {ints}\n")
```

Measured before the change: 134,300.

## Elide dead 1x1 bottleneck layer and skip its frozen kernel in Adam

At 64x64 input the deepest down block reaches 1x1 spatial size. Instance norm there turns its output into beta alone, so the conv feeding it has no effect and its kernel gets zero gradient. The change drops that conv's forward and weight-gradient work and replaces the norm forward and backward with small 1x1 kernels. It also adds an Adam variant that skips the frozen kernel's parameter range, cutting a large share of optimizer memory traffic. This depends on the exact semantics holding: Adam with a zero gradient would still decay m and v and move the weights, so leaving them frozen differs unless they were already zero. A runtime check (_frozen_ok / _elision) appears to guard that condition.

```diff
diff --git a/include/p2pgan.h b/include/p2pgan.h
--- a/include/p2pgan.h
+++ b/include/p2pgan.h
@@ -105,6 +105,12 @@
                      const p2p_tensor* draw, float* dgamma_part, float* dbeta_part,
                      float* ws, long long ws_bytes, int nsplit, void* stream);
 
+int p2p_norm_act_fwd_1x1(int dtype, int N, int C, const float* gamma, const float* beta, int act, float alpha,
+                         const unsigned char* mask, const p2p_tensor* out, void* stream);
+int p2p_norm_act_bwd_1x1(int dtype, int N, int C, const float* gamma, const float* beta, int act, float alpha,
+                         const unsigned char* mask, const p2p_gsrc* g1, const p2p_gsrc* g2, float* dgamma_part,
+                         float* dbeta_part, void* stream);
+
 int p2p_act_bwd(int dtype, int N, int H, int W, int C, const p2p_tensor* act_out, const p2p_gsrc* g1,
                 const p2p_gsrc* g2, float alpha, const p2p_tensor* draw, void* stream);
 
@@ -202,6 +208,8 @@
 int p2p_adam_tick(int* t_dev, float* lr_t_dev, float lr, float beta1, float beta2, void* stream);
 int p2p_adam_flat_dev(float* p, const float* g, float* m, float* v, long long n, const float* lr_t_dev,
                       float beta1, float beta2, float eps, float gscale, void* stream);
+int p2p_adam_flat_dev_excl(float* p, const float* g, float* m, float* v, long long n, long long ex_lo, long long ex_hi,
+                           const float* lr_t_dev, float beta1, float beta2, float eps, float gscale, void* stream);
 int p2p_counter_add(long long* counter_dev, long long inc, void* stream);
 int p2p_grad_accumulate(float* dst, const float* src, long long n, int first, void* stream);
 
diff --git a/palette_and_histo_gan_amd/_lib.py b/palette_and_histo_gan_amd/_lib.py
--- a/palette_and_histo_gan_amd/_lib.py
+++ b/palette_and_histo_gan_amd/_lib.py
@@ -40,6 +40,8 @@
     "p2p_norm_act_fwd": [_i, _i, _i, _i, _i, _vp, _i, _i, _ll, _vp, _vp, _f, _i, _f, _vp, _TP, _vp, _vp, _vp, _ll, _i, _vp],
     "p2p_norm_act_fwd_tail": [_i, _i, _i, _i, _i, _vp, _i, _i, _ll, _vp, _vp, _f, _i, _f, _vp, _TP, _vp, _vp, _vp, _ll, _i, _TP, _i, _vp],
     "p2p_norm_act_bwd": [_i, _i, _i, _i, _i, _vp, _vp, _vp, _vp, _i, _f, _vp, _GP, _GP, _TP, _vp, _vp, _vp, _ll, _i, _vp],
+    "p2p_norm_act_fwd_1x1": [_i, _i, _i, _vp, _vp, _i, _f, _vp, _TP, _vp],
+    "p2p_norm_act_bwd_1x1": [_i, _i, _i, _vp, _vp, _i, _f, _vp, _GP, _GP, _vp, _vp, _vp],
     "p2p_colsum": [_vp, _i, _i, _f, _vp, _vp],
     "p2p_colsum_batched": [_vp, _vp, _i, _i, _vp, _vp],
     "p2p_bce_logits": [_i, _i, _i, _i, _i, _TP, _f, _TP, _TP, _vp, _vp],
@@ -52,6 +54,7 @@
     "p2p_adam_flat": [_vp, _vp, _vp, _vp, _ll, _i, _f, _f, _f, _f, _f, _vp],
     "p2p_adam_tick": [_vp, _vp, _f, _f, _f, _vp],
     "p2p_adam_flat_dev": [_vp, _vp, _vp, _vp, _ll, _vp, _f, _f, _f, _f, _vp],
+    "p2p_adam_flat_dev_excl": [_vp, _vp, _vp, _vp, _ll, _ll, _ll, _vp, _f, _f, _f, _f, _vp],
     "p2p_counter_add": [_vp, _ll, _vp],
     "p2p_grad_accumulate": [_vp, _vp, _ll, _i, _vp],
     "p2p_dropout_mask_dev": [_vp, _ll, _ll, _vp, _ll, _ll, _vp],
diff --git a/palette_and_histo_gan_amd/csrc/norm_act.hip b/palette_and_histo_gan_amd/csrc/norm_act.hip
--- a/palette_and_histo_gan_amd/csrc/norm_act.hip
+++ b/palette_and_histo_gan_amd/csrc/norm_act.hip
@@ -1203,6 +1203,95 @@
     return p2p_check_launch("p2p_norm_act_bwd");
 }
 
+template <typename T>
+__global__ __launch_bounds__(256) void norm_act_fwd_1x1_kernel(int C, long long items, const float* __restrict__ gamma,
+                                                               const float* __restrict__ beta, int act, float alpha,
+                                                               const unsigned char* __restrict__ mask, TView out) {
+    constexpr int VN = VecOf<T>::N;
+    const long long item = (long long)blockIdx.x * 256 + threadIdx.x;
+    if (item >= items) return;
+    const int cvn = C / VN;
+    const int n = (int)(item / cvn), c = (int)(item - (long long)n * cvn) * VN;
+    float keep[VN], y[VN];
+    if (mask) mask_vload8(mask + (long long)n * C + c, keep, VN);
+#pragma unroll
+    for (int k = 0; k < VN; ++k) {
+        float v = 0.f * gamma[c + k] + beta[c + k];
+        if (mask) v *= keep[k];
+        if (act == P2P_ACT_LEAKY) v = v > 0.f ? v : alpha * v;
+        else if (act == P2P_ACT_RELU) v = v > 0.f ? v : 0.f;
+        y[k] = v;
+    }
+    vstore<T>((T*)out.ptr + out.off(n, 0, 0) + c, y);
+}
+
+template <typename T, int SLABS>
+__global__ __launch_bounds__(256) void norm_act_bwd_1x1_kernel(int C, long long items, const float* __restrict__ gamma,
+                                                               const float* __restrict__ beta, int act, float alpha,
+                                                               const unsigned char* __restrict__ mask, GSrc g1, GSrc g2,
+                                                               float* __restrict__ dgamma_part, float* __restrict__ dbeta_part) {
+    constexpr int VN = VecOf<T>::N;
+    const long long item = (long long)blockIdx.x * 256 + threadIdx.x;
+    if (item >= items) return;
+    const int cvn = C / VN;
+    const int n = (int)(item / cvn), c = (int)(item - (long long)n * cvn) * VN;
+    float a1[VN], a2[VN], keep[VN];
+    gsrc_vload<T, SLABS>(g1, n, c, a1);
+    gsrc_vload<T, SLABS>(g2, n, c, a2);
+    if (mask) mask_vload8(mask + (long long)n * C + c, keep, VN);
+#pragma unroll
+    for (int k = 0; k < VN; ++k) {
+        float a = 0.f * gamma[c + k] + beta[c + k];
+        const float kp = mask ? keep[k] : 1.f;
+        a *= kp;
+        float slope = 1.f;
+        if (act == P2P_ACT_LEAKY) slope = a > 0.f ? 1.f : alpha;
+        else if (act == P2P_ACT_RELU) slope = a > 0.f ? 1.f : 0.f;
+        const float d = (a1[k] + a2[k]) * slope * kp;
+        dbeta_part[(long long)n * C + c + k] = 0.f + d;
+        dgamma_part[(long long)n * C + c + k] = 0.f;
+    }
+}
+
+static bool gsrc_vec_ok(const p2p_gsrc* g, int vn) {
+    if (!g || !g->ptr || g->kind != 1) return true;
+    return g->ld % vn == 0 && g->coff % vn == 0 && ((uintptr_t)g->ptr % 16) == 0;
+}
+
+extern "C" int p2p_norm_act_fwd_1x1(int dtype, int N, int C, const float* gamma, const float* beta, int act, float alpha,
+                                    const unsigned char* mask, const p2p_tensor* out, void* stream) {
+    P2P_REQUIRE(N > 0 && C > 0, "p2p_norm_act_fwd_1x1: bad shape");
+    P2P_REQUIRE(gamma && beta && out && out->ptr, "p2p_norm_act_fwd_1x1: null pointer");
+    const int vn = dtype == P2P_BF16 ? 8 : 4;
+    P2P_REQUIRE(C % 8 == 0 && out->ld % vn == 0 && ((uintptr_t)out->ptr % 16) == 0,
+                "p2p_norm_act_fwd_1x1: pixels must be whole 16-byte vectors (C %% 8 == 0, aligned view)");
+    const long long items = (long long)N * (C / vn);
+    const dim3 grid((unsigned)((items + 255) / 256));
+    P2P_DISPATCH_DTYPE(dtype, (norm_act_fwd_1x1_kernel<T><<<grid, 256, 0, (hipStream_t)stream>>>(C, items, gamma, beta, act, alpha, mask,
+                                                                                                 make_view(out))));
+    return p2p_check_launch("p2p_norm_act_fwd_1x1");
+}
+
+extern "C" int p2p_norm_act_bwd_1x1(int dtype, int N, int C, const float* gamma, const float* beta, int act, float alpha,
+                                    const unsigned char* mask, const p2p_gsrc* g1, const p2p_gsrc* g2, float* dgamma_part,
+                                    float* dbeta_part, void* stream) {
+    P2P_REQUIRE(N > 0 && C > 0, "p2p_norm_act_bwd_1x1: bad shape");
+    P2P_REQUIRE(gamma && beta && g1 && dgamma_part && dbeta_part, "p2p_norm_act_bwd_1x1: null pointer");
+    const int vn = dtype == P2P_BF16 ? 8 : 4;
+    P2P_REQUIRE(C % 8 == 0 && gsrc_vec_ok(g1, vn) && gsrc_vec_ok(g2, vn),
+                "p2p_norm_act_bwd_1x1: pixels must be whole 16-byte vectors (C %% 8 == 0, aligned gradient sources)");
+    const bool g_slabs = g1->kind == 2 || (g2 && g2->kind == 2);
+    const long long items = (long long)N * (C / vn);
+    const dim3 grid((unsigned)((items + 255) / 256));
+    hipStream_t st = (hipStream_t)stream;
+#define NB_1X1(S_) norm_act_bwd_1x1_kernel<T, S_><<<grid, 256, 0, st>>>(C, items, gamma, beta, act, alpha, mask, make_gsrc(g1), make_gsrc(g2), \
+                                                                       dgamma_part, dbeta_part)
+    if (g_slabs) { P2P_DISPATCH_DTYPE(dtype, NB_1X1(4)); }
+    else { P2P_DISPATCH_DTYPE(dtype, NB_1X1(0)); }
+#undef NB_1X1
+    return p2p_check_launch("p2p_norm_act_bwd_1x1");
+}
+
 extern "C" int p2p_colsum(const float* part, int rows, int cols, float scale, float* out, void* stream) {
     P2P_REQUIRE(part && out && rows > 0 && cols > 0, "p2p_colsum: bad args");
     colsum_kernel<<<dim3((cols + 255) / 256), 256, 0, (hipStream_t)stream>>>(part, rows, cols, scale, out);
diff --git a/palette_and_histo_gan_amd/csrc/optim.hip b/palette_and_histo_gan_amd/csrc/optim.hip
--- a/palette_and_histo_gan_amd/csrc/optim.hip
+++ b/palette_and_histo_gan_amd/csrc/optim.hip
@@ -34,6 +34,15 @@
     lr_t[0] = (float)((double)lr * sqrt(1.0 - pow((double)b2, (double)tt)) / (1.0 - pow((double)b1, (double)tt)));
 }
 
+__device__ __forceinline__ void adam_update(float& p, float g, float& m, float& v, float lr_t, float b1, float b2, float eps,
+                                            float gscale) {
+#pragma clang fp contract(off)
+    const float gg = g * gscale;
+    m = __builtin_fmaf(1.f - b1, gg, b1 * m);
+    v = __builtin_fmaf(b2, v, ((1.f - b2) * gg) * gg);
+    p = p - lr_t * m / (sqrtf(v) + eps);
+}
+
 __global__ void adam_flat_dev_kernel(float* __restrict__ p, const float* __restrict__ g, float* __restrict__ m,
                                      float* __restrict__ v, long long n, const float* __restrict__ lr_t_dev, float b1,
                                      float b2, float eps, float gscale) {
@@ -44,19 +53,14 @@
         f32x4 gi = *(const f32x4*)(g + i), mi = *(const f32x4*)(m + i), vi = *(const f32x4*)(v + i), pi = *(const f32x4*)(p + i);
 #pragma unroll
         for (int k = 0; k < 4; ++k) {
-            float gg = gi[k] * gscale;
-            mi[k] = b1 * mi[k] + (1.f - b1) * gg;
-            vi[k] = b2 * vi[k] + (1.f - b2) * gg * gg;
-            pi[k] = pi[k] - lr_t * mi[k] / (sqrtf(vi[k]) + eps);
+            float pk = pi[k], mk = mi[k], vk = vi[k];
+            adam_update(pk, gi[k], mk, vk, lr_t, b1, b2, eps, gscale);
+            pi[k] = pk; mi[k] = mk; vi[k] = vk;
         }
         *(f32x4*)(m + i) = mi; *(f32x4*)(v + i) = vi; *(f32x4*)(p + i) = pi;
     }
     if (blockIdx.x == 0 && threadIdx.x == 0)
-        for (long long j = n / 4 * 4; j < n; ++j) {
-            float gg = g[j] * gscale;
-            float mj = b1 * m[j] + (1.f - b1) * gg, vj = b2 * v[j] + (1.f - b2) * gg * gg;
-            m[j] = mj; v[j] = vj; p[j] = p[j] - lr_t * mj / (sqrtf(vj) + eps);
-        }
+        for (long long j = n / 4 * 4; j < n; ++j) adam_update(p[j], g[j], m[j], v[j], lr_t, b1, b2, eps, gscale);
 }
 
 extern "C" int p2p_adam_tick(int* t_dev, float* lr_t_dev, float lr, float beta1, float beta2, void* stream) {
@@ -75,6 +79,52 @@
     if (blocks < 1) blocks = 1;
     adam_flat_dev_kernel<<<dim3((unsigned)blocks), 256, 0, (hipStream_t)stream>>>(p, g, m, v, n, lr_t_dev, beta1, beta2, eps, gscale);
     return p2p_check_launch("p2p_adam_flat_dev");
+}
+
+__global__ void adam_flat_dev_excl_kernel(float* __restrict__ p, const float* __restrict__ g, float* __restrict__ m,
+                                          float* __restrict__ v, long long n, long long ex_lo, long long ex_hi,
+                                          const float* __restrict__ lr_t_dev, float b1, float b2, float eps, float gscale) {
+    const float lr_t = lr_t_dev[0];
+    const long long hv_lo = (ex_lo + 3) / 4, hv_hi = ex_hi / 4;
+    const long long hole = hv_hi > hv_lo ? hv_hi - hv_lo : 0;
+    const long long live = n / 4 - hole;
+    long long q = (long long)blockIdx.x * blockDim.x + threadIdx.x;
+    const long long stride = (long long)gridDim.x * blockDim.x;
+    for (; q < live; q += stride) {
+        const long long i = (q < hv_lo ? q : q + hole) * 4;
+        if (i + 4 <= ex_lo || i >= ex_hi) {
+            f32x4 gi = *(const f32x4*)(g + i), mi = *(const f32x4*)(m + i), vi = *(const f32x4*)(v + i), pi = *(const f32x4*)(p + i);
+#pragma unroll
+            for (int k = 0; k < 4; ++k) {
+                float pk = pi[k], mk = mi[k], vk = vi[k];
+                adam_update(pk, gi[k], mk, vk, lr_t, b1, b2, eps, gscale);
+                pi[k] = pk; mi[k] = mk; vi[k] = vk;
+            }
+            *(f32x4*)(m + i) = mi; *(f32x4*)(v + i) = vi; *(f32x4*)(p + i) = pi;
+        } else {
+            for (long long j = i; j < i + 4; ++j)
+                if (j < ex_lo || j >= ex_hi) adam_update(p[j], g[j], m[j], v[j], lr_t, b1, b2, eps, gscale);
+        }
+    }
+    if (blockIdx.x == 0 && threadIdx.x == 0)
+        for (long long j = n / 4 * 4; j < n; ++j)
+            if (j < ex_lo || j >= ex_hi) adam_update(p[j], g[j], m[j], v[j], lr_t, b1, b2, eps, gscale);
+}
+
+extern "C" int p2p_adam_flat_dev_excl(float* p, const float* g, float* m, float* v, long long n, long long ex_lo, long long ex_hi,
+                                      const float* lr_t_dev, float beta1, float beta2, float eps, float gscale, void* stream) {
+    P2P_REQUIRE(p && g && m && v && n > 0 && lr_t_dev, "p2p_adam_flat_dev_excl: bad args");
+    P2P_REQUIRE(0 <= ex_lo && ex_lo <= ex_hi && ex_hi <= n, "p2p_adam_flat_dev_excl: the excluded range must lie inside [0, n)");
+    P2P_REQUIRE(((uintptr_t)p % 16) == 0 && ((uintptr_t)g % 16) == 0 && ((uintptr_t)m % 16) == 0 && ((uintptr_t)v % 16) == 0,
+                "p2p_adam_flat_dev_excl: buffers must be 16-byte aligned");
+    const long long hv_lo = (ex_lo + 3) / 4, hv_hi = ex_hi / 4;
+    const long long live = n / 4 - (hv_hi > hv_lo ? hv_hi - hv_lo : 0);
+    long long blocks = (live + 255) / 256;
+    if (blocks > 8192) blocks = 8192;
+    if (blocks < 1) blocks = 1;
+    adam_flat_dev_excl_kernel<<<dim3((unsigned)blocks), 256, 0, (hipStream_t)stream>>>(p, g, m, v, n, ex_lo, ex_hi, lr_t_dev, beta1,
+                                                                                       beta2, eps, gscale);
+    return p2p_check_launch("p2p_adam_flat_dev_excl");
 }
 
 __global__ void counter_add_kernel(long long* c, long long inc) { c[0] += inc; }
diff --git a/palette_and_histo_gan_amd/csrc/replay.hip b/palette_and_histo_gan_amd/csrc/replay.hip
--- a/palette_and_histo_gan_amd/csrc/replay.hip
+++ b/palette_and_histo_gan_amd/csrc/replay.hip
@@ -40,11 +40,11 @@
     P2P_E(p2p_conv_fewin_actbwd) P2P_E(p2p_conv_fewout) P2P_E(p2p_wgemm_edge)
     P2P_E(p2p_wgrad_small) P2P_E(p2p_view_colsum) P2P_E(p2p_act_bwd)
     P2P_E(p2p_weight_prep_pad) P2P_E(p2p_wgemm) P2P_E(p2p_norm_act_fwd)
-    P2P_E(p2p_norm_act_fwd_tail) P2P_E(p2p_norm_act_bwd) P2P_E(p2p_colsum)
+    P2P_E(p2p_norm_act_fwd_tail) P2P_E(p2p_norm_act_bwd) P2P_E(p2p_norm_act_fwd_1x1) P2P_E(p2p_norm_act_bwd_1x1) P2P_E(p2p_colsum)
     P2P_E(p2p_colsum_batched) P2P_E(p2p_bce_logits) P2P_E(p2p_bce_logits_pad8)
     P2P_E(p2p_loss_partials_sum) P2P_E(p2p_tanh_l1_fwd) P2P_E(p2p_tanh_l1_fwd_pair)
     P2P_E(p2p_tanh_l1_bwd) P2P_E(p2p_tanh_l1_bwd_pad8) P2P_E(p2p_adam_flat)
-    P2P_E(p2p_adam_tick) P2P_E(p2p_adam_flat_dev) P2P_E(p2p_counter_add) P2P_E(p2p_grad_accumulate)
+    P2P_E(p2p_adam_tick) P2P_E(p2p_adam_flat_dev) P2P_E(p2p_adam_flat_dev_excl) P2P_E(p2p_counter_add) P2P_E(p2p_grad_accumulate)
     P2P_E(p2p_dropout_mask_dev) P2P_E(p2p_weight_prep) P2P_E(p2p_weight_prep_batched)
     P2P_E(p2p_adam_prep_batched) P2P_E(p2p_pack_input) P2P_E(p2p_pack_pair)
     P2P_E(p2p_pack_pair_idx) P2P_E(p2p_pack_input_multi) P2P_E(p2p_finish_losses)
diff --git a/palette_and_histo_gan_amd/engine.py b/palette_and_histo_gan_amd/engine.py
--- a/palette_and_histo_gan_amd/engine.py
+++ b/palette_and_histo_gan_amd/engine.py
@@ -449,6 +449,14 @@
         self.use_head_fused = os.environ.get("P2P_HEAD_FUSED", "1") != "0"
         self.hist_fwd3 = self.hist_bwd3 = self.hist_points = 1
         self.split_prep = int(os.environ.get("P2P_SPLIT_PREP", "1"))
+        self.elide_dead_bottleneck = int(os.environ.get("P2P_ELIDE_DEAD", "1"))
+        self._dead = next((i for i in range(2, len(DOWN_FILTERS) + 1) if img_size // 2 ** i == 1), None)
+        self._frozen = None
+        if self._dead is not None:
+            o = self.G.offsets[f"down{self._dead}.kernel"]
+            self._frozen = (o, o + int(np.prod(self.G.shapes[f"down{self._dead}.kernel"])))
+        self._frozen_ok = None
+        self._elide = 0
         self.refresh_weight_copies()
 
     def _slot_property(slot):
@@ -504,14 +512,19 @@
                     lw.wd = torch.zeros(16 * cg * cd, dtype=tdt, device=dev)
                 self.W[(sid, name)] = lw
 
-    def _prep_tasks(self, part="all"):
+    def _prep_tasks(self, part="all", live=False):
+        want = part
+        if live:
+            part = (part, "live")
         if self._prep_table.get(part) is not None:
             return self._prep_table[part]
         head_end = self.G.buckets[-1][0] if len(self.G.buckets) >= 2 else 0
         specs = []
         for (sid, name), lw in self.W.items():
             in_head = sid == "G" and self.G.offsets[name + ".kernel"] + 16 * lw.cg * lw.cd <= head_end
-            if (part == "head" and not in_head) or (part == "rest" and in_head) or (part in ("G", "D") and sid != part):
+            if (want == "head" and not in_head) or (want == "rest" and in_head) or (want in ("G", "D") and sid != want):
+                continue
+            if live and (sid, name) == ("G", f"down{self._dead}"):
                 continue
             master = self._store(sid).p(name + ".kernel")
             if lw.wt is not None or lw.wn is not None:
@@ -588,9 +601,11 @@
         L.call("p2p_adam_prep_batched", self.dtype, n_elems, _p(raw), ntasks, total, _p(store.params), _p(store.grads), _p(store.m),
                _p(store.v), _p(store.lr_t_dev), self._slot_b1, self._slot_b2, self._slot_eps, _stream())
 
-    def refresh_weight_copies(self, part="all"):
+    def refresh_weight_copies(self, part="all", outside=True):
         self._copies_version += 1
-        raw, ntasks, total = self._prep_tasks(part)
+        if outside:
+            self._frozen_ok = None
+        raw, ntasks, total = self._prep_tasks(part, live=bool(self._elide))
         if ntasks:
             L.call("p2p_weight_prep_batched", self.dtype, _p(raw), ntasks, total, _stream())
 
@@ -601,6 +616,33 @@
     def _wd(self, sid, name):
         lw = self.W[(sid, name)]
         return _p(lw.wd) if lw.wd is not None else self._store(sid).p(name + ".kernel")
+
+    def _elision(self):
+        lvl = int(self.elide_dead_bottleneck)
+        if not lvl or self._dead is None or self.batch_invariant or not self.use_mfma or self.fuse_adam:
+            return 0
+        if self._frozen_ok is None:
+            lo, hi = self._frozen
+            self._frozen_ok = self.device.type != "cuda" or not any(
+                bool(torch.count_nonzero(t[lo:hi])) for t in (self.G.grads, self.G.m, self.G.v))
+        return lvl if self._frozen_ok else 0
+
+    def _zero_raw(self, P, N, c):
+        z = P.get("zraw")
+        if z is None:
+            z = P["zraw"] = DenseBuf(N, 1, 1, c, self.tdt, self.device)
+            z.t.zero_()
+        return z
+
+    def _adam_range(self, store, lo, hi):
+        ex = self._frozen if (self._elide >= 2 and store is self.G) else None
+        if ex is not None and lo <= ex[0] and ex[1] <= hi:
+            L.call("p2p_adam_flat_dev_excl", _p(store.params, lo), _p(store.grads, lo), _p(store.m, lo), _p(store.v, lo), hi - lo,
+                   ex[0] - lo, ex[1] - lo, _p(store.lr_t_dev), self._slot_b1, self._slot_b2, self._slot_eps, 1.0, _stream())
+            return
+        assert ex is None or ex[1] <= lo or hi <= ex[0], "the dead kernel straddles an Adam range"
+        L.call("p2p_adam_flat_dev", _p(store.params, lo), _p(store.grads, lo), _p(store.m, lo), _p(store.v, lo), hi - lo,
+               _p(store.lr_t_dev), self._slot_b1, self._slot_b2, self._slot_eps, 1.0, _stream())
 
     def set_params(self, g_values=None, d_values=None):
         if g_values is not None:
@@ -824,19 +866,23 @@
                                 and UP_FILTERS[5] % 8 == 0 and S * S > 16)
         return P[key]
 
-    def _wgrad(self, P, sid, name, N, lh, hi, lo, stride=2, dbias=None):
+    def _wgrad(self, P, sid, name, N, lh, hi, lo, stride=2, dbias=None, dead=False):
+        dp = self._dp
+        nb, b = len(self.G.buckets), self.G.bucket_of[name] if sid == "G" else None
+        closes = sid == "G" and self.G.bucket_last_layer[b] == name
+        head_done = dp is None and closes and self.side.enabled and nb >= 2 and b == nb - 2
+        reduce_now = dp is not None and closes and b != nb - 1
+        if dead and not (head_done or reduce_now):
+            return
         self.side.fork()
         with self.side.run():
-            self._wgrad_impl(P, sid, name, N, lh, hi, lo, stride, dbias)
-            dp = self._dp
-            if dp is None and sid == "G" and self.side.enabled and len(self.G.buckets) >= 2 \
-                    and self.G.bucket_last_layer[len(self.G.buckets) - 2] == name:
+            if not dead:
+                self._wgrad_impl(P, sid, name, N, lh, hi, lo, stride, dbias)
+            if head_done:
                 self._adam_head_ev = _record_event()
-            if dp is not None and sid == "G":
-                b = self.G.bucket_of[name]
-                if self.G.bucket_last_layer[b] == name and b != len(self.G.buckets) - 1:
-                    lo_e, hi_e = self.G.buckets[b]
-                    dp.allreduce_async(self.G.grads[lo_e:hi_e])
+            if reduce_now:
+                lo_e, hi_e = self.G.buckets[b]
+                dp.allreduce_async(self.G.grads[lo_e:hi_e])
 
     def _wgrad_impl(self, P, sid, name, N, lh, hi, lo, stride=2, dbias=None):
         lw = self.W[(sid, name)]
@@ -905,9 +951,10 @@
         slabs = rk[2] if len(rk) == 3 else P["slabs"]
         return L.GSrc(slabs.data_ptr(), 2, rk[1], buf.n * buf.h * buf.w * buf.c, buf.c, coff)
 
-    def _norm_bwd(self, P, name, N, res, c, raw_buf, stats, act, mask, g1, g2, draw_view):
+    def _norm_bwd(self, P, name, N, res, c, raw_buf, stats, act, mask, g1, g2, draw_view, fork_follows=True):
         ob, og = P["part_off"][name]
-        self.side.prefork()
+        if fork_follows:
+            self.side.prefork()
         L.call("p2p_norm_act_bwd", self.dtype, N, res, res, c, raw_buf.ptr(), _p(stats), self.G.p(name + ".gamma"),
                self.G.p(name + ".beta"), act, LEAKY_ALPHA, _p(mask) if mask is not None else NULL, C.byref(g1),
                C.byref(g2) if g2 is not None else None, C.byref(draw_view), _p(P["part"], og), _p(P["part"], ob),
@@ -945,7 +992,7 @@
         return (kind, B, self.side.enabled, self.side.stop_event_forks, self.side_hist.enabled, self.fuse_adam, self.use_head_fused, self.hist_fwd3, self.hist_bwd3,
                 self.hist_points, self.fuse_act_bwd, self.split_prep, self.full_pixels, self.use_conv_fewout, self.use_conv_strip, self.use_conv_fewin,
                 self.use_mfma, bool(self.batch_invariant), bool(self.wgemm_pipe), int(self.splitk_target), int(self.wgemm_want), int(self.wgemm_want_pipe),
-                int(st.cuda_stream), int(st.stream_id),
+                int(st.cuda_stream), int(st.stream_id), int(self._elide),
                 None if dp is None else id(dp)) + extra
 
     def _bind_batch(self, src_t, real_t):
@@ -1048,6 +1095,13 @@
             out_view = P["a6"].view() if i == 6 else c[6 - i].view(coff=UP_FILTERS[5 - i])
             if i == 1:
                 self._conv(P, L.OP_G, "G", "down1", B, res, src_view, out_view, act=L.ACT_LEAKY, tmp=P["rd"].get(1))
+            elif self._elide and i == self._dead:
+                if self._elide >= 2:
+                    L.call("p2p_norm_act_fwd_1x1", self.dtype, B, f, self.G.p(f"down{i}.gamma"), self.G.p(f"down{i}.beta"),
+                           L.ACT_LEAKY, LEAKY_ALPHA, NULL, C.byref(out_view), _stream())
+                else:
+                    self._norm_fwd(P, B, res, f, self._zero_raw(P, B, f), (1, 1), self.G.p(f"down{i}.gamma"),
+                                   self.G.p(f"down{i}.beta"), L.ACT_LEAKY, None, out_view, P["sd"][i])
             elif self._fused_block(P, L.OP_G, f"down{i}", B, res, src_view, P["rd"][i], L.ACT_LEAKY, out_view, P["sd"][i]):
                 pass
             else:
@@ -1120,22 +1174,26 @@
         self._dp = dp
         self._batch_offset = int(batch_offset)
         src_t, real_t = self._to_device(source, ic, B), self._to_device(real, ic, B)
-        key = self._replay_key("rgba", B, masks, dp, apply_update, float(lambda_l1),
-                               None if lambda_hist is None else float(lambda_hist), Bg, int(batch_offset))
-        if key in self._replays:
-            return self._replay(key, P, src_t, real_t, hist=lambda_hist is not None)
-        recording = self._begin_record(key)
-        if recording and dp is not None:
-            dp = self._dp = _RecDP(dp)
+        self._elide = self._elision()
         try:
-            out = self._train_step_rgba_body(P, B, Bg, src_t, real_t, lambda_l1, lambda_hist, masks, apply_update, dp)
-        except BaseException:
+            key = self._replay_key("rgba", B, masks, dp, apply_update, float(lambda_l1),
+                                   None if lambda_hist is None else float(lambda_hist), Bg, int(batch_offset))
+            if key in self._replays:
+                return self._replay(key, P, src_t, real_t, hist=lambda_hist is not None)
+            recording = self._begin_record(key)
+            if recording and dp is not None:
+                dp = self._dp = _RecDP(dp)
+            try:
+                out = self._train_step_rgba_body(P, B, Bg, src_t, real_t, lambda_l1, lambda_hist, masks, apply_update, dp)
+            except BaseException:
+                if recording:
+                    self._end_record(key, False)
+                raise
             if recording:
-                self._end_record(key, False)
-            raise
-        if recording:
-            self._end_record(key, True)
-        return out
+                self._end_record(key, True)
+            return out
+        finally:
+            self._elide = 0
 
     def _train_step_rgba_body(self, P, B, Bg, src_t, real_t, lambda_l1, lambda_hist, masks, apply_update, dp):
         S, ic = self.S, self.in_ch
@@ -1271,6 +1329,18 @@
             else:
                 g1 = self._gs(P, gc[6 - i], rk_gc[6 - i], UP_FILTERS[5 - i])
                 g2 = g_from_down
+            if self._elide and i == self._dead:
+                if self._elide >= 2:
+                    ob, og = P["part_off"][f"down{i}"]
+                    L.call("p2p_norm_act_bwd_1x1", self.dtype, B, f, self.G.p(f"down{i}.gamma"), self.G.p(f"down{i}.beta"),
+                           L.ACT_LEAKY, LEAKY_ALPHA, NULL, C.byref(g1), C.byref(g2) if g2 is not None else None,
+                           _p(P["part"], og), _p(P["part"], ob), _stream())
+                else:
+                    self._norm_bwd(P, f"down{i}", B, res, f, self._zero_raw(P, B, f), P["sd"][i], L.ACT_LEAKY, None, g1, g2,
+                                   P["dd"][i].view(), fork_follows=False)
+                self._wgrad(P, "G", f"down{i}", B, res, None, None, dead=True)
+                g_from_down = None
+                continue
             if i > 1:
                 self._norm_bwd(P, f"down{i}", B, res, f, P["rd"][i], P["sd"][i], L.ACT_LEAKY, None, g1, g2,
                                P["dd"][i].view())
@@ -1348,10 +1418,9 @@
             self._adam_prep("G_head")
             self._head_prepped = True
             return n
-        L.call("p2p_adam_flat_dev", _p(self.G.params), _p(self.G.grads), _p(self.G.m), _p(self.G.v), n,
-               _p(self.G.lr_t_dev), self._slot_b1, self._slot_b2, self._slot_eps, 1.0, _stream())
+        self._adam_range(self.G, 0, n)
         if self.split_prep:
-            self.refresh_weight_copies("head")
+            self.refresh_weight_copies("head", outside=False)
             self._head_prepped = True
         return n
 
@@ -1382,13 +1451,11 @@
             store.t += 1
             if not ticked:
                 L.call("p2p_adam_tick", _p(store.t_dev), _p(store.lr_t_dev), self._slot_lr, self._slot_b1, self._slot_b2, _stream())
-            off = g_from if store is self.G else 0
-            L.call("p2p_adam_flat_dev", _p(store.params, off), _p(store.grads, off), _p(store.m, off), _p(store.v, off),
-                   store.numel - off, _p(store.lr_t_dev), self._slot_b1, self._slot_b2, self._slot_eps, 1.0, _stream())
+            self._adam_range(store, g_from if store is self.G else 0, store.numel)
         if not ticked:
             L.call("p2p_counter_add", _p(self.mask_counter_dev), 1, _stream())
         head_done, self._head_prepped = self._head_prepped and g_from > 0, False
-        self.refresh_weight_copies("rest" if head_done else "all")
+        self.refresh_weight_copies("rest" if head_done else "all", outside=False)
 
     def _histogram_loss(self, P, B, Bg, lambda_hist, hist_allreduce):
         S = self.S
@@ -1463,21 +1530,25 @@
         self._batch_offset = int(batch_offset)
         src_t = self._to_device(source_idx, 1, B, is_int=True)
         real_t = self._to_device(real_idx, 1, B, is_int=True)
-        key = self._replay_key("indexed", B, masks, dp, apply_update, float(lambda_segmentation), Bg, int(batch_offset))
-        if key in self._replays:
-            return self._replay(key, P, src_t, real_t)
-        recording = self._begin_record(key)
-        if recording and dp is not None:
-            self._dp = _RecDP(dp)
+        self._elide = self._elision()
         try:
-            out = self._train_step_indexed_body(P, B, Bg, src_t, real_t, lambda_segmentation, masks, apply_update)
-        except BaseException:
+            key = self._replay_key("indexed", B, masks, dp, apply_update, float(lambda_segmentation), Bg, int(batch_offset))
+            if key in self._replays:
+                return self._replay(key, P, src_t, real_t)
+            recording = self._begin_record(key)
+            if recording and dp is not None:
+                self._dp = _RecDP(dp)
+            try:
+                out = self._train_step_indexed_body(P, B, Bg, src_t, real_t, lambda_segmentation, masks, apply_update)
+            except BaseException:
+                if recording:
+                    self._end_record(key, False)
+                raise
             if recording:
-                self._end_record(key, False)
-            raise
-        if recording:
-            self._end_record(key, True)
-        return out
+                self._end_record(key, True)
+            return out
+        finally:
+            self._elide = 0
 
     def _pack_indexed(self, P, B, src_t, real_t):
         S = self.S
@@ -1631,7 +1702,7 @@
         for t, c in snap:
             t.copy_(c)
         self.G.t, self.D.t = t_host
-        self.refresh_weight_copies()
+        self.refresh_weight_copies(outside=False)
         torch.cuda.synchronize(self.device)
         graph = torch.cuda.CUDAGraph()
         with torch.cuda.graph(graph):
diff --git a/palette_and_histo_gan_amd/flops.py b/palette_and_histo_gan_amd/flops.py
--- a/palette_and_histo_gan_amd/flops.py
+++ b/palette_and_histo_gan_amd/flops.py
@@ -105,6 +105,14 @@
         t = n * h * w * c
         by = t * esz + _gsrc_bytes(args[12], t, esz) + (_gsrc_bytes(args[13], t, esz) if args[13] is not None else 0) + t * esz
         return {"flops": 0.0, "mfma": None, "bytes": by}
+    if name == "p2p_norm_act_fwd_1x1":
+        _, n, c = _ints(args, 3)
+        return {"flops": 0.0, "mfma": None, "bytes": float(n * c * esz)}
+    if name == "p2p_norm_act_bwd_1x1":
+        _, n, c = _ints(args, 3)
+        t = n * c
+        return {"flops": 0.0, "mfma": None,
+                "bytes": _gsrc_bytes(args[8], t, esz) + (_gsrc_bytes(args[9], t, esz) if args[9] is not None else 0) + 2 * 4.0 * t}
     if name == "p2p_act_bwd":
         _, n, h, w, c = _ints(args, 5)
         t = n * h * w * c
@@ -144,6 +152,8 @@
         return {"flops": 0.0, "mfma": None, "bytes": n * h * w * (2.0 * c * esz + 2 * 8 * esz)}
     if name == "p2p_adam_flat_dev":
         return {"flops": 0.0, "mfma": None, "bytes": 7 * 4.0 * int(args[4])}
+    if name == "p2p_adam_flat_dev_excl":
+        return {"flops": 0.0, "mfma": None, "bytes": 7 * 4.0 * (int(args[4]) - (int(args[6]) - int(args[5])))}
     if name == "p2p_adam_prep_batched":
         return {"flops": 0.0, "mfma": None, "bytes": (7 * 4.0 + 2 * esz) * int(args[1])}
     if name == "p2p_pack_pair":
```

After: 136,500, median of 6. 1.6% higher.
